# heyblackC/DFMIR

Measured on AMD Instinct MI355X. Metric: train-step image-pairs/sec (fwd+bwd): 2D 256x256 bs=16 and 3D 160^3 bs=1, higher is better.
Workload: dtype f32 (fp16x2-split MFMA, fp32 accumulate)

## Files before the change

dfmir_amd/csrc/common.h:

```cpp
#pragma once
#include <hip/hip_runtime.h>
#include <stdint.h>
#include <stdlib.h>
#include <atomic>
#include "../../include/dfmir_hip.h"

#define DF_LAUNCH_CHECK()                                  \
  do {                                                     \
    hipError_t e_ = hipGetLastError();                     \
    if (e_ != hipSuccess) return df_set_error((int)e_, __FILE__, __LINE__); \
  } while (0)
#define DF_ARG_CHECK(cond)                                 \
  do {                                                     \
    if (!(cond)) return df_set_error(-1, __FILE__, __LINE__); \
  } while (0)

int df_set_error(int code, const char* file, int line);

bool df_opt_get(const char* name, char* buf, int buf_len);
int df_opt_gen();
static inline bool df_opt_on(const char* name) {
  char b[8];
  return df_opt_get(name, b, sizeof(b)) && b[0] != 0 && !(b[0] == '0' && b[1] == 0);
}
struct DfOptFlag {
  const char* name;
  std::atomic<long long> st{-1};
  bool get() {
    const int g = df_opt_gen();
    const long long s = st.load(std::memory_order_relaxed);
    if (s >= 0 && (int)(s >> 1) == g) return (s & 1) != 0;
    const bool v = df_opt_on(name);
    st.store(((long long)g << 1) | (v ? 1 : 0), std::memory_order_relaxed);
    return v;
  }
};
struct DfOptInt {
  const char* name;
  int def;
  std::atomic<long long> st{-1};
  int get() {
    const int g = df_opt_gen();
    const long long s = st.load(std::memory_order_relaxed);
    if (s >= 0 && (int)(s >> 32) == g) return (int)(unsigned)(s & 0xffffffffLL);
    char b[32];
    const int v = df_opt_get(name, b, sizeof(b)) ? atoi(b) : def;
    st.store(((long long)g << 32) | (unsigned)v, std::memory_order_relaxed);
    return v;
  }
};

static inline unsigned df_grid(long long n, int bs, long long cap = 1LL << 20) {
  long long b = (n + bs - 1) / bs;
  if (b < 1) b = 1;
  if (b > cap) b = cap;
  return (unsigned)b;
}

static inline int df_cu_count() {
  static std::atomic<int> cache[64];
  int dev = 0;
  if (hipGetDevice(&dev) != hipSuccess || dev < 0 || dev >= 64) return 256;
  int v = cache[dev].load(std::memory_order_relaxed);
  if (v > 0) return v;
  if (hipDeviceGetAttribute(&v, hipDeviceAttributeMultiprocessorCount, dev) != hipSuccess || v <= 0) v = 256;
  cache[dev].store(v, std::memory_order_relaxed);
  return v;
}

const float* df_det_fx();
__device__ __forceinline__ void df_acc(float* base, long long idx, float v, const float* fx) {
  if (fx) atomicAdd(reinterpret_cast<unsigned long long*>(base) + idx, (unsigned long long)__float2ll_rn(v * fx[0]));
  else atomicAdd(base + idx, v);
}

static __global__ void df_zero_small_k(float* __restrict__ p, int n) {
  const int i = blockIdx.x * blockDim.x + threadIdx.x;
  if (i < n) p[i] = 0.f;
}
static inline hipError_t df_zero_async(float* p, int n, hipStream_t st) {
  df_zero_small_k<<<(unsigned)((n + 63) / 64), 64, 0, st>>>(p, n);
  return hipGetLastError();
}

__device__ __forceinline__ float wave_sum(float v) {
#pragma unroll
  for (int o = 32; o > 0; o >>= 1) v += __shfl_down(v, o, 64);
  return v;
}
__device__ __forceinline__ double wave_sum(double v) {
#pragma unroll
  for (int o = 32; o > 0; o >>= 1) v += __shfl_down(v, o, 64);
  return v;
}
__device__ __forceinline__ float wave_max(float v) {
#pragma unroll
  for (int o = 32; o > 0; o >>= 1) v = fmaxf(v, __shfl_down(v, o, 64));
  return v;
}

__device__ __forceinline__ float block_sum(float v, float* sm ) {
  const int lane = threadIdx.x & 63, wid = threadIdx.x >> 6;
  const int nw = (blockDim.x + 63) >> 6;
  v = wave_sum(v);
  __syncthreads();
  if (lane == 0) sm[wid] = v;
  __syncthreads();
  if (wid == 0) {
    float t = (lane < nw) ? sm[lane] : 0.f;
    t = wave_sum(t);
    if (lane == 0) sm[16] = t;
  }
  __syncthreads();
  return sm[16];
}
template <int T>
__device__ __forceinline__ double block_sum_ordered(double v, double* sm ) {
  v = wave_sum(v);
  __syncthreads();
  if ((threadIdx.x & 63) == 0) sm[threadIdx.x >> 6] = v;
  __syncthreads();
  double t = 0.0;
  if (threadIdx.x == 0)
    for (int w = 0; w < T / 64; ++w) t += sm[w];
  return t;
}
template <int T>
static __global__ __launch_bounds__(T) void df_slot_mean_k(const double* __restrict__ part, int nslots, double count,
                                                           float* __restrict__ out) {
  __shared__ double red[T / 64];
  double s = 0.0;
  for (int i = threadIdx.x; i < nslots; i += T) s += part[i];
  s = block_sum_ordered<T>(s, red);
  if (threadIdx.x == 0) out[0] = (float)(s / count);
}
__device__ __forceinline__ float block_max(float v, float* sm) {
  const int lane = threadIdx.x & 63, wid = threadIdx.x >> 6;
  const int nw = (blockDim.x + 63) >> 6;
  v = wave_max(v);
  __syncthreads();
  if (lane == 0) sm[wid] = v;
  __syncthreads();
  if (wid == 0) {
    float t = (lane < nw) ? sm[lane] : -3.0e38f;
    t = wave_max(t);
    if (lane == 0) sm[16] = t;
  }
  __syncthreads();
  return sm[16];
}
__device__ __forceinline__ void publish_block_absmax(float m, unsigned* smax, float* out_block) {
  const float t = wave_max(m);
  if ((threadIdx.x & 63) == 0) atomicMax(smax, __float_as_uint(t == t ? t : __uint_as_float(0x7f800000u)));
  __syncthreads();
  if (threadIdx.x == 0) *out_block = __uint_as_float(*smax);
}
#define DF_PROBE_SLOTS 64
__device__ __forceinline__ void publish_block_absmax_acc(float m, unsigned* smax, float* out) {
  const float t = wave_max(m);
  if ((threadIdx.x & 63) == 0) atomicMax(smax, __float_as_uint(t == t ? t : __uint_as_float(0x7f800000u)));
  __syncthreads();
  if (threadIdx.x == 0) atomicMax(reinterpret_cast<unsigned*>(out) + (blockIdx.x & (DF_PROBE_SLOTS - 1)), *smax);
}
__device__ __forceinline__ float reduce_absmax(const float* __restrict__ a, int n, float* sm) {
  if (n <= 1) return a[0];
  float m = 0.f;
  for (int i = threadIdx.x; i < n; i += blockDim.x) m = fmaxf(m, a[i]);
  return block_max(m, sm);
}

__device__ __forceinline__ bool df_in_coord(int o, int t, int stride, int pad, int dil, int size,
                                            int pad_mode, int& idx) {
  int c = o * stride - pad + t;
  if (dil == 1) {
    if (pad_mode == 1) {
      if (c < 0) c = -c;
      if (c >= size) c = 2 * (size - 1) - c;
      c = c < 0 ? 0 : (c >= size ? size - 1 : c);
      idx = c;
      return true;
    }
    idx = c;
    return (unsigned)c < (unsigned)size;
  }
  if (c < 0) { idx = 0; return false; }
  int q = c / dil;
  idx = q;
  return (q * dil == c) && (q < size);
}
```

dfmir_amd/csrc/conv3x3s.hip:

```cpp
#include "split_f16.h"

#ifndef PP_COMPUTE_PRIO
#define PP_COMPUTE_PRIO 1
#endif
#ifndef CS_COMPUTE_PRIO
#define CS_COMPUTE_PRIO 1
#endif
#ifndef CS_STORE_PRIO
#define CS_STORE_PRIO 0
#endif
typedef __bf16 bf16x8 __attribute__((ext_vector_type(8)));
typedef __bf16 bf16x2 __attribute__((ext_vector_type(2)));
typedef _Float16 f16x2 __attribute__((ext_vector_type(2)));
typedef float f32x2 __attribute__((ext_vector_type(2)));

__device__ __forceinline__ unsigned pk_bf16(float a, float b) {
  const f32x2 v = {a, b};
  return __builtin_bit_cast(unsigned, __builtin_convertvector(v, bf16x2));
}

template <int NSP>
__device__ __forceinline__ void split_pair(float x0, float x1, unsigned (&p)[NSP]) {
  if constexpr (NSP == 3) {
    p[0] = pk_bf16(x0, x1);
    const float r0 = x0 - __uint_as_float(p[0] << 16), r1 = x1 - __uint_as_float(p[0] & 0xffff0000u);
    p[1] = pk_bf16(r0, r1);
    p[2] = pk_bf16(r0 - __uint_as_float(p[1] << 16), r1 - __uint_as_float(p[1] & 0xffff0000u));
  } else {
    const f32x2 v = {x0, x1};
    const f16x2 h = __builtin_convertvector(v, f16x2);
    const f32x2 r = v - __builtin_convertvector(h, f32x2);
    p[0] = __builtin_bit_cast(unsigned, h);
    p[1] = __builtin_bit_cast(unsigned, __builtin_convertvector(r, f16x2));
  }
}
template <int NSP>
__device__ __forceinline__ void split_pair_s(float x0, float x1, float s, unsigned (&p)[NSP]) {
  if constexpr (NSP == 2) split_pair_scaled(x0, x1, s, p[0], p[1]);
  else split_pair<NSP>(x0, x1, p);
}
template <int NSP>
__device__ __forceinline__ void split8(const float v[8], u32x4 (&out)[NSP]) {
#pragma unroll
  for (int w = 0; w < 4; ++w) {
    unsigned p[NSP];
    split_pair<NSP>(v[2 * w], v[2 * w + 1], p);
#pragma unroll
    for (int s = 0; s < NSP; ++s) out[s][w] = p[s];
  }
}
template <int NSP>
__device__ __forceinline__ void split8_s(const float v[8], float s, u32x4 (&out)[NSP]) {
  if constexpr (NSP == 2) split8_scaled(v, s, out[0], out[1]);
  else split8<NSP>(v, out);
}
template <int NSP>
__device__ __forceinline__ f32x16 mma16(u32x4 a, u32x4 b, f32x16 c) {
  if constexpr (NSP == 3)
    return __builtin_amdgcn_mfma_f32_32x32x16_bf16(__builtin_bit_cast(bf16x8, a), __builtin_bit_cast(bf16x8, b), c, 0, 0, 0);
  else
    return mfma32_f16(a, b, c);
}
template <int NSP> struct Prod;
template <> struct Prod<3> { static constexpr int N = 6; static constexpr int A[6] = {2, 0, 1, 1, 0, 0}, B[6] = {0, 2, 1, 0, 1, 0}; };
template <> struct Prod<2> { static constexpr int N = 3; static constexpr int A[3] = {1, 0, 0}, B[3] = {0, 1, 0}; };

__global__ __launch_bounds__(256) void absmax_k(const float* __restrict__ x, long long n, unsigned* __restrict__ out) {
  __shared__ float red[8];
  float m = 0.f;
  const long long n4 = n >> 2;
  const float4* x4 = reinterpret_cast<const float4*>(x);
  const long long st = (long long)gridDim.x * 256;
  long long i = (long long)blockIdx.x * 256 + threadIdx.x;
  const float4 z4 = make_float4(0.f, 0.f, 0.f, 0.f);
  for (; i < n4; i += 4 * st) {
    const float4 a = x4[i];
    const float4 b = i + st < n4 ? x4[i + st] : z4;
    const float4 c = i + 2 * st < n4 ? x4[i + 2 * st] : z4;
    const float4 d = i + 3 * st < n4 ? x4[i + 3 * st] : z4;
    const float ma = fmaxf(fmaxf(fabsf(a.x), fabsf(a.y)), fmaxf(fabsf(a.z), fabsf(a.w)));
    const float mb = fmaxf(fmaxf(fabsf(b.x), fabsf(b.y)), fmaxf(fabsf(b.z), fabsf(b.w)));
    const float mc = fmaxf(fmaxf(fabsf(c.x), fabsf(c.y)), fmaxf(fabsf(c.z), fabsf(c.w)));
    const float md = fmaxf(fmaxf(fabsf(d.x), fabsf(d.y)), fmaxf(fabsf(d.z), fabsf(d.w)));
    m = fmaxf(m, fmaxf(fmaxf(ma, mb), fmaxf(mc, md)));
  }
  for (i = (n4 << 2) + (long long)blockIdx.x * 256 + threadIdx.x; i < n; i += (long long)gridDim.x * 256)
    m = fmaxf(m, fabsf(x[i]));
#pragma unroll
  for (int o = 32; o > 0; o >>= 1) m = fmaxf(m, __shfl_xor(m, o));
  if ((threadIdx.x & 63) == 0) red[threadIdx.x >> 6] = m;
  __syncthreads();
  if (threadIdx.x == 0) {
    m = fmaxf(fmaxf(red[0], red[1]), fmaxf(red[2], red[3]));
    if (!(m == m)) m = __uint_as_float(0x7f800000u);
    if (__float_as_uint(m) > *reinterpret_cast<volatile unsigned*>(out)) atomicMax(out, __float_as_uint(m));
  }
}
int df_absmax_launch(const float* x, long long n, float* out, hipStream_t st, bool zero_first) {
  if (zero_first) {
    hipError_t e = df_zero_async(out, 1, st);
    if (e != hipSuccess) return (int)e;
  }
  long long blocks = (n / 4 + 255) / 256;
  if (blocks < 1) blocks = 1;
  if (blocks > 2048) blocks = 2048;
  absmax_k<<<(unsigned)blocks, 256, 0, st>>>(x, n, reinterpret_cast<unsigned*>(out));
  return (int)hipGetLastError();
}

template <int NSP>
__global__ __launch_bounds__(256) void weight_split_k(const float* __restrict__ w_tcc, u32x4* __restrict__ out,
                                                      float* __restrict__ trailer, int npart, int K, int M) {
  __shared__ float red[17];
  const int chunks = (K + 7) >> 3;
  const long long total = (long long)chunks * 9 * M;
  int e = 0;
  if (NSP == 2) {
    e = scale_exp(reduce_absmax(trailer + 4, npart, red));
    if (blockIdx.x == 0 && threadIdx.x == 0) trailer[1] = (float)e;
  }
  const float sc = pow2f(e);
  for (long long i = (long long)blockIdx.x * 256 + threadIdx.x; i < total; i += (long long)gridDim.x * 256) {
    const int m = (int)(i % M);
    const int tap = (int)((i / M) % 9);
    const int ch = (int)(i / ((long long)9 * M));
    float v[8];
#pragma unroll
    for (int j = 0; j < 8; ++j) {
      const int kk = ch * 8 + j;
      v[j] = kk < K ? w_tcc[((long long)tap * K + kk) * M + m] * sc : 0.f;
    }
    u32x4 sp[NSP];
    split8<NSP>(v, sp);
    const long long base = (long long)ch * 9 * NSP * M + (long long)tap * M + m;
#pragma unroll
    for (int s = 0; s < NSP; ++s) out[base + (long long)s * 9 * M] = sp[s];
  }
}

int df_split_mode() {
  static std::atomic<long long> st{-1};
  const int g = df_opt_gen();
  const long long cur = st.load(std::memory_order_relaxed);
  if (cur >= 0 && (int)(cur >> 8) == g) return (int)(cur & 0xff);
  char s[16];
  const bool has = df_opt_get("DFMIR_CONV_SPLIT", s, sizeof(s));
  const int mode = df_opt_on("DFMIR_CONV_FP32") ? 0 : ((has && s[0] == 'b') ? 3 : 2);
  st.store(((long long)g << 8) | mode, std::memory_order_relaxed);
  return mode;
}

static inline float* split_section(const float* packed, int K, int M) {
  return const_cast<float*>(packed) + df_pack_tcc_floats(K, M, 9);
}
static inline float* split_trailer(const float* packed, int K, int M, int nsp) {
  return split_section(packed, K, M) + (long long)((K + 7) / 8) * 9 * nsp * M * 4;
}

float* df_weight_probe_slots(float* packed, int K, int M) {
  const int mode = df_split_mode();
  return mode == 2 ? split_trailer(packed, K, M, mode) + 4 : nullptr;
}
int df_weight_split_launch(const float* w_tcc, float* packed, int K, int M, int npart, hipStream_t st) {
  const int mode = df_split_mode();
  if (mode == 0) return 0;
  const long long total = (long long)((K + 7) / 8) * 9 * M;
  u32x4* sec = reinterpret_cast<u32x4*>(split_section(packed, K, M));
  float* tr = split_trailer(packed, K, M, mode);
  if (mode == 2) weight_split_k<2><<<df_grid(total, 256, 2048), 256, 0, st>>>(w_tcc, sec, tr, npart, K, M);
  else weight_split_k<3><<<df_grid(total, 256, 2048), 256, 0, st>>>(w_tcc, sec, tr, npart, K, M);
  return (int)hipGetLastError();
}

template <int NSP>
__global__ __launch_bounds__(256) void weight_split_batch_k(const DfPackJobDev* __restrict__ jobs) {
  const DfPackJobDev jb = jobs[blockIdx.y];
  if ((int)blockIdx.x >= jb.nsplit) return;
  __shared__ float red[17];
  const int K = jb.mode ? jb.Cout : jb.Cin, M = jb.mode ? jb.Cin : jb.Cout;
  const int chunks = (K + 7) >> 3;
  const long long total = (long long)chunks * 9 * M;
  int e = 0;
  if (NSP == 2) {
    e = scale_exp(reduce_absmax(jb.trailer + 4, jb.nblk, red));
    if (blockIdx.x == 0 && threadIdx.x == 0) jb.trailer[1] = (float)e;
  }
  const float sc = pow2f(e);
  u32x4* out = reinterpret_cast<u32x4*>(jb.sec);
  for (long long i = (long long)blockIdx.x * 256 + threadIdx.x; i < total; i += (long long)jb.nsplit * 256) {
    const int m = (int)(i % M);
    const int tap = (int)((i / M) % 9);
    const int ch = (int)(i / ((long long)9 * M));
    float v[8];
#pragma unroll
    for (int j = 0; j < 8; ++j) {
      const int kk = ch * 8 + j;
      v[j] = kk < K ? jb.o[((long long)tap * K + kk) * M + m] * sc : 0.f;
    }
    u32x4 sp[NSP];
    split8<NSP>(v, sp);
    const long long base = (long long)ch * 9 * NSP * M + (long long)tap * M + m;
#pragma unroll
    for (int s = 0; s < NSP; ++s) out[base + (long long)s * 9 * M] = sp[s];
  }
}
void df_weight_split_fill(DfPackJobDev* j) {
  const int mode = df_split_mode();
  j->part = nullptr; j->sec = nullptr; j->trailer = nullptr; j->nsplit = 0;
  if (j->T != 9 || mode == 0) return;
  const int K = j->mode ? j->Cout : j->Cin, M = j->mode ? j->Cin : j->Cout;
  j->sec = split_section(j->o, K, M);
  j->trailer = split_trailer(j->o, K, M, mode);
  j->part = mode == 2 ? j->trailer + 4 : nullptr;
  j->nsplit = (int)df_grid((long long)((K + 7) / 8) * 9 * M, 256, 2048);
}
int df_weight_split_batch_launch(const DfPackJobDev* jobs_dev, int njobs, int max_nsplit, hipStream_t st) {
  const int mode = df_split_mode();
  if (mode == 0 || max_nsplit <= 0) return 0;
  const dim3 grid((unsigned)max_nsplit, (unsigned)njobs);
  if (mode == 2) weight_split_batch_k<2><<<grid, 256, 0, st>>>(jobs_dev);
  else weight_split_batch_k<3><<<grid, 256, 0, st>>>(jobs_dev);
  return (int)hipGetLastError();
}

template <int NSP, int BM, int XP, int TM, int TN, int NV>
__device__ __forceinline__ void split_mma_chunk(const u32x4* __restrict__ Ab, const u32x4* __restrict__ Xb,
                                                const int (&aoff)[5], const int (&bidx)[5][TN],
                                                f32x16 (&acc)[TM][TN]) {
  using P = Prod<NSP>;
  u32x4 a[2][TM][NSP], b[2][TN][NSP];
#define SPLIT_LOAD(set_, pr_)                                                                    \
  {                                                                                              \
    _Pragma("unroll") for (int i = 0; i < TM; ++i)                                               \
      _Pragma("unroll") for (int s = 0; s < NSP; ++s) a[set_][i][s] = Ab[s * 9 * BM + aoff[pr_] + i * 32]; \
    _Pragma("unroll") for (int j = 0; j < TN; ++j)                                               \
      _Pragma("unroll") for (int s = 0; s < NSP; ++s) b[set_][j][s] = Xb[s * XP + bidx[pr_][j]]; \
  }
  SPLIT_LOAD(0, 0)
#pragma unroll
  for (int pr = 0; pr < 5; ++pr) {
    if (pr < 4) SPLIT_LOAD((pr + 1) & 1, pr + 1)
#pragma unroll
    for (int q = 0; q < P::N; ++q)
#pragma unroll
      for (int i = 0; i < TM; ++i)
#pragma unroll
        for (int j = 0; j < TN; ++j)
          acc[i][j] = mma16<NSP>(a[pr & 1][i][P::A[q]], b[pr & 1][j][P::B[q]], acc[i][j]);
  }
#undef SPLIT_LOAD
  constexpr int NL = NSP * (TM + TN), NM = P::N * TM * TN;
  constexpr int LP = NL < NM ? NL : NM;
  constexpr int VP = ((NV + 3) / 4 < NM - LP) ? (NV + 3) / 4 : NM - LP;
#pragma unroll
  for (int i = 0; i < NL; ++i) __builtin_amdgcn_sched_group_barrier(0x100, 1, 0);
#pragma unroll
  for (int pr = 0; pr < 4; ++pr) {
#pragma unroll
    for (int i = 0; i < LP; ++i) {
      __builtin_amdgcn_sched_group_barrier(0x008, 1, 0);
      __builtin_amdgcn_sched_group_barrier(0x100, 1, 0);
      if (i == LP - 1) {
#pragma unroll
        for (int e = 0; e < NL - LP; ++e) __builtin_amdgcn_sched_group_barrier(0x100, 1, 0);
      }
    }
#pragma unroll
    for (int i = 0; i < VP; ++i) {
      __builtin_amdgcn_sched_group_barrier(0x008, 1, 0);
      __builtin_amdgcn_sched_group_barrier(0x020, 1, 0);
    }
#pragma unroll
    for (int i = 0; i < NM - LP - VP; ++i) __builtin_amdgcn_sched_group_barrier(0x008, 1, 0);
  }
#pragma unroll
  for (int i = 0; i < NM; ++i) __builtin_amdgcn_sched_group_barrier(0x008, 1, 0);
}

struct SplitScale {
  const float* x_amax;
  int x_n;
  const float* w_trailer;
};

template <int NSP, int XP, int BM>
__global__ __launch_bounds__(512, 1) void conv3x3_split_pp_k(const float* __restrict__ x,
                                                             const u32x4* __restrict__ ws,
                                                             const float* __restrict__ bias,
                                                             float* __restrict__ y, Conv3P k, SplitScale sc) {
  constexpr int BNG = 128, CK = 8, TM = 2, TN = (BM == 128) ? 2 : 1, WN = (BM == 128) ? 2 : 4;
  constexpr int NS = (XP + 255) / 256;
  constexpr int WU = 9 * NSP * BM, WH = WU / 2;
  constexpr int NW = (WH + 255) / 256;
  constexpr int ZPOS = XP - 1;
  __shared__ __attribute__((aligned(16))) u32x4 As[2][WU];
  __shared__ __attribute__((aligned(16))) u32x4 Xs[2][NSP * XP];
  __shared__ float bs[BM];

  const int grp = threadIdx.x >> 8, tid = threadIdx.x & 255, lane = tid & 63, wid = tid >> 6;
  const int wm = wid / WN, wn = wid % WN;
  const int l31 = lane & 31, lhi = lane >> 5;
  const int HWo = k.Ho * k.Wo, HWi = k.Hi * k.Wi;
  const int n = blockIdx.x / k.tiles_per_img;
  const int t = blockIdx.x - n * k.tiles_per_img;
  const int p0 = t * (2 * BNG) + grp * BNG;
  const bool gvalid = p0 < HWo;
  const int pend = (p0 + BNG < HWo) ? p0 + BNG : HWo;
  const int m0 = blockIdx.y * BM;
  const int y0 = p0 / k.Wo, y1 = (pend - 1) / k.Wo;
  const bool single = (y0 == y1);
  const int x0 = p0 - y0 * k.Wo, x1 = (pend - 1) - y1 * k.Wo;
  const int xoff = single ? x0 : 0;
  const int ncols = single ? (x1 - x0 + 3) : (k.Wo + 2);
  const int nrows = y1 - y0 + 3;
  const int npos = gvalid ? nrows * ncols : 0;
  u32x4* __restrict__ Xg = Xs[grp];

  float xscale = 1.f, oscale = 1.f, oscale2 = 1.f;
  if (NSP == 2) {
    const int ex = scale_exp(reduce_absmax(sc.x_amax, sc.x_n, bs));
    __syncthreads();
    const int ew = (int)sc.w_trailer[1];
    xscale = pow2f(ex);
    oscale = pow2f(-ex);
    oscale2 = pow2f(-ew);
  }

  constexpr unsigned OOB = 0x80000000u;
  unsigned gvo[NS][CK];
#pragma unroll
  for (int s = 0; s < NS; ++s) {
    const int pos = tid + 256 * s;
    int off = -1;
    if (pos < npos) {
      const int r = pos / ncols, c = pos - r * ncols;
      off = halo_offset(y0 - k.pad + r, xoff - k.pad + c, k.Hi, k.Wi, k.pad_mode);
    }
#pragma unroll
    for (int c = 0; c < CK; ++c) gvo[s][c] = off < 0 ? OOB : (unsigned)(off + c * HWi) * 4u;
  }
  if ((int)threadIdx.x < BM) bs[threadIdx.x] = (bias && (m0 + (int)threadIdx.x) < k.Cout) ? bias[m0 + threadIdx.x] : 0.f;
  if (tid < NSP) Xg[tid * XP + ZPOS] = u32x4{0u, 0u, 0u, 0u};

  int pbase[TN];
#pragma unroll
  for (int j = 0; j < TN; ++j) {
    int q = p0 + (wn * TN + j) * 32 + l31;
    q = q < pend ? q : pend - 1;
    const int yy = q / k.Wo, xx = q - yy * k.Wo;
    pbase[j] = (yy - y0) * ncols + (xx - xoff);
  }
  int aoff[5], bidx[5][TN];
#pragma unroll
  for (int pr = 0; pr < 5; ++pr) {
    const int tp = (pr == 4) ? 8 : 2 * pr + lhi;
    aoff[pr] = tp * BM + wm * TM * 32 + l31;
#pragma unroll
    for (int j = 0; j < TN; ++j)
      bidx[pr][j] = ((pr == 4) && lhi) ? ZPOS : pbase[j] + (tp / 3) * ncols + (tp % 3);
  }

  f32x16 acc[TM][TN];
#pragma unroll
  for (int i = 0; i < TM; ++i)
#pragma unroll
    for (int j = 0; j < TN; ++j)
#pragma unroll
      for (int r = 0; r < 16; ++r) acc[i][j][r] = 0.f;

  const float* xn = x + (long long)n * k.Cin * HWi;
  const int chunks = (k.Cin + CK - 1) / CK;
  unsigned wbyte[NW];
#pragma unroll
  for (int j = 0; j < NW; ++j) {
    const int loc = tid + 256 * j;
    const int idx = grp * WH + loc;
    const int seg = idx / BM, co = m0 + (idx % BM);
    wbyte[j] = (loc < WH && co < k.Cout) ? (unsigned)(seg * k.Cout + co) * 16u : OOB;
  }
  const int wunits = 9 * NSP * k.Cout;

  u32x4 rw[NW];
  unsigned rx[NS][CK];

#define P3_GLOADW(ch_)                                                                           \
  {                                                                                              \
    const int c_ = (ch_);                                                                        \
    const __amdgpu_buffer_rsrc_t rw_ = __builtin_amdgcn_make_buffer_rsrc(                        \
        const_cast<u32x4*>(ws + (long long)c_ * wunits), 0, c_ < chunks ? (unsigned)wunits * 16u : 0u, 0x00020000); \
    _Pragma("unroll") for (int j = 0; j < NW; ++j)                                               \
      rw[j] = __builtin_amdgcn_raw_buffer_load_b128(rw_, wbyte[j], 0, 0);                        \
  }
#define P3_GLOADX(ch_)                                                                           \
  {                                                                                              \
    const int c0_ = (ch_) * CK;                                                                  \
    const int left_ = k.Cin - c0_;                                                               \
    const __amdgpu_buffer_rsrc_t rx_ = __builtin_amdgcn_make_buffer_rsrc(                        \
        const_cast<float*>(xn + (long long)c0_ * HWi), 0,                                        \
        left_ > 0 ? (unsigned)((left_ < CK ? left_ : CK) * HWi) * 4u : 0u, 0x00020000);          \
    _Pragma("unroll") for (int s = 0; s < NS; ++s) {                                             \
      _Pragma("unroll") for (int c = 0; c < CK; ++c)                                             \
        rx[s][c] = __builtin_amdgcn_raw_buffer_load_b32(rx_, gvo[s][c], 0, 0);                   \
    }                                                                                            \
  }
#define P3_LSTOREW(buf_)                                                                         \
  {                                                                                              \
    _Pragma("unroll") for (int j = 0; j < NW; ++j) {                                             \
      const int loc = tid + 256 * j;                                                             \
      if (loc < WH) As[buf_][grp * WH + loc] = rw[j];                                            \
    }                                                                                            \
  }
#define P3_LSTOREX()                                                                             \
  {                                                                                              \
    _Pragma("unroll") for (int s = 0; s < NS; ++s) {                                             \
      const int pos = tid + 256 * s;                                                             \
      if (pos < npos) {                                                                          \
        float v[8];                                                                              \
        _Pragma("unroll") for (int c = 0; c < CK; ++c)                                           \
          v[c] = __uint_as_float(rx[s][c]);                                                      \
        u32x4 sp[NSP];                                                                           \
        split8_s<NSP>(v, xscale, sp);                                                                      \
        _Pragma("unroll") for (int q = 0; q < NSP; ++q) Xg[q * XP + pos] = sp[q];                \
      }                                                                                          \
    }                                                                                            \
  }

  P3_GLOADW(0);
  P3_GLOADX(0);
  P3_LSTOREW(0);
  P3_LSTOREX();
  if (grp == 1 && chunks > 1) P3_GLOADW(1);
  __syncthreads();

  for (int h = 0; h < 2 * chunks; ++h) {
    const int c = h >> 1;
    if ((h & 1) == grp) {
      __builtin_amdgcn_s_setprio(PP_COMPUTE_PRIO);
      if (gvalid) {
        P3_GLOADX(c + 1);
        P3_GLOADW(c + 1 + grp);
        split_mma_chunk<NSP, BM, XP, TM, TN, NW + NS * CK>(As[c & 1], Xg, aoff, bidx, acc);
      } else {
        P3_GLOADW(c + 1 + grp);
      }
    } else {
      __builtin_amdgcn_s_setprio(0);
      const int cx = c + 1 - grp;
      if (cx < chunks && h > 0) P3_LSTOREX();
      if (c + 1 < chunks) P3_LSTOREW((c + 1) & 1);
    }
    __syncthreads();
  }
#undef P3_GLOADW
#undef P3_GLOADX
#undef P3_LSTOREW
#undef P3_LSTOREX

  if (!gvalid) return;
  float* yb = y + (long long)n * k.Cout * HWo;
#pragma unroll
  for (int j = 0; j < TN; ++j) {
    const int q = p0 + (wn * TN + j) * 32 + l31;
    if (q >= pend) continue;
#pragma unroll
    for (int i = 0; i < TM; ++i) {
      const int cl = (wm * TM + i) * 32 + 4 * lhi;
#pragma unroll
      for (int r = 0; r < 16; ++r) {
        const int cc = cl + (r & 3) + 8 * (r >> 2);
        const int co = m0 + cc;
        if (co < k.Cout) {
          float v = (NSP == 2 ? acc[i][j][r] * oscale * oscale2 : acc[i][j][r]) + bs[cc];
          if (k.act == 1) v = v > 0.f ? v : v * k.slope;
          else if (k.act == 2) v = tanhf(v);
          yb[(long long)co * HWo + q] = v;
        }
      }
    }
  }
}

constexpr int CS_TH = 8, CS_TW = 32, CS_PW = CS_TW + 2, CS_XP = 352;

template <int CPG, int XP, int NW, int NS>
__device__ __forceinline__ void cs_mma_chunk_rr(const u32x4* __restrict__ Ab, const u32x4* __restrict__ Xb, int abase,
                                                int xb, f32x16 (&acc)[4],
                                                const __amdgpu_buffer_rsrc_t rw_, const unsigned (&wb)[NW], u32x4 (&rw)[NW],
                                                const __amdgpu_buffer_rsrc_t rx_, const unsigned (&gvo)[NS][8],
                                                unsigned (&rx)[NS][8]) {
  constexpr int SA = 9 * 2 * CPG, SX = 2 * XP;
  constexpr int NL = NW + 8 * NS;
  using P = Prod<2>;
  u32x4 a[9][2], xr[3][6][2];
#define CS_LDA(st_, s_) a[st_][s_] = Ab[(s_) * SA + (((st_) % 3) * 3 + (st_) / 3) * (2 * CPG) + abase];
#define CS_LDX(kx_, r_, s_) xr[kx_][r_][s_] = Xb[(s_) * SX + xb + (r_) * CS_PW + (kx_)];
#define CS_NEED(n_)                                                                              \
  {                                                                                              \
    constexpr int kx_ = (n_) / 3, ky_ = (n_) % 3;                                                \
    CS_LDA(n_, 1)                                                                                \
    if (ky_ == 0) { _Pragma("unroll") for (int r = 0; r < 4; ++r) CS_LDX(kx_, r, 0) }            \
    else CS_LDX(kx_, ky_ + 3, 0)                                                                 \
    CS_LDA(n_, 0)                                                                                \
    if (ky_ == 0) { _Pragma("unroll") for (int r = 0; r < 4; ++r) CS_LDX(kx_, r, 1) }            \
    else CS_LDX(kx_, ky_ + 3, 1)                                                                 \
  }
  CS_NEED(0)
  __builtin_amdgcn_sched_barrier(0);
#pragma unroll
  for (int st = 0; st < 9; ++st) {
    const int kx = st / 3, ky = st % 3;
    int nds = 0;
    if (st == 0) { CS_NEED(1) CS_NEED(2) nds = 8; }
    else if (st == 1) { CS_NEED(3) nds = 10; }
    else if (st == 2) { CS_NEED(4) nds = 4; }
    else if (st == 3) { CS_NEED(5) nds = 4; }
    else if (st == 4) { CS_NEED(6) nds = 10; }
    else if (st == 5) { CS_NEED(7) nds = 4; }
    else if (st == 6) { CS_NEED(8) nds = 4; }
    int L0, nvm;
    if (NL == 25) {
      L0 = st == 0 ? 0 : st == 1 ? 4 : st == 2 ? 6 : st == 3 ? 10 : st == 4 ? 14 : st == 5 ? 16 : st == 6 ? 20 : 24;
      nvm = (st == 1 || st == 4) ? 2 : (st == 7 ? 1 : (st == 8 ? 0 : 4));
    } else {
      const int lo = NL / 8, ex = NL % 8;
      L0 = st * lo + (st < ex ? st : ex);
      nvm = st < 8 ? lo + (st < ex ? 1 : 0) : 0;
    }
#pragma unroll
    for (int q = 0; q < (NL + 7) / 8; ++q) {
      const int L = L0 + q;
      if (q < nvm) {
        if (L < NW) rw[L] = __builtin_amdgcn_raw_buffer_load_b128(rw_, wb[L], 0, 0);
        else if (L < NL) rx[(L - NW) >> 3][(L - NW) & 7] = __builtin_amdgcn_raw_buffer_load_b32(rx_, gvo[(L - NW) >> 3][(L - NW) & 7], 0, 0);
      }
    }
#pragma unroll
    for (int q = 0; q < P::N; ++q)
#pragma unroll
      for (int j = 0; j < 4; ++j)
        acc[j] = mma16<2>(xr[kx][ky + j][P::B[q]], a[st][P::A[q]], acc[j]);
#pragma unroll
    for (int i = 0; i < 12; ++i) {
      __builtin_amdgcn_sched_group_barrier(0x008, 1, 0);
      if (i < nds) __builtin_amdgcn_sched_group_barrier(0x100, 1, 0);
      if (i >= 12 - nvm) __builtin_amdgcn_sched_group_barrier(0x020, 1, 0);
    }
    __builtin_amdgcn_sched_barrier(0);
  }
#undef CS_NEED
#undef CS_LDA
#undef CS_LDX
}

struct ConvCsP {
  int N, Cin, Cout, Hi, Wi, Ho, Wo, pad, pad_mode, act;
  float slope;
  int tiles_x, tiles_y;
  const float* res;
  const float* ring;
  int ring_rl;
  int xcd_pair;
  int dephase;
  int vec4;
};

#ifdef CS_TRACE
__device__ unsigned g_cs_trace[8 * 32 * 8 + 8];
extern "C" int dfmir_cs_trace_dump(unsigned* out) {
  return (int)hipMemcpyFromSymbol(out, HIP_SYMBOL(g_cs_trace), sizeof(unsigned) * (8 * 32 * 8 + 8));
}
#define TRC(slot_) { if (trace_blk && lane == 0) trc[((grp * 4 + wid) * 32 + (h & 31)) * 8 + (slot_)] = (unsigned)__builtin_readcyclecounter(); }
__device__ unsigned g_cs_wg[2048 * 6];
extern "C" int dfmir_cs_wg_dump(unsigned* out) {
  return (int)hipMemcpyFromSymbol(out, HIP_SYMBOL(g_cs_wg), sizeof(unsigned) * 2048 * 6);
}
#define WGT(slot_) { if (threadIdx.x == 0 && bix < 2048 && biy == 0) g_cs_wg[bix * 6 + (slot_)] = (unsigned)wall_clock64(); }
#else
#define WGT(slot_)
#define TRC(slot_)
#endif
template <int CPG, int TH>
struct CsLds {
  static constexpr int XP = (TH == 8 ? CS_XP : 640);
  static constexpr int WUG = 2 * 9 * 2 * CPG;
  static constexpr int XSU = 2 * 2 * XP;
  static constexpr int XS_OFF = 2 * WUG * 16, BS_OFF = XS_OFF + 2 * XSU * 16, BYTES = BS_OFF + 2 * CPG * 4;
};
template <int CPG, int TH>
__global__ __launch_bounds__(512, 1) void conv3x3_split_cs_k(const float* __restrict__ x, const u32x4* __restrict__ ws,
                                                             const float* __restrict__ bias, float* __restrict__ y,
                                                             ConvCsP k, SplitScale sc) {
  using L = CsLds<CPG, TH>;
  __shared__ __attribute__((aligned(16))) u32x4 Wg[2][L::WUG];
  __shared__ __attribute__((aligned(16))) u32x4 Xs[2][L::XSU];
  __shared__ float bs[2 * CPG];
  const int bix = (int)blockIdx.x, biy = (int)blockIdx.y, gdx = (int)gridDim.x;
#include "conv3x3s_cs_body.inc"
}

#ifdef DFMIR_BUILD_W1
#include "../../scripts/ubench/conv3x3_split_w1.inc"
#endif

static bool cs_plan(const DfConvGeom* g, int* th_out, int* tx_out, int* ty_out) {
  if (df_split_mode() != 2) return false;
  const int th = g->Cout > 64 ? 8 : 16;
  const int tx = (g->Wo + CS_TW - 1) / CS_TW, ty = (g->Ho + th - 1) / th;
  const double fill = (double)g->Ho * g->Wo / ((double)tx * CS_TW * ty * th);
  if (!((long long)g->N * tx * ty < (1LL << 31) && fill >= 0.85)) return false;
  *th_out = th; *tx_out = tx; *ty_out = ty;
  return true;
}
static bool split_fwd_geom_ok(const DfConvGeom* g) {
  if (!(g->KD == 1 && g->KH == 3 && g->KW == 3 && g->Di == 1 && g->Do == 1 && g->stride == 1 && g->dil == 1))
    return false;
  if (g->Cout <= 32 || g->Cin < 16 || g->ph != g->pw || g->pd != 0) return false;
  const int p = g->ph;
  if (!(p == 1 || (p == 2 && g->pad_mode == 0))) return false;
  if (g->Ho != g->Hi + 2 * p - 2 || g->Wo != g->Wi + 2 * p - 2) return false;
  const long long HWo = (long long)g->Ho * g->Wo;
  if (HWo >= (1LL << 30) || (long long)g->Hi * g->Wi >= (1LL << 30)) return false;
  if ((long long)((g->Cin + 7) / 8) * 27 * g->Cout * 16 >= (1LL << 31)) return false;
  if (worst_npos(g->Wo, (int)HWo, 128) > 399) return false;
  return true;
}
int df_conv3x3_split_res_ok(const DfConvGeom* g) {
  int th, tx, ty;
  return (df_split_mode() == 2 && split_fwd_geom_ok(g) && cs_plan(g, &th, &tx, &ty)) ? 1 : 0;
}
struct CsLaunch {
  ConvCsP kc;
  dim3 grid;
  int form;
};
static bool cs_setup(const DfConvGeom* g, const float* res, const float* ring, int ring_rl, const float* y, CsLaunch* L) {
  int th = 0, tlx = 0, tly = 0;
  if (!cs_plan(g, &th, &tlx, &tly)) return false;
  ConvCsP kc{g->N, g->Cin, g->Cout, g->Hi, g->Wi, g->Ho, g->Wo, g->ph, g->pad_mode, g->act, g->slope, tlx, tly, res,
             ring, ring_rl, 0, 0, 0};
  kc.vec4 = (g->Wo % 4 == 0 && ((uintptr_t)y & 15) == 0 && ((uintptr_t)res & 15) == 0) ? 1 : 0;
  static DfOptInt dephase_o{"DFMIR_CS_DEPHASE", 0};
  const long long nb = (long long)g->N * tlx * tly;
  if (nb * ((g->Cout + 127) / 128) >= 512) kc.dephase = dephase_o.get();
  static DfOptInt xcd_o{"DFMIR_CS_XCD_PAIR", 2};
  const int xcd_pair = xcd_o.get();
  if (g->Cout > 64) {
    dim3 grid((unsigned)nb, (unsigned)((g->Cout + 127) / 128));
    if (xcd_pair && grid.y <= 2 && (nb & 7) == 0) {
      kc.xcd_pair = xcd_pair == 1 ? (grid.y == 2 ? 1 : 0) : (int)grid.y + 1;
      if (kc.xcd_pair) grid = dim3((unsigned)(grid.y * nb), 1u);
    }
    L->grid = grid;
    L->form = 1;
  } else {
    if (xcd_pair >= 2 && (nb & 7) == 0) kc.xcd_pair = 2;
    L->grid = dim3((unsigned)nb, 1u);
    L->form = 2;
  }
  L->kc = kc;
  return true;
}
bool df_conv3x3_split_fwd_try(const DfConvGeom* g, const float* x, const float* x_amax, int x_n, const float* w_packed,
                              const float* bias, const float* res, const float* ring, int ring_rl, float* y,
                              hipStream_t st, int* rc) {
  const int mode = df_split_mode();
  if (mode == 0 || (mode == 2 && !(x_amax && x_n > 0))) return false;
  if (!split_fwd_geom_ok(g)) return false;
  const int p = g->ph;
  const long long HWo = (long long)g->Ho * g->Wo;
  Conv3P k{g->N, g->Cin, g->Cout, g->Hi, g->Wi, g->Ho, g->Wo, p, g->pad_mode, g->act, g->slope, 0};
  const u32x4* ws = reinterpret_cast<const u32x4*>(split_section(w_packed, g->Cin, g->Cout));
  const SplitScale sc{x_amax, x_n, split_trailer(w_packed, g->Cin, g->Cout, mode)};
  CsLaunch cl;
  if (mode == 2 && cs_setup(g, res, ring, ring_rl, y, &cl)) {
    const ConvCsP& kc = cl.kc;
    if (cl.form == 1) {
#ifdef DFMIR_BUILD_W1
      static DfOptFlag w1_o{"DFMIR_CONV_W1"};
      if (w1_o.get() && kc.vec4 && g->act != 2 && (g->Cin % 16) == 0 && (g->Ho % 16) == 0 && (g->Wo % 32) == 0) {
        ConvCsP kw = kc;
        kw.tiles_y = g->Ho / 16;
        const long long nbw = (long long)g->N * kw.tiles_x * kw.tiles_y;
        const unsigned gyw = (unsigned)((g->Cout + 127) / 128);
        kw.xcd_pair = 0;
        dim3 gw((unsigned)nbw, gyw);
        if ((nbw & 7) == 0 && gyw <= 2) { kw.xcd_pair = (int)gyw + 1; gw = dim3((unsigned)(gyw * nbw), 1u); }
        conv3x3_split_w1_k<0><<<gw, 256, 0, st>>>(x, ws, bias, y, kw, sc);
      } else
#endif
      conv3x3_split_cs_k<64, 8><<<cl.grid, 512, 0, st>>>(x, ws, bias, y, kc, sc);
    } else {
      conv3x3_split_cs_k<32, 16><<<cl.grid, 512, 0, st>>>(x, ws, bias, y, kc, sc);
    }
    hipError_t e = hipGetLastError();
    *rc = (e == hipSuccess) ? 0 : df_set_error((int)e, __FILE__, __LINE__);
    return true;
  }
  if (res || ring) { *rc = df_set_error((int)hipErrorInvalidValue, __FILE__, __LINE__); return true; }
  k.tiles_per_img = (int)((HWo + 255) / 256);
  const bool big = g->Cout > 64;
  dim3 grid((unsigned)(g->N * k.tiles_per_img), big ? (unsigned)((g->Cout + 127) / 128) : 1u);
  if (mode == 2) {
    if (big) conv3x3_split_pp_k<2, 400, 128><<<grid, 512, 0, st>>>(x, ws, bias, y, k, sc);
    else conv3x3_split_pp_k<2, 400, 64><<<grid, 512, 0, st>>>(x, ws, bias, y, k, sc);
  } else {
    if (big) conv3x3_split_pp_k<3, 400, 128><<<grid, 512, 0, st>>>(x, ws, bias, y, k, sc);
    else conv3x3_split_pp_k<3, 400, 64><<<grid, 512, 0, st>>>(x, ws, bias, y, k, sc);
  }
  hipError_t e = hipGetLastError();
  *rc = (e == hipSuccess) ? 0 : df_set_error((int)e, __FILE__, __LINE__);
  return true;
}

struct WS3P {
  int N, Cin, Cout, H, W, pad_mode;
  int runs_per_row, runs_per_img, runs_total, runs_per_block;
  const float* x_amax;
  const float* dy_amax;
  int x_n, dy_n;
  float* db;
  const float* dy_pmax;
  int swap;
  float* dbx;
  const float* fx;
};

template <int NSP, int BC>
__global__ __launch_bounds__(512, 1) void conv3x3_wgrad_split_k(const float* __restrict__ x,
                                                                const float* __restrict__ dy,
                                                                float* __restrict__ dwt, WS3P k) {
  using P = Prod<NSP>;
  constexpr int CT = 64, NWC = BC / 32, KS = 4 / NWC, NSTEP = 18 / KS;
  constexpr int XSLAB = 2 * CT;
  __shared__ __attribute__((aligned(16))) u32x4 Xc[NSP * 3 * 4 * XSLAB];
  __shared__ __attribute__((aligned(16))) u32x4 Dy[NSP * 2 * 2 * BC];
  __shared__ float bsum[BC];

  const int tid = threadIdx.x, lane = tid & 63, wid = tid >> 6;
  const bool want_db = k.db != nullptr && blockIdx.y == 0;
  if (tid < BC) bsum[tid] = 0.f;
  float bacc = 0.f;
  const int wc = wid % NWC, wi = (wid / NWC) & 1, kh = wid / (2 * NWC);
  const int l31 = lane & 31, lhi = lane >> 5;
  const int HW = k.H * k.W;
  const int ci0 = blockIdx.y * CT, co0 = blockIdx.z * BC;
  const int run_beg = blockIdx.x * k.runs_per_block;
  int run_end = run_beg + k.runs_per_block;
  if (run_end > k.runs_total) run_end = k.runs_total;

  float xscale = 1.f, dscale = 1.f, oscale = 1.f, oscale2 = 1.f;
  if (NSP == 2) {
    __shared__ float red[17];
    const int ex = scale_exp(reduce_absmax(k.x_amax, k.x_n, red));
    __syncthreads();
    const int ed = scale_exp(reduce_absmax(k.dy_amax, k.dy_n, red));
    xscale = pow2f(ex); dscale = pow2f(ed); oscale = pow2f(-ex); oscale2 = pow2f(-ed);
  }

  const int xc = tid & 63, xu = (tid >> 6) & 1, xr = tid >> 7;
  const int dc = tid % BC, du = (tid / BC) & 1, dk = (tid / (2 * BC)) & 1;
  const bool dload = tid < 4 * BC;
  const unsigned hw4 = (unsigned)HW * 4u;
  constexpr unsigned OOB = 0x80000000u;

  f32x16 acc[9];
#pragma unroll
  for (int t = 0; t < 9; ++t)
#pragma unroll
    for (int r = 0; r < 16; ++r) acc[t][r] = 0.f;

  u32x4 rxa, rxb, rda, rdb;
  unsigned rxl, rxr;

#define WS_GLOAD(run_)                                                                           \
  {                                                                                              \
    const int n_ = (run_) / k.runs_per_img;                                                      \
    const int q_ = (run_) - n_ * k.runs_per_img;                                                 \
    const int yp_ = q_ / k.runs_per_row, xs_ = q_ - yp_ * k.runs_per_row;                        \
    const int y0_ = 2 * yp_, x0_ = 16 * xs_ + 8 * xu;                                            \
    const __amdgpu_buffer_rsrc_t bx_ = __builtin_amdgcn_make_buffer_rsrc(                        \
        const_cast<float*>(x + (long long)n_ * k.Cin * HW), 0, (unsigned)(k.Cin * HW) * 4u, 0x00020000); \
    const __amdgpu_buffer_rsrc_t bd_ = __builtin_amdgcn_make_buffer_rsrc(                        \
        const_cast<float*>(dy + (long long)n_ * k.Cout * HW), 0, (unsigned)(k.Cout * HW) * 4u, 0x00020000); \
    const bool cok_ = ci0 + xc < k.Cin;                                                          \
    const unsigned cb_ = (unsigned)(ci0 + xc) * hw4;                                             \
     \
                                             \
    int ry_ = y0_ - 1 + xr;                                                                      \
    bool rok_ = (unsigned)ry_ < (unsigned)k.H;                                                   \
    if (k.pad_mode == 1) { ry_ = ry_ < 0 ? -ry_ : (ry_ >= k.H ? 2 * (k.H - 1) - ry_ : ry_); rok_ = true; } \
    const int rb_ = ry_ * k.W;                                                                   \
    const bool lin_ = x0_ > 0, rin_ = x0_ + 8 < k.W;                                             \
    const int ol_ = rb_ + (lin_ ? x0_ - 1 : 1), or_ = rb_ + (rin_ ? x0_ + 8 : k.W - 2);          \
    const bool lok_ = rok_ && cok_ && (lin_ || k.pad_mode == 1), rrok_ = rok_ && cok_ && (rin_ || k.pad_mode == 1); \
    const unsigned xb_ = (rok_ && cok_) ? cb_ + (unsigned)(rb_ + x0_) * 4u : OOB;                \
    rxa = __builtin_amdgcn_raw_buffer_load_b128(bx_, xb_, 0, 0);                                 \
    rxb = __builtin_amdgcn_raw_buffer_load_b128(bx_, xb_ == OOB ? OOB : xb_ + 16u, 0, 0);        \
    rxl = __builtin_amdgcn_raw_buffer_load_b32(bx_, lok_ ? cb_ + (unsigned)ol_ * 4u : OOB, 0, 0); \
    rxr = __builtin_amdgcn_raw_buffer_load_b32(bx_, rrok_ ? cb_ + (unsigned)or_ * 4u : OOB, 0, 0); \
    const unsigned db_ = (co0 + dc >= k.Cout || !dload) ? OOB                                    \
        : (unsigned)(co0 + dc) * hw4 + (unsigned)((y0_ + dk) * k.W + 16 * xs_ + 8 * du) * 4u;    \
    rda = __builtin_amdgcn_raw_buffer_load_b128(bd_, db_, 0, 0);                                 \
    rdb = __builtin_amdgcn_raw_buffer_load_b128(bd_, db_ == OOB ? OOB : db_ + 16u, 0, 0);        \
  }
#define WS_LSTORE()                                                                              \
  {                                                                                              \
    float r[10];                                                                                 \
    r[0] = __uint_as_float(rxl); r[9] = __uint_as_float(rxr);                                    \
    _Pragma("unroll") for (int e = 0; e < 4; ++e) { r[1 + e] = __uint_as_float(rxa[e]); r[5 + e] = __uint_as_float(rxb[e]); } \
    unsigned pa[5][NSP], pb[4][NSP];                                                             \
    _Pragma("unroll") for (int i = 0; i < 5; ++i) split_pair_s<NSP>(r[2 * i], r[2 * i + 1], xscale, pa[i]); \
    if (NSP == 2) {             \
      _Pragma("unroll") for (int i = 0; i < 4; ++i)                                              \
        _Pragma("unroll") for (int s = 0; s < NSP; ++s) pb[i][s] = __builtin_amdgcn_alignbit(pa[i + 1][s], pa[i][s], 16); \
    } else {                                                                                     \
      _Pragma("unroll") for (int i = 0; i < 4; ++i) split_pair<NSP>(r[2 * i + 1], r[2 * i + 2], pb[i]); \
    }                                                                                            \
    _Pragma("unroll") for (int s = 0; s < NSP; ++s) {                                            \
      u32x4* dst = Xc + ((s * 3 * 4 + xr) * 2 + xu) * CT + xc;                                   \
      dst[0] = u32x4{pa[0][s], pa[1][s], pa[2][s], pa[3][s]};                                    \
      dst[4 * XSLAB] = u32x4{pb[0][s], pb[1][s], pb[2][s], pb[3][s]};                            \
      dst[8 * XSLAB] = u32x4{pa[1][s], pa[2][s], pa[3][s], pa[4][s]};                            \
    }                                                                                            \
    float v[8];                                                                                  \
    _Pragma("unroll") for (int e = 0; e < 4; ++e) { v[e] = __uint_as_float(rda[e]); v[4 + e] = __uint_as_float(rdb[e]); } \
    bacc += ((v[0] + v[1]) + (v[2] + v[3])) + ((v[4] + v[5]) + (v[6] + v[7]));    \
    u32x4 sp[NSP];                                                                               \
    split8_s<NSP>(v, dscale, sp);                                                                \
    if (dload) { _Pragma("unroll") for (int s = 0; s < NSP; ++s) Dy[((s * 2 + dk) * 2 + du) * BC + dc] = sp[s]; } \
  }

  if (run_beg < run_end) {
    WS_GLOAD(run_beg);
    WS_LSTORE();
  }
  __syncthreads();

  const int abase = lhi * CT + wi * 32 + l31 + (KS == 2 ? kh * XSLAB : 0);
  const int bbase = lhi * BC + wc * 32 + l31 + (KS == 2 ? kh * 2 * BC : 0);
  for (int run = run_beg; run < run_end; ++run) {
    const bool more = (run + 1) < run_end;
    if (more) WS_GLOAD(run + 1);
    u32x4 b[NSP], a[2][NSP];
#define WS_LOADA(set_, step_)                                                                    \
  _Pragma("unroll") for (int s = 0; s < NSP; ++s)                                                \
    a[set_][s] = Xc[((s * 3 + ((step_) % 3)) * 4 + (step_) / 9 + ((step_) % 9) / 3) * XSLAB + abase];
    WS_LOADA(0, 0)
#pragma unroll
    for (int step = 0; step < NSTEP; ++step) {
      if (step % 9 == 0) {
#pragma unroll
        for (int s = 0; s < NSP; ++s) b[s] = Dy[(s * 2 + step / 9) * 2 * BC + bbase];
      }
      if (step + 1 < NSTEP) WS_LOADA((step + 1) & 1, step + 1)
#pragma unroll
      for (int q = 0; q < P::N; ++q)
        acc[step % 9] = mma16<NSP>(a[step & 1][P::A[q]], b[P::B[q]], acc[step % 9]);
    }
#undef WS_LOADA
#pragma unroll
    for (int i = 0; i < 2 * NSP; ++i) __builtin_amdgcn_sched_group_barrier(0x100, 1, 0);
#pragma unroll
    for (int step = 0; step < NSTEP; ++step) {
      const int nr = (step + 1 < NSTEP ? NSP : 0) + ((step + 1) % 9 == 0 && step + 1 < NSTEP ? NSP : 0);
#pragma unroll
      for (int i = 0; i < P::N; ++i) {
        __builtin_amdgcn_sched_group_barrier(0x008, 1, 0);
        if (i < nr) __builtin_amdgcn_sched_group_barrier(0x100, 1, 0);
        if (i == P::N - 1) {
#pragma unroll
          for (int e = P::N; e < nr; ++e) __builtin_amdgcn_sched_group_barrier(0x100, 1, 0);
        }
      }
    }
    if (more) {
      __syncthreads();
      WS_LSTORE();
      __syncthreads();
    }
  }
#undef WS_GLOAD
#undef WS_LSTORE

  if (want_db) {
    if (dload) atomicAdd(&bsum[dc], bacc);
    __syncthreads();
    if (tid < BC && co0 + tid < k.Cout) atomicAdd(&k.db[co0 + tid], bsum[tid]);
  }
  const int co = co0 + wc * 32 + l31;
  if (co < k.Cout) {
#pragma unroll
    for (int t = 0; t < 9; ++t) {
#pragma unroll
      for (int r = 0; r < 16; ++r) {
        const int ci = ci0 + wi * 32 + 4 * lhi + (r & 3) + 8 * (r >> 2);
        if (ci < k.Cin)
          df_acc(dwt, ((long long)t * k.Cin + ci) * k.Cout + co, NSP == 2 ? acc[t][r] * oscale * oscale2 : acc[t][r], k.fx);
      }
    }
  }
}

struct RingP {
  int N, K, M, H, W;
  int RL;
  const float* cols;
};
constexpr int RING_KG = 32;

template <int RP>
__global__ __launch_bounds__(512) void conv3x3_reflect_ring_k(const float* __restrict__ dy, const u32x4* __restrict__ ws,
                                                              float* __restrict__ ring, RingP k, SplitScale sc) {
  constexpr int NSP = 2;
  using P = Prod<2>;
  __shared__ __attribute__((aligned(16))) u32x4 Ls[NSP * RING_KG * RP];
  __shared__ float red[17];
  const int tid = threadIdx.x, lane = tid & 63;
  const int wid = __builtin_amdgcn_readfirstlane((int)(threadIdx.x >> 6));
  const int l31 = lane & 31, lhi = lane >> 5;
  const int strip = blockIdx.x & 3, n = blockIdx.x >> 2;
  const int m0 = blockIdx.y * 128;
  const bool rowstrip = strip < 2;
  const int L = rowstrip ? k.W : k.H;
  const int HW = k.H * k.W;
  const float* dyl = dy + (long long)n * k.K * HW +
                     (strip == 0 ? 0 : strip == 1 ? (k.H - 1) * k.W : strip == 2 ? 0 : k.W - 1);
  const int istr = rowstrip ? 1 : k.W;

  const int ex = scale_exp(reduce_absmax(sc.x_amax, sc.x_n, red));
  const int ew = (int)sc.w_trailer[1];
  const float xscale = pow2f(ex), oscale = pow2f(-ex), oscale2 = pow2f(-ew);

  const int kg_n = (k.K + 7) >> 3;
  {
    const int npad = RP - L;
    for (int it = tid; it < NSP * RING_KG * npad; it += 512) {
      const int q = it % npad, g = it / npad;
      Ls[g * RP + (q < 2 ? q : L + q)] = u32x4{0u, 0u, 0u, 0u};
    }
    const int kz = RING_KG - kg_n;
    for (int it = tid; it < NSP * kz * L; it += 512) {
      const int i = it % L, g = it / L, s2 = g / kz, kg = kg_n + g % kz;
      Ls[(s2 * RING_KG + kg) * RP + i + 2] = u32x4{0u, 0u, 0u, 0u};
    }
  }
  for (int it = tid; it < kg_n * L; it += 512) {
    const int i = it % L, kg = it / L;
    float v[8];
#pragma unroll
    for (int e = 0; e < 8; ++e) {
      const int kk = kg * 8 + e;
      if (!rowstrip && k.cols) v[e] = kk < k.K ? k.cols[(((long long)n * k.K + kk) * 2 + (strip - 2)) * k.H + i] : 0.f;
      else v[e] = kk < k.K ? dyl[(long long)kk * HW + (long long)i * istr] : 0.f;
    }
    u32x4 sp[NSP];
    split8_s<NSP>(v, xscale, sp);
#pragma unroll
    for (int s = 0; s < NSP; ++s) Ls[(s * RING_KG + kg) * RP + i + 2] = sp[s];
  }
  __syncthreads();

  const int mb = wid & 3, kh = wid >> 2;
  const int m = m0 + mb * 32 + l31;
  const int nb_n = (L + 2 + 31) >> 5;
  f32x16 acc[3];
#pragma unroll
  for (int b = 0; b < 3; ++b)
#pragma unroll
    for (int r = 0; r < 16; ++r) acc[b][r] = 0.f;
  const int chunks = (k.K + 15) >> 4;
  const int tap0 = strip == 0 ? 6 : strip == 1 ? 0 : strip == 2 ? 2 : 0, tapd = rowstrip ? 1 : 3;
  u32x4 a[3][NSP], an[3][NSP], an2[3][NSP];
#define RING_LOADA(dst_, c_)                                                                     \
  {                                                                                              \
    const int kg_ = 2 * (c_) + lhi;                                                              \
    const bool ok_ = (c_) < chunks && kg_ < kg_n && m < k.M;                                     \
    _Pragma("unroll") for (int j = 0; j < 3; ++j)                                                \
      _Pragma("unroll") for (int s = 0; s < NSP; ++s)                                            \
        dst_[j][s] = ok_ ? ws[((long long)kg_ * NSP * 9 + s * 9 + tap0 + j * tapd) * k.M + m] : u32x4{0u, 0u, 0u, 0u}; \
  }
  RING_LOADA(a, kh)
  RING_LOADA(an, kh + 2)
  for (int c = kh; c < chunks; c += 2) {
    RING_LOADA(an2, c + 4)
    const int kg = 2 * c + lhi;
#pragma unroll
    for (int j = 0; j < 3; ++j) {
#pragma unroll
      for (int b = 0; b < 3; ++b) {
        if (b < nb_n) {
          int pos = b * 32 + l31 + j;
          pos = pos < RP ? pos : RP - 1;
          u32x4 x2[NSP];
#pragma unroll
          for (int s = 0; s < NSP; ++s) x2[s] = Ls[(s * RING_KG + kg) * RP + pos];
#pragma unroll
          for (int q = 0; q < P::N; ++q) acc[b] = mma16<NSP>(a[j][P::A[q]], x2[P::B[q]], acc[b]);
        }
      }
    }
#pragma unroll
    for (int j = 0; j < 3; ++j)
#pragma unroll
      for (int s = 0; s < NSP; ++s) { a[j][s] = an[j][s]; an[j][s] = an2[j][s]; }
  }
#undef RING_LOADA

  __syncthreads();
  float* xch = reinterpret_cast<float*>(Ls);
  if (kh == 1) {
#pragma unroll
    for (int b = 0; b < 3; ++b)
#pragma unroll
      for (int r = 0; r < 16; ++r) xch[((mb * 3 + b) * 16 + r) * 64 + lane] = acc[b][r];
  }
  __syncthreads();
  if (kh == 1) return;
  float* rg = ring + ((long long)(n * 4 + strip) * k.M) * k.RL;
#pragma unroll
  for (int b = 0; b < 3; ++b) {
    if (b >= nb_n) continue;
    const int c = b * 32 + l31;
    if (c > L + 1) continue;
#pragma unroll
    for (int r = 0; r < 16; ++r) {
      const int mm = m0 + mb * 32 + 4 * lhi + (r & 3) + 8 * (r >> 2);
      if (mm < k.M)
        rg[(long long)mm * k.RL + c] = (acc[b][r] + xch[((mb * 3 + b) * 16 + r) * 64 + lane]) * oscale * oscale2;
    }
  }
}

int df_conv3x3_reflect_ring_ok(const DfConvGeom* g) {
  if (df_split_mode() != 2) return 0;
  if (!(g->KD == 1 && g->KH == 3 && g->KW == 3 && g->Di == 1 && g->Do == 1 && g->stride == 1 && g->dil == 1)) return 0;
  if (g->pad_mode != 1 || g->ph != 1 || g->pw != 1 || g->pd != 0) return 0;
  if (g->Ho != g->Hi || g->Wo != g->Wi || g->Hi < 4 || g->Wi < 4 || g->Hi > 94 || g->Wi > 94) return 0;
  if (g->Cout > 8 * RING_KG || g->Cout < 16 || g->Cin <= 32) return 0;
  return 1;
}
int df_conv3x3_reflect_ring_len(const DfConvGeom* g) { return ((g->Hi > g->Wi ? g->Hi : g->Wi) + 2 + 3) & ~3; }
int df_conv3x3_reflect_ring_launch(const DfConvGeom* g, const float* dy, const float* dy_cols, const float* dy_amax,
                                   int dy_n, const float* wd_packed, float* ring, hipStream_t st) {
  const RingP k{g->N, g->Cout, g->Cin, g->Hi, g->Wi, df_conv3x3_reflect_ring_len(g), dy_cols};
  const u32x4* ws = reinterpret_cast<const u32x4*>(split_section(wd_packed, g->Cout, g->Cin));
  const SplitScale sc{dy_amax, dy_n, split_trailer(wd_packed, g->Cout, g->Cin, 2)};
  const dim3 grid((unsigned)(4 * g->N), (unsigned)((g->Cin + 127) / 128));
  if (g->Hi <= 64 && g->Wi <= 64) conv3x3_reflect_ring_k<72><<<grid, 512, 0, st>>>(dy, ws, ring, k, sc);
  else conv3x3_reflect_ring_k<100><<<grid, 512, 0, st>>>(dy, ws, ring, k, sc);
  return (int)hipGetLastError();
}

#ifdef W2_TRACE
__device__ unsigned g_w2_trace[8 * 64 * 8];
extern "C" int dfmir_w2_trace_dump(unsigned* out) {
  return (int)hipMemcpyFromSymbol(out, HIP_SYMBOL(g_w2_trace), sizeof(g_w2_trace));
}
#define W2T(slot_) { if (trace_blk && lane == 0 && run - run_beg < 64) g_w2_trace[(wid * 64 + (run - run_beg)) * 8 + (slot_)] = (unsigned)__builtin_readcyclecounter(); }
#define W2T_VM() { __builtin_amdgcn_s_waitcnt(0x0f70); W2T(4) }
#else
#define W2T(slot_)
#define W2T_VM()
#endif
#ifndef W2_ALT
#define W2_ALT 0
#endif
#ifndef W2_PRIO_C
#define W2_PRIO_C 0
#endif
#ifndef W2_PRIO_G0
#define W2_PRIO_G0 1
#endif
#ifndef W2_PRIO_G1
#define W2_PRIO_G1 2
#endif
#ifndef W2_CTPAD
#define W2_CTPAD 0
#endif
struct W2Lds {
  static constexpr int XCU = 2 * 3 * 4 * 2 * (64 + W2_CTPAD), DYU = 2 * 2 * 2 * 128;
  static constexpr int DY_OFF = 2 * XCU * 16, EDC_OFF = DY_OFF + 2 * DYU * 16, RED_OFF = EDC_OFF + 128 * 4, BYTES = RED_OFF + 80;
};
__global__ __launch_bounds__(512, 1) void conv3x3_wgrad_split2_k(const float* __restrict__ x,
                                                                 const float* __restrict__ dy,
                                                                 float* __restrict__ dwt, WS3P k) {
  __shared__ __attribute__((aligned(16))) u32x4 Xc[2 * W2Lds::XCU];
  __shared__ __attribute__((aligned(16))) u32x4 Dy[2 * W2Lds::DYU];
  __shared__ float red[17];
  __shared__ int edc[128];
  const unsigned bix = blockIdx.x, biy = blockIdx.y, biz = blockIdx.z;
#include "conv3x3s_w2_body.inc"
}

bool df_conv3x3_split_wgrad_swaps(const DfConvGeom* g) {
  return df_split_mode() == 2 && g->KD == 1 && g->KH == 3 && g->KW == 3 && g->Di == 1 && g->Do == 1 && g->stride == 1 &&
         g->dil == 1 && g->ph == 1 && g->pw == 1 && g->pd == 0 && g->Ho == g->Hi && g->Wo == g->Wi && g->pad_mode == 0 &&
         g->Cout == 64 && g->Cin > 64;
}
static bool ws_setup(const DfConvGeom* g, const float* x_amax, int x_n, const float* dy_amax, int dy_n, float* db,
                     const float* dy_pmax, WS3P* kp, dim3* grid, int* which) {
  const int mode = df_split_mode();
  if (mode == 0 || (mode == 2 && !(x_amax && dy_amax && x_n > 0 && dy_n > 0))) return false;
  if (!(g->KD == 1 && g->KH == 3 && g->KW == 3 && g->Di == 1 && g->Do == 1 && g->stride == 1 && g->dil == 1))
    return false;
  if (g->ph != 1 || g->pw != 1 || g->pd != 0 || g->Ho != g->Hi || g->Wo != g->Wi) return false;
  if (g->Cout < 64 || g->Cin < 64) return false;
  const bool wide = g->Cout > 64;
  if ((g->Hi & 1) || (g->Wi & 15) || g->Hi < 2) return false;
  const long long HW = (long long)g->Hi * g->Wi;
  if (HW * g->Cin * 4 >= (1LL << 31) || HW * g->Cout * 4 >= (1LL << 31)) return false;
  const bool swap = mode == 2 && x_amax && dy_amax && df_conv3x3_split_wgrad_swaps(g);
  WS3P k{g->N, g->Cin, g->Cout, g->Hi, g->Wi, g->pad_mode, g->Wi / 16, 0, 0, 0, x_amax, dy_amax, x_n, dy_n, db, dy_pmax, 0, nullptr, df_det_fx()};
  if (swap) {
    k.Cin = g->Cout; k.Cout = g->Cin;
    k.x_amax = dy_amax; k.dy_amax = x_amax; k.x_n = dy_n; k.dy_n = x_n;
    k.db = nullptr; k.dbx = db; k.dy_pmax = nullptr; k.swap = 1;
  }
  k.runs_per_img = (g->Hi / 2) * k.runs_per_row;
  const long long total = (long long)g->N * k.runs_per_img;
  if (total >= (1LL << 30)) return false;
  k.runs_total = (int)total;
  const unsigned ny = (k.Cin + 63) / 64, nz = (wide || swap) ? (k.Cout + 127) / 128 : 1;
  long long want = 256 / ((long long)ny * nz);
  if (want < 1) want = 1;
  long long maxs = (k.runs_total + 7) / 8;
  if (maxs < 1) maxs = 1;
  if (want > maxs) want = maxs;
  k.runs_per_block = (int)((k.runs_total + want - 1) / want);
  const unsigned nx = (k.runs_total + k.runs_per_block - 1) / k.runs_per_block;
  *grid = dim3(nx, ny, nz);
  *kp = k;
  if (mode == 2) *which = swap ? 1 : wide ? 2 : 3;
  else *which = wide ? 4 : 5;
  return true;
}
bool df_conv3x3_split_wgrad_try(const DfConvGeom* g, const float* x, const float* x_amax, int x_n, const float* dy,
                                const float* dy_amax, int dy_n, float* dw_tcc, float* db, hipStream_t st, int* rc,
                                const float* dy_pmax) {
  WS3P k;
  dim3 grid;
  int which = 0;
  if (!ws_setup(g, x_amax, x_n, dy_amax, dy_n, db, dy_pmax, &k, &grid, &which)) return false;
  if (which == 1) conv3x3_wgrad_split2_k<<<grid, 512, 0, st>>>(dy, x, dw_tcc, k);
  else if (which == 2) conv3x3_wgrad_split2_k<<<grid, 512, 0, st>>>(x, dy, dw_tcc, k);
  else if (which == 3) conv3x3_wgrad_split_k<2, 64><<<grid, 512, 0, st>>>(x, dy, dw_tcc, k);
  else if (which == 4) conv3x3_wgrad_split_k<3, 128><<<grid, 512, 0, st>>>(x, dy, dw_tcc, k);
  else conv3x3_wgrad_split_k<3, 64><<<grid, 512, 0, st>>>(x, dy, dw_tcc, k);
  hipError_t e = hipGetLastError();
  *rc = (e == hipSuccess) ? 0 : df_set_error((int)e, __FILE__, __LINE__);
  return true;
}

struct PairP {
  int order;
  int nd, ndx;
  int nw, nwx, nwy;
  int gd, gw;
};
template <int CPG, int TH>
__global__ __launch_bounds__(512, 1) void conv3x3_bwd_pair_k(const float* __restrict__ dyd, const u32x4* __restrict__ ws,
                                                             float* __restrict__ dx, ConvCsP kc, SplitScale sc,
                                                             const float* __restrict__ xw, const float* __restrict__ dyw,
                                                             float* __restrict__ dwt, WS3P kw, PairP pp) {
  constexpr int LDS_B = CsLds<CPG, TH>::BYTES > W2Lds::BYTES ? CsLds<CPG, TH>::BYTES : W2Lds::BYTES;
  __shared__ __attribute__((aligned(16))) unsigned char lds[LDS_B];
  const int id = (int)blockIdx.x;
  bool wg;
  int l;
  if (pp.order == 0) {
    wg = id < 8 * pp.gw;
    l = wg ? id : id - 8 * pp.gw;
  } else if (pp.order == 1) {
    wg = id >= 8 * pp.gd;
    l = wg ? id - 8 * pp.gd : id;
  } else {
    const unsigned long long g = (unsigned)id >> 3, tot = (unsigned)(pp.gd + pp.gw);
    const int wb = (int)(g * (unsigned)pp.gw / tot);
    wg = (int)((g + 1) * (unsigned)pp.gw / tot) > wb;
    l = ((wg ? wb : (int)g - wb) << 3) | (id & 7);
  }
  if (!wg) {
    if (l >= pp.nd) return;
    using L = CsLds<CPG, TH>;
    const float* __restrict__ x = dyd;
    const float* __restrict__ bias = nullptr;
    float* __restrict__ y = dx;
    const ConvCsP& k = kc;
    const int bix = l % pp.ndx, biy = l / pp.ndx, gdx = pp.ndx;
    u32x4 (*Wg)[L::WUG] = reinterpret_cast<u32x4 (*)[L::WUG]>(lds);
    u32x4 (*Xs)[L::XSU] = reinterpret_cast<u32x4 (*)[L::XSU]>(lds + L::XS_OFF);
    float* bs = reinterpret_cast<float*>(lds + L::BS_OFF);
#include "conv3x3s_cs_body.inc"
  } else {
    if (l >= pp.nw) return;
    const float* __restrict__ x = xw;
    const float* __restrict__ dy = dyw;
    const WS3P& k = kw;
    const int t = l / pp.nwx;
    const unsigned bix = (unsigned)(l - t * pp.nwx), biy = (unsigned)(t % pp.nwy), biz = (unsigned)(t / pp.nwy);
    u32x4* Xc = reinterpret_cast<u32x4*>(lds);
    u32x4* Dy = reinterpret_cast<u32x4*>(lds + W2Lds::DY_OFF);
    int* edc = reinterpret_cast<int*>(lds + W2Lds::EDC_OFF);
    float* red = reinterpret_cast<float*>(lds + W2Lds::RED_OFF);
#include "conv3x3s_w2_body.inc"
  }
}

#ifndef DF_BWD_PAIR_DEFAULT
#define DF_BWD_PAIR_DEFAULT 1
#endif
#ifndef DF_BWD_PAIR_ORDER_DEFAULT
#define DF_BWD_PAIR_ORDER_DEFAULT 1
#endif
static bool bwd_pair_enabled() {
  static DfOptFlag no_o{"DFMIR_NO_BWD_PAIR"};
  static DfOptInt on_o{"DFMIR_BWD_PAIR", DF_BWD_PAIR_DEFAULT};
  return !no_o.get() && on_o.get() != 0;
}
static bool bwd_pair_setup(const DfConvGeom* gd, const DfConvGeom* gw, const float* dy_amax, int dy_n, const float* x_amax,
                           int x_n, const float* res, const float* ring, int ring_rl, const float* dx, float* db,
                           const float* dy_pmax, CsLaunch* cl, WS3P* kw, dim3* wgrid, int* which) {
  if (!bwd_pair_enabled() || df_split_mode() != 2) return false;
  if (!(gd->N == gw->N && gd->Cin == gw->Cout && gd->Cout == gw->Cin && gd->Hi == gw->Ho && gd->Wi == gw->Wo &&
        gd->Ho == gw->Hi && gd->Wo == gw->Wi && gd->act == 0))
    return false;
  if (!(dy_amax && dy_n > 0 && x_amax && x_n > 0)) return false;
#ifdef DFMIR_BUILD_W1
  static DfOptFlag w1_o{"DFMIR_CONV_W1"};
  if (w1_o.get()) return false;
#endif
  if (!split_fwd_geom_ok(gd) || !cs_setup(gd, res, ring, ring_rl, dx, cl)) return false;
  if (!ws_setup(gw, x_amax, x_n, dy_amax, dy_n, db, dy_pmax, kw, wgrid, which) || *which > 2 || kw->fx != nullptr) return false;
  const long long nd = (long long)cl->grid.x * cl->grid.y, nw = (long long)wgrid->x * wgrid->y * wgrid->z;
  return nd + nw + 16 < (1LL << 31);
}
int df_conv3x3_bwd_pair_ok(const DfConvGeom* gd, const DfConvGeom* gw) {
  static const float one = 1.f;
  CsLaunch cl;
  WS3P kw;
  dim3 wgrid;
  int which = 0;
  return bwd_pair_setup(gd, gw, &one, 1, &one, 1, nullptr, nullptr, 0, nullptr, nullptr, nullptr, &cl, &kw, &wgrid, &which) ? 1 : 0;
}
bool df_conv3x3_bwd_pair_try(const DfConvGeom* gd, const DfConvGeom* gw, const float* dy, const float* dy_amax, int dy_n,
                             const float* dy_pmax, const float* wd_packed, const float* res, const float* ring, int ring_rl,
                             float* dx, const float* x, const float* x_amax, int x_n, float* dw_tcc, float* db,
                             hipStream_t st, int* rc) {
  CsLaunch cl;
  WS3P kw;
  dim3 wgrid;
  int which = 0;
  if (!bwd_pair_setup(gd, gw, dy_amax, dy_n, x_amax, x_n, res, ring, ring_rl, dx, db, dy_pmax, &cl, &kw, &wgrid, &which))
    return false;
  static DfOptInt order_o{"DFMIR_BWD_PAIR_ORDER", DF_BWD_PAIR_ORDER_DEFAULT};
  int order = order_o.get();
  if (order < 0 || order > 2) order = DF_BWD_PAIR_ORDER_DEFAULT;
  const u32x4* ws = reinterpret_cast<const u32x4*>(split_section(wd_packed, gd->Cin, gd->Cout));
  const SplitScale sc{dy_amax, dy_n, split_trailer(wd_packed, gd->Cin, gd->Cout, 2)};
  PairP pp;
  pp.order = order;
  pp.nd = (int)(cl.grid.x * cl.grid.y); pp.ndx = (int)cl.grid.x;
  pp.nw = (int)(wgrid.x * wgrid.y * wgrid.z); pp.nwx = (int)wgrid.x; pp.nwy = (int)wgrid.y;
  pp.gd = (pp.nd + 7) >> 3; pp.gw = (pp.nw + 7) >> 3;
  const dim3 grid((unsigned)(8 * (pp.gd + pp.gw)));
  const float* xw = which == 1 ? dy : x;
  const float* dyw = which == 1 ? x : dy;
  if (cl.form == 1) conv3x3_bwd_pair_k<64, 8><<<grid, 512, 0, st>>>(dy, ws, dx, cl.kc, sc, xw, dyw, dw_tcc, kw, pp);
  else conv3x3_bwd_pair_k<32, 16><<<grid, 512, 0, st>>>(dy, ws, dx, cl.kc, sc, xw, dyw, dw_tcc, kw, pp);
  hipError_t e = hipGetLastError();
  *rc = (e == hipSuccess) ? 0 : df_set_error((int)e, __FILE__, __LINE__);
  return true;
}
```

dfmir_amd/csrc/conv3x3s_cs_body.inc:

```
  static_assert((CPG == 64 && TH == 8) || (CPG == 32 && TH == 16), "tile forms");
  constexpr int CS_TH = TH;
  constexpr int NSP = 2, XP = CsLds<CPG, TH>::XP, NPOS = (CS_TH + 2) * CS_PW;
  constexpr int WUG = NSP * 9 * 2 * CPG;
  constexpr int NW = (WUG + 255) / 256;
  constexpr int NS = (NPOS + 255) / 256;
  static_assert(WUG == CsLds<CPG, TH>::WUG && NSP * 2 * XP == CsLds<CPG, TH>::XSU, "arena layout");
#ifdef CS_TRACE
  __shared__ unsigned trc[8 * 32 * 8];
  const bool trace_blk = bix == 300 && biy == 0;
  const unsigned long long trc_t0 = __builtin_readcyclecounter(), trc_r0 = wall_clock64();
#endif

  const int grp = __builtin_amdgcn_readfirstlane((int)(threadIdx.x >> 8));
  const int tid = threadIdx.x & 255, lane = tid & 63, wid = tid >> 6;
  const int l31 = lane & 31, lhi = lane >> 5;
  const int HWo = k.Ho * k.Wo, HWi = k.Hi * k.Wi;
  if (k.dephase > 0 && biy == 0 && bix < 256) {
    const unsigned long long t0 = wall_clock64();
    const unsigned wait = (unsigned)bix * (unsigned)k.dephase >> 8;
    while ((unsigned)(wall_clock64() - t0) < wait) __builtin_amdgcn_s_sleep(4);
  }
  WGT(0)
#ifdef CS_TRACE
  if (threadIdx.x == 0 && bix < 2048 && biy == 0) {
    g_cs_wg[bix * 6 + 4] = __builtin_amdgcn_s_getreg(63492);
    g_cs_wg[bix * 6 + 5] = __builtin_amdgcn_s_getreg(63508);
  }
#endif
  int bt = bix, bm = biy;
  if (k.xcd_pair == 1) { bm = (bt >> 3) & 1; bt = ((bt >> 4) << 3) + (bt & 7); }
  else if (k.xcd_pair >= 2) {
    const int ny = k.xcd_pair - 1, per = (gdx >> 3) / ny, j = bt >> 3;
    bm = j % ny;
    bt = (bt & 7) * per + j / ny;
  }
  const int tx = bt % k.tiles_x; bt /= k.tiles_x;
  const int ty = bt % k.tiles_y;
  const int n = bt / k.tiles_y;
  const int oy0 = ty * CS_TH, ox0 = tx * CS_TW;
  const int m0 = bm * (2 * CPG), m0g = m0 + CPG * grp;

  const int ex = scale_exp(reduce_absmax(sc.x_amax, sc.x_n, bs));
  __syncthreads();
  const int ew = (int)sc.w_trailer[1];
  const float xscale = pow2f(ex), oscale = pow2f(-ex), oscale2 = pow2f(-ew);

  constexpr unsigned OOB = 0x80000000u;
  unsigned gvo[NS][8];
#pragma unroll
  for (int s = 0; s < NS; ++s) {
    const int pos = tid + 256 * s;
    int off = -1;
    if (pos < NPOS) {
      const int r = pos / CS_PW, c = pos - r * CS_PW;
      off = halo_offset(oy0 - k.pad + r, ox0 - k.pad + c, k.Hi, k.Wi, k.pad_mode);
    }
#pragma unroll
    for (int c = 0; c < 8; ++c) gvo[s][c] = off < 0 ? OOB : (unsigned)(off + (8 * grp + c) * HWi) * 4u;
  }
  if (threadIdx.x < 2 * CPG) bs[threadIdx.x] = (bias && (m0 + (int)threadIdx.x) < k.Cout) ? bias[m0 + threadIdx.x] : 0.f;

  const int rowgrp = CPG == 64 ? (wid >> 1) : wid;
  const int xb = lhi * XP + 4 * rowgrp * CS_PW + l31;
  const int abase = lhi * CPG + l31 + (CPG == 64 ? 32 * (wid & 1) : 0);

  f32x16 acc[4];
#pragma unroll
  for (int i = 0; i < 4; ++i)
#pragma unroll
    for (int r = 0; r < 16; ++r) acc[i][r] = 0.f;

  const float* xn = x + (long long)n * k.Cin * HWi;
  const int chunks8 = (k.Cin + 7) / 8, chunks = (k.Cin + 15) / 16;
  unsigned wb[NW];
#pragma unroll
  for (int j = 0; j < NW; ++j) {
    const int idx = tid + 256 * j;
    const int co = m0g + (idx % CPG), r = idx / CPG;
    const int half = r & 1, st = r >> 1;
    wb[j] = (idx < WUG && co < k.Cout) ? (unsigned)((half * NSP * 9 + st) * k.Cout + co) * 16u : OOB;
  }
  const int wunits8 = NSP * 9 * k.Cout;

  u32x4 rw[NW];
  unsigned rx[NS][8];
#define CS_GLOADW(c_)                                                                            \
  {                                                                                              \
    const int q_ = 2 * (c_);                                                                     \
    const int left_ = chunks8 - q_;                                                              \
    const __amdgpu_buffer_rsrc_t rw_ = __builtin_amdgcn_make_buffer_rsrc(                        \
        const_cast<u32x4*>(ws + (long long)q_ * wunits8), 0,                                     \
        left_ > 0 ? (unsigned)((left_ < 2 ? left_ : 2) * wunits8) * 16u : 0u, 0x00020000);       \
    _Pragma("unroll") for (int j = 0; j < NW; ++j) rw[j] = __builtin_amdgcn_raw_buffer_load_b128(rw_, wb[j], 0, 0); \
  }
#define CS_GLOADX(c_)                                                                            \
  {                                                                                              \
    const int c0_ = 16 * (c_);                                                                   \
    const int left_ = k.Cin - c0_;                                                               \
    const __amdgpu_buffer_rsrc_t rx_ = __builtin_amdgcn_make_buffer_rsrc(                        \
        const_cast<float*>(xn + (long long)c0_ * HWi), 0,                                        \
        left_ > 0 ? (unsigned)((left_ < 16 ? left_ : 16) * HWi) * 4u : 0u, 0x00020000);          \
    _Pragma("unroll") for (int s = 0; s < NS; ++s)                                               \
      _Pragma("unroll") for (int c = 0; c < 8; ++c)                                              \
        rx[s][c] = __builtin_amdgcn_raw_buffer_load_b32(rx_, gvo[s][c], 0, 0);                   \
  }
#define CS_LSTOREW()                                                                             \
  { _Pragma("unroll") for (int j = 0; j < NW; ++j) if (WUG % 256 == 0 || tid + 256 * j < WUG) Wg[grp][tid + 256 * j] = rw[j]; }
#define CS_LSTOREX(buf_)                                                                         \
  {                                                                                              \
    _Pragma("unroll") for (int s = 0; s < NS; ++s) {                                             \
      const int pos = tid + 256 * s;                                                             \
      if (pos < NPOS) {                                                                          \
        float v[8];                                                                              \
        _Pragma("unroll") for (int c = 0; c < 8; ++c) v[c] = __uint_as_float(rx[s][c]);          \
        CS_NORM_PROBE_OPS()                                                                      \
        u32x4 sp[NSP];                                                                           \
        split8_s<NSP>(v, xscale, sp);                                                                      \
        _Pragma("unroll") for (int q = 0; q < NSP; ++q) Xs[buf_][(q * 2 + grp) * XP + pos] = sp[q]; \
      }                                                                                          \
    }                                                                                            \
  }

#ifdef CS_NORM_PROBE
  const float np_r = fmaf(oscale2, 0.f, 1.f), np_m = oscale2 * 0.f, np_lo = fmaf(oscale2, 0.f, -3.0e38f);
#define CS_NORM_PROBE_OPS() _Pragma("unroll") for (int c = 0; c < 8; ++c) v[c] = fmaxf(fmaf(v[c], np_r, np_m), np_lo);
#else
#define CS_NORM_PROBE_OPS()
#endif
  CS_GLOADX(0);
  if (grp == 0) CS_GLOADW(0);
  CS_LSTOREX(0);
  if (grp == 0) CS_LSTOREW();
  if (grp == 1) { CS_GLOADW(0); CS_GLOADX(1); }
  __syncthreads();
  WGT(1)

  for (int h = 0; h < 2 * chunks; ++h) {
    const int c = h >> 1;
    TRC(0)
    if ((h & 1) == grp) {
      __builtin_amdgcn_s_setprio(CS_COMPUTE_PRIO);
      const int qw_ = 2 * (c + 1), lw_ = chunks8 - qw_;
      const __amdgpu_buffer_rsrc_t rwd = __builtin_amdgcn_make_buffer_rsrc(
          const_cast<u32x4*>(ws + (long long)qw_ * wunits8), 0,
          lw_ > 0 ? (unsigned)((lw_ < 2 ? lw_ : 2) * wunits8) * 16u : 0u, 0x00020000);
      const int cx_ = 16 * (c + 1 + grp), lx_ = k.Cin - cx_;
      const __amdgpu_buffer_rsrc_t rxd = __builtin_amdgcn_make_buffer_rsrc(
          const_cast<float*>(xn + (long long)cx_ * HWi), 0,
          lx_ > 0 ? (unsigned)((lx_ < 16 ? lx_ : 16) * HWi) * 4u : 0u, 0x00020000);
      cs_mma_chunk_rr<CPG, XP, NW, NS>(Wg[grp], Xs[c & 1], abase, xb, acc, rwd, wb, rw, rxd, gvo, rx);
    } else {
      __builtin_amdgcn_s_setprio(CS_STORE_PRIO);
      {
#ifdef CS_TRACE
      __builtin_amdgcn_s_waitcnt(0x0f70);
      TRC(3)
#endif
#ifdef CS_TRACE
      CS_LSTOREW();
      TRC(4)
      if (c + 1 < chunks) CS_LSTOREX((c + 1) & 1);
#else
      if (grp == 0) {
        if (c + 1 < chunks) { CS_LSTOREW(); CS_LSTOREX((c + 1) & 1); }
      } else {
        CS_LSTOREW();
        if (c + 1 < chunks) CS_LSTOREX((c + 1) & 1);
      }
#endif
      }
    }
    TRC(1)
#ifndef CS_NO_EARLY_EPI
    if (h + 1 < 2 * chunks)
#endif
    __syncthreads();
    TRC(2)
  }
  WGT(2)
#ifdef CS_TRACE
  if (trace_blk) {
    __syncthreads();
    for (int i = threadIdx.x; i < 8 * 32 * 8; i += 512) g_cs_trace[i] = trc[i];
    if (threadIdx.x == 0) {
      const unsigned long long t1 = __builtin_readcyclecounter(), r1 = wall_clock64();
      g_cs_trace[2048] = (unsigned)trc_t0; g_cs_trace[2049] = (unsigned)t1;
      g_cs_trace[2050] = (unsigned)trc_r0; g_cs_trace[2051] = (unsigned)r1;
    }
  }
#endif
#undef CS_GLOADW
#undef CS_GLOADX
#undef CS_LSTOREW
#undef CS_LSTOREX
#undef CS_NORM_PROBE_OPS

  float* yb = y + (long long)n * k.Cout * HWo;
#pragma unroll
  for (int b = 0; b < 4; ++b) {
    const int i = CPG == 32 ? 0 : (wid & 1);
    const int row = 4 * rowgrp + b;
    const int oy = oy0 + row;
    const int cc = CPG * grp + i * 32 + l31, co = m0 + cc;
#ifdef CS_KO_EPI
    if (oy >= k.Ho || co >= k.Cout || acc[b][0] != 12345.678f) continue;
#else
    if (oy >= k.Ho || co >= k.Cout) continue;
#endif
    const float bv = bs[cc], osc = oscale * oscale2;
    const long long rowoff = (long long)co * HWo + (long long)oy * k.Wo;
    const float* rb = k.res ? k.res + (long long)n * k.Cout * HWo + rowoff : nullptr;
    const float* rg = k.ring ? k.ring + ((long long)n * 4 * k.Cout + co) * k.ring_rl : nullptr;
    const long long ss = (long long)k.Cout * k.ring_rl;
    const bool row_ring = rg != nullptr && (oy == 1 || oy == k.Ho - 2);
    float4 rv[4];
#pragma unroll
    for (int q = 0; q < 4; ++q) {
      rv[q] = make_float4(0.f, 0.f, 0.f, 0.f);
      const int ox = ox0 + 8 * q + 4 * lhi;
      if (rb && ox < k.Wo) {
        if (k.vec4) rv[q] = *reinterpret_cast<const float4*>(rb + ox);
        else {
          rv[q].x = rb[ox];
          if (ox + 1 < k.Wo) rv[q].y = rb[ox + 1];
          if (ox + 2 < k.Wo) rv[q].z = rb[ox + 2];
          if (ox + 3 < k.Wo) rv[q].w = rb[ox + 3];
        }
      }
    }
#pragma unroll
    for (int q = 0; q < 4; ++q) {
      const int ox = ox0 + 8 * q + 4 * lhi;
      if (ox >= k.Wo) continue;
      float v[4];
      const float r4[4] = {rv[q].x, rv[q].y, rv[q].z, rv[q].w};
#pragma unroll
      for (int e = 0; e < 4; ++e) {
        float t = acc[b][4 * q + e] * osc + bv;
        if (k.act == 1) t = t > 0.f ? t : t * k.slope;
        else if (k.act == 2) t = tanhf(t);
        v[e] = t + r4[e];
      }
      if (rg) {
#pragma unroll
        for (int e = 0; e < 4; ++e) {
          const int xx = ox + e;
          if (xx < k.Wo) {
            if (row_ring) {
              if (oy == 1) v[e] += rg[xx + 1] + (xx == 1 ? rg[0] : 0.f) + (xx == k.Wo - 2 ? rg[k.Wo + 1] : 0.f);
              if (oy == k.Ho - 2) v[e] += rg[ss + xx + 1] + (xx == 1 ? rg[ss] : 0.f) + (xx == k.Wo - 2 ? rg[ss + k.Wo + 1] : 0.f);
            }
            if (xx == 1) v[e] += rg[2 * ss + oy + 1];
            if (xx == k.Wo - 2) v[e] += rg[3 * ss + oy + 1];
          }
        }
      }
      float* yp = yb + rowoff + ox;
#ifdef CS_NT_STORE
      if (k.vec4) __builtin_nontemporal_store(f32x4{v[0], v[1], v[2], v[3]}, reinterpret_cast<f32x4*>(yp));
#else
      if (k.vec4) *reinterpret_cast<f32x4*>(yp) = f32x4{v[0], v[1], v[2], v[3]};
#endif
      else {
        yp[0] = v[0];
        if (ox + 1 < k.Wo) yp[1] = v[1];
        if (ox + 2 < k.Wo) yp[2] = v[2];
        if (ox + 3 < k.Wo) yp[3] = v[3];
      }
    }
  }
#ifdef CS_TRACE
  __builtin_amdgcn_s_waitcnt(0x0f70);
#endif
  WGT(3)
```

dfmir_amd/csrc/conv3x3s_w2_body.inc:

```
  constexpr int NSP = 2, BC = 128, CT = 64;
  using P = Prod<2>;
  constexpr int CTP = CT + W2_CTPAD;
  constexpr int XSLAB = 2 * CTP;
  constexpr int XCU = NSP * 3 * 4 * XSLAB, DYU = NSP * 2 * 2 * BC;
  static_assert(XCU == W2Lds::XCU && DYU == W2Lds::DYU, "arena layout");

  const int tid = threadIdx.x, lane = tid & 63;
  const int wid = __builtin_amdgcn_readfirstlane((int)(threadIdx.x >> 6));
  const bool want_db = k.db != nullptr && biy == 0;
  float bacc = 0.f, baccx = 0.f;
  const int wc = wid & 3, wi = wid >> 2;
  const int l31 = lane & 31, lhi = lane >> 5;
  const int HW = k.H * k.W;
  const int ci0 = biy * CT, co0 = biz * BC;
  const int run_beg = bix * k.runs_per_block;
  int run_end = run_beg + k.runs_per_block;
  if (run_end > k.runs_total) run_end = k.runs_total;

  const int ex = scale_exp(reduce_absmax(k.x_amax, k.x_n, red));
  __syncthreads();
  const int ed = scale_exp(reduce_absmax(k.dy_amax, k.dy_n, red));
  if (tid < BC) {
    int e = ed;
    if (k.dy_pmax) {
      float m = 0.f;
      if (co0 + tid < k.Cout)
        for (int n = 0; n < k.N; ++n) m = fmaxf(m, k.dy_pmax[(long long)n * k.Cout + co0 + tid]);
      e = scale_exp(m);
    }
    edc[tid] = e;
  }
  __syncthreads();

  const int xc = tid & 63, xu = (tid >> 6) & 1, xr = tid >> 7;
  const int dc = tid & (BC - 1), du = (tid >> 7) & 1, dk = tid >> 8;
  const bool xin = k.dbx != nullptr && biz == 0 && (xr == 1 || xr == 2);
  const float xscale = pow2f(ex), dscale = pow2f(edc[dc]), oscale = pow2f(-ex), oscale2 = pow2f(-edc[wc * 32 + l31]);
  const unsigned hw4 = (unsigned)HW * 4u;
  constexpr unsigned OOB = 0x80000000u;

  f32x16 acc[9];
#pragma unroll
  for (int t = 0; t < 9; ++t)
#pragma unroll
    for (int r = 0; r < 16; ++r) acc[t][r] = 0.f;

  u32x4 rxa, rxb, rda, rdb;
  unsigned rxl, rxr;

#ifndef W2_KO
#define W2_KO 0
#endif
#define W2_GLOAD(run_)                                                                           \
  if (!(W2_KO & 1) || k.N < 0) {                                                                 \
    const bool live_ = (run_) < run_end;                                                         \
    const int n_ = live_ ? (run_) / k.runs_per_img : 0;                                          \
    const int q_ = live_ ? (run_) - n_ * k.runs_per_img : 0;                                     \
    const int yp_ = q_ / k.runs_per_row, xs_ = q_ - yp_ * k.runs_per_row;                        \
    const int y0_ = 2 * yp_, x0_ = 16 * xs_ + 8 * xu;                                            \
    const __amdgpu_buffer_rsrc_t bx_ = __builtin_amdgcn_make_buffer_rsrc(                        \
        const_cast<float*>(x + (long long)n_ * k.Cin * HW), 0, live_ ? (unsigned)(k.Cin * HW) * 4u : 0u, 0x00020000); \
    const __amdgpu_buffer_rsrc_t bd_ = __builtin_amdgcn_make_buffer_rsrc(                        \
        const_cast<float*>(dy + (long long)n_ * k.Cout * HW), 0, live_ ? (unsigned)(k.Cout * HW) * 4u : 0u, 0x00020000); \
    const bool cok_ = ci0 + xc < k.Cin;                                                          \
    const unsigned cb_ = (unsigned)(ci0 + xc) * hw4;                                             \
    int ry_ = y0_ - 1 + xr;                                                                      \
    bool rok_ = (unsigned)ry_ < (unsigned)k.H;                                                   \
    if (k.pad_mode == 1) { ry_ = ry_ < 0 ? -ry_ : (ry_ >= k.H ? 2 * (k.H - 1) - ry_ : ry_); rok_ = true; } \
    const int rb_ = ry_ * k.W;                                                                   \
    const bool lin_ = x0_ > 0, rin_ = x0_ + 8 < k.W;                                             \
    const int ol_ = rb_ + (lin_ ? x0_ - 1 : 1), or_ = rb_ + (rin_ ? x0_ + 8 : k.W - 2);          \
    const bool lok_ = rok_ && cok_ && (lin_ || k.pad_mode == 1), rrok_ = rok_ && cok_ && (rin_ || k.pad_mode == 1); \
    const unsigned xb_ = (rok_ && cok_) ? cb_ + (unsigned)(rb_ + x0_) * 4u : OOB;                \
    rxa = __builtin_amdgcn_raw_buffer_load_b128(bx_, xb_, 0, 0);                                 \
    rxb = __builtin_amdgcn_raw_buffer_load_b128(bx_, xb_ == OOB ? OOB : xb_ + 16u, 0, 0);        \
    rxl = __builtin_amdgcn_raw_buffer_load_b32(bx_, lok_ ? cb_ + (unsigned)ol_ * 4u : OOB, 0, 0); \
    rxr = __builtin_amdgcn_raw_buffer_load_b32(bx_, rrok_ ? cb_ + (unsigned)or_ * 4u : OOB, 0, 0); \
    const unsigned db_ = (co0 + dc >= k.Cout) ? OOB                                              \
        : (unsigned)(co0 + dc) * hw4 + (unsigned)((y0_ + dk) * k.W + 16 * xs_ + 8 * du) * 4u;    \
    rda = __builtin_amdgcn_raw_buffer_load_b128(bd_, db_, 0, 0);                                 \
    rdb = __builtin_amdgcn_raw_buffer_load_b128(bd_, db_ == OOB ? OOB : db_ + 16u, 0, 0);        \
  }
#ifdef W2_NORM_PROBE
  const float np_r = fmaf(oscale, 0.f, 1.f), np_m = oscale * 0.f, np_lo = fmaf(oscale, 0.f, -3.0e38f);
#define W2_NORM_PROBE_OPS() _Pragma("unroll") for (int i = 0; i < 10; ++i) r[i] = fmaxf((r[i] - np_m) * np_r, np_lo);
#else
#define W2_NORM_PROBE_OPS()
#endif
#define W2_LSTORE(buf_)                                                                          \
  {                                                                                              \
    float r[10];                                                                                 \
    r[0] = __uint_as_float(rxl); r[9] = __uint_as_float(rxr);                                    \
    _Pragma("unroll") for (int e = 0; e < 4; ++e) { r[1 + e] = __uint_as_float(rxa[e]); r[5 + e] = __uint_as_float(rxb[e]); } \
    W2_NORM_PROBE_OPS()                                                                          \
    baccx += xin ? ((r[1] + r[2]) + (r[3] + r[4])) + ((r[5] + r[6]) + (r[7] + r[8])) : 0.f;      \
    unsigned pa[5][NSP], pb[4][NSP];                                                             \
    if (W2_KO & 4) { _Pragma("unroll") for (int i = 0; i < 5; ++i) { pa[i][0] = __float_as_uint(r[2 * i]); pa[i][1] = __float_as_uint(r[2 * i + 1]); } } \
    else _Pragma("unroll") for (int i = 0; i < 5; ++i) split_pair_scaled(r[2 * i], r[2 * i + 1], xscale, pa[i][0], pa[i][1]); \
    _Pragma("unroll") for (int i = 0; i < 4; ++i)                                                \
      _Pragma("unroll") for (int s = 0; s < NSP; ++s) pb[i][s] = __builtin_amdgcn_alignbit(pa[i + 1][s], pa[i][s], 16); \
    if (!(W2_KO & 2) || k.N < 0) _Pragma("unroll") for (int s = 0; s < NSP; ++s) {                 \
      u32x4* dst = Xc + (buf_) * XCU + (s * 3 * 4 + xr) * XSLAB + xu * CTP + xc;                    \
      dst[0] = u32x4{pa[0][s], pa[1][s], pa[2][s], pa[3][s]};                                    \
      dst[4 * XSLAB] = u32x4{pb[0][s], pb[1][s], pb[2][s], pb[3][s]};                            \
      dst[8 * XSLAB] = u32x4{pa[1][s], pa[2][s], pa[3][s], pa[4][s]};                            \
    }                                                                                            \
    float v[8];                                                                                  \
    _Pragma("unroll") for (int e = 0; e < 4; ++e) { v[e] = __uint_as_float(rda[e]); v[4 + e] = __uint_as_float(rdb[e]); } \
    bacc += ((v[0] + v[1]) + (v[2] + v[3])) + ((v[4] + v[5]) + (v[6] + v[7]));                   \
    u32x4 sp[NSP];                                                                               \
    if (W2_KO & 4) { sp[0] = rda; sp[1] = rdb; } else                                            \
    split8_s<NSP>(v, dscale, sp);                                                                \
    if (!(W2_KO & 2) || k.N < 0) _Pragma("unroll") for (int s = 0; s < NSP; ++s) Dy[(buf_) * DYU + ((s * 2 + dk) * 2 + du) * BC + dc] = sp[s]; \
  }

  const int abase = lhi * CTP + wi * 32 + l31;
  const int bbase = lhi * BC + wc * 32 + l31;
#ifndef W2_LEAD
#define W2_LEAD 1
#endif
#ifdef W2_NOPRIO
#define W2_PRIO(p_)
#else
#define W2_PRIO(p_) __builtin_amdgcn_s_setprio(p_)
#endif
#define W2_UDX(u_) ((u_) / 4)
#define W2_UROW(u_) ((u_) < 4 ? (u_) : ((u_) % 4 == 0 ? 1 : ((u_) % 4 == 1 ? 0 : (u_) % 4)))
#define W2_LOADA(set_, u_)                                                                       \
  _Pragma("unroll") for (int s = 0; s < NSP; ++s)                                                \
    a[set_][s] = Xb[((s * 3 + W2_UDX(u_)) * 4 + W2_UROW(u_)) * XSLAB + abase];
#define W2_MMA_PHASE(buf_)                                                                       \
  {                                                                                              \
    const u32x4* Xb = Xc + (buf_) * XCU;                                                         \
    const u32x4* Db = Dy + (buf_) * DYU;                                                         \
    u32x4 b[2][NSP], a[W2_LEAD + 1][NSP];                                                        \
    _Pragma("unroll") for (int s = 0; s < NSP; ++s) b[0][s] = Db[(s * 2 + 0) * 2 * BC + bbase];  \
    W2_LOADA(0, 0)                                                                               \
    _Pragma("unroll") for (int s = 0; s < NSP; ++s) b[1][s] = Db[(s * 2 + 1) * 2 * BC + bbase];  \
    if (W2_LEAD > 1) W2_LOADA(1, 1)                                                              \
    __builtin_amdgcn_sched_barrier(0);                                                           \
    _Pragma("unroll") for (int u = 0; u < 12; ++u) {                                             \
      if (u + W2_LEAD < 12) W2_LOADA((u + W2_LEAD) % (W2_LEAD + 1), u + W2_LEAD)                 \
      const int dx_ = W2_UDX(u), row_ = W2_UROW(u);                                              \
       \
      _Pragma("unroll") for (int qo = 0; qo < (W2_ALT ? P::N : 1); ++qo)                         \
      _Pragma("unroll") for (int ks = 0; ks < 2; ++ks) {                                         \
        const int ty_ = row_ - ks;                                                               \
        if (ty_ >= 0 && ty_ <= 2) {                                                              \
          _Pragma("unroll") for (int q = (W2_ALT ? qo : 0); q < (W2_ALT ? qo + 1 : P::N); ++q)   \
            acc[ty_ * 3 + dx_] = mma16<NSP>(a[u % (W2_LEAD + 1)][P::A[q]], b[ks][P::B[q]], acc[ty_ * 3 + dx_]); \
        }                                                                                        \
      }                                                                                          \
      const int nm_ = (row_ == 0 || row_ == 3) ? 3 : 6;                                          \
      _Pragma("unroll") for (int i = 0; i < 6; ++i) {                                            \
        if (i < nm_) __builtin_amdgcn_sched_group_barrier(0x008, 1, 0);                          \
        if (i < NSP && u + W2_LEAD < 12) __builtin_amdgcn_sched_group_barrier(0x100, 1, 0);      \
      }                                                                                          \
      __builtin_amdgcn_sched_barrier(0);                                                         \
    }                                                                                            \
  }

  if (run_beg < run_end) {
    W2_GLOAD(run_beg);
    W2_LSTORE(0);
    W2_GLOAD(run_beg + 1);
  }
  __syncthreads();

#ifdef W2_TRACE
  const bool trace_blk = bix == 5 && biy == 1 && biz == 0;
#endif
  if (wi == 0) {
    for (int run = run_beg; run < run_end; ++run) {
      const int buf = (run - run_beg) & 1;
      W2T(0)
      W2_PRIO(W2_PRIO_C);
      W2T_VM()
      W2_LSTORE(buf ^ 1);
      W2_GLOAD(run + 2);
      __builtin_amdgcn_sched_barrier(0);
      W2T(1)
      W2_PRIO(W2_PRIO_G0);
      if (!(W2_KO & 8) || k.N < 0) W2_MMA_PHASE(buf);
      W2T(2)
      __syncthreads();
      W2T(3)
    }
  } else {
    for (int run = run_beg; run < run_end; ++run) {
      const int buf = (run - run_beg) & 1;
      W2T(0)
      W2_PRIO(W2_PRIO_G1);
      if (!(W2_KO & 8) || k.N < 0) W2_MMA_PHASE(buf);
      __builtin_amdgcn_sched_barrier(0);
      W2T(1)
      W2_PRIO(W2_PRIO_C);
      W2T_VM()
      W2_LSTORE(buf ^ 1);
      W2_GLOAD(run + 2);
      W2T(2)
      __syncthreads();
      W2T(3)
    }
  }
#undef W2_GLOAD
#undef W2_LSTORE
#undef W2_LOADA
#undef W2_MMA_PHASE
#undef W2_UDX
#undef W2_UROW

  float* part = reinterpret_cast<float*>(Xc);
  if (want_db) {
    part[(tid >> 7) * BC + dc] = bacc;
    __syncthreads();
    if (tid < BC && co0 + tid < k.Cout)
      atomicAdd(&k.db[co0 + tid], (part[tid] + part[BC + tid]) + (part[2 * BC + tid] + part[3 * BC + tid]));
    __syncthreads();
  }
  if (k.dbx != nullptr && biz == 0) {
    part[(tid >> 6) * CT + xc] = baccx;
    __syncthreads();
    if (tid < CT && ci0 + tid < k.Cin) {
      float t = 0.f;
#pragma unroll
      for (int i = 0; i < 8; i += 2) t += part[i * CT + tid] + part[(i + 1) * CT + tid];
      atomicAdd(&k.dbx[ci0 + tid], t);
    }
  }
  if (k.swap) {
    __syncthreads();
    float* T = reinterpret_cast<float*>(Xc) + wid * (32 * 33);
#pragma unroll
    for (int t = 0; t < 9; ++t) {
#pragma unroll
      for (int r = 0; r < 16; ++r) T[(4 * lhi + (r & 3) + 8 * (r >> 2)) * 33 + l31] = acc[t][r] * oscale * oscale2;
      __syncthreads();
      const int ci = ci0 + wi * 32 + l31;
#pragma unroll
      for (int r = 0; r < 16; ++r) {
        const int col = 4 * lhi + (r & 3) + 8 * (r >> 2);
        const int co = co0 + wc * 32 + col;
        const float v = T[l31 * 33 + col];
        if (ci < k.Cin && co < k.Cout) df_acc(dwt, ((long long)(8 - t) * k.Cout + co) * k.Cin + ci, v, k.fx);
      }
      __syncthreads();
    }
    return;
  }
  const int co = co0 + wc * 32 + l31;
  if (co < k.Cout) {
#pragma unroll
    for (int t = 0; t < 9; ++t) {
#pragma unroll
      for (int r = 0; r < 16; ++r) {
        const int ci = ci0 + wi * 32 + 4 * lhi + (r & 3) + 8 * (r >> 2);
        if (ci < k.Cin) df_acc(dwt, ((long long)t * k.Cin + ci) * k.Cout + co, acc[t][r] * oscale * oscale2, k.fx);
      }
    }
  }
```

dfmir_amd/csrc/in_blurdown.hip:

```cpp
#include "common.h"

typedef unsigned irb_u32x4 __attribute__((ext_vector_type(4)));
typedef unsigned irb_u32x2 __attribute__((ext_vector_type(2)));
__device__ __forceinline__ float4 irb_ld4(__amdgpu_buffer_rsrc_t r, unsigned voff, unsigned soff) {
  const irb_u32x4 t = __builtin_amdgcn_raw_buffer_load_b128(r, voff, soff, 0);
  return make_float4(__uint_as_float(t.x), __uint_as_float(t.y), __uint_as_float(t.z), __uint_as_float(t.w));
}
__device__ __forceinline__ float2 irb_ld2(__amdgpu_buffer_rsrc_t r, unsigned voff, unsigned soff) {
  const irb_u32x2 t = __builtin_amdgcn_raw_buffer_load_b64(r, voff, soff, 0);
  return make_float2(__uint_as_float(t.x), __uint_as_float(t.y));
}
__device__ __forceinline__ void irb_st4(float4 v, __amdgpu_buffer_rsrc_t r, unsigned voff, unsigned soff) {
  irb_u32x4 t;
  t.x = __float_as_uint(v.x); t.y = __float_as_uint(v.y); t.z = __float_as_uint(v.z); t.w = __float_as_uint(v.w);
  __builtin_amdgcn_raw_buffer_store_b128(t, r, voff + soff, 0, 0);
}
__device__ __forceinline__ void irb_st2(float2 v, __amdgpu_buffer_rsrc_t r, unsigned voff, unsigned soff) {
  irb_u32x2 t;
  t.x = __float_as_uint(v.x); t.y = __float_as_uint(v.y);
  __builtin_amdgcn_raw_buffer_store_b64(t, r, voff, soff, 0);
}
__global__ __launch_bounds__(1024) void in_relu_blurdown_fwd256_k(const float* __restrict__ x, float* __restrict__ z,
                                                                  float* __restrict__ mean_o, float* __restrict__ rstd_o,
                                                                  float eps, float* __restrict__ amax) {
  constexpr int S = 65536;
  __shared__ float sm[17];
  __shared__ unsigned smax;
  __shared__ float edge[16][128];
  if (threadIdx.x == 0) smax = 0u;
  const int w = __builtin_amdgcn_readfirstlane((int)(threadIdx.x >> 6)), l = threadIdx.x & 63;
  const __amdgpu_buffer_rsrc_t xr = __builtin_amdgcn_make_buffer_rsrc(const_cast<float*>(x + (long long)blockIdx.x * S), 0,
                                                                       S * 4u, 0x00020000);
  const __amdgpu_buffer_rsrc_t zr = __builtin_amdgcn_make_buffer_rsrc(z + (long long)blockIdx.x * (S / 4), 0, S, 0x00020000);
  float4 v[16];
  float s = 0.f;
#pragma unroll
  for (int i = 0; i < 16; ++i) {
    v[i] = irb_ld4(xr, 16u * l, (unsigned)(16 * w + i) * 1024u);
    s += (v[i].x + v[i].y) + (v[i].z + v[i].w);
  }
  const float mean = block_sum(s, sm) / (float)S;
  float q = 0.f;
#pragma unroll
  for (int i = 0; i < 16; ++i) {
    const float a = v[i].x - mean, b = v[i].y - mean, c = v[i].z - mean, d = v[i].w - mean;
    q += (a * a + b * b) + (c * c + d * d);
  }
  const float var = block_sum(q, sm) / (float)S;
  const float rstd = 1.0f / sqrtf(var + eps);
  if (threadIdx.x == 0) {
    mean_o[blockIdx.x] = mean;
    rstd_o[blockIdx.x] = rstd;
  }
  float am = 0.f;
#pragma unroll
  for (int i = 0; i < 16; ++i) {
    const float ox = fmaxf((v[i].x - mean) * rstd, 0.f), oy = fmaxf((v[i].y - mean) * rstd, 0.f);
    const float oz = fmaxf((v[i].z - mean) * rstd, 0.f), ow = fmaxf((v[i].w - mean) * rstd, 0.f);
    am = fmaxf(fmaxf(am, fmaxf(ox, oy)), fmaxf(oz, ow));
    float left = __shfl_up(ow, 1, 64);
    if (l == 0) left = oy;
    v[i].x = 0.25f * left + 0.5f * ox + 0.25f * oy;
    v[i].y = 0.25f * oy + 0.5f * oz + 0.25f * ow;
  }
  *reinterpret_cast<float2*>(&edge[w][2 * l]) = make_float2(v[15].x, v[15].y);
  __syncthreads();
  const float2 up = w > 0 ? *reinterpret_cast<const float2*>(&edge[w - 1][2 * l]) : make_float2(v[1].x, v[1].y);
#pragma unroll
  for (int j = 0; j < 8; ++j) {
    const float a0 = j == 0 ? up.x : v[2 * j - 1].x, a1 = j == 0 ? up.y : v[2 * j - 1].y;
    float2 o;
    o.x = 0.25f * a0 + 0.5f * v[2 * j].x + 0.25f * v[2 * j + 1].x;
    o.y = 0.25f * a1 + 0.5f * v[2 * j].y + 0.25f * v[2 * j + 1].y;
    irb_st2(o, zr, 8u * l, (unsigned)(8 * w + j) * 512u);
  }
  if (amax) publish_block_absmax_acc(am, &smax, amax);
}

__global__ __launch_bounds__(1024) void in_relu_blurdown_bwd256_k(const float* __restrict__ dz, const float* __restrict__ x,
                                                                  const float* __restrict__ mean_i,
                                                                  const float* __restrict__ rstd_i, float* __restrict__ dx,
                                                                  float* __restrict__ amax, float* __restrict__ pmax) {
  constexpr int S = 65536;
  __shared__ float sm[17];
  __shared__ unsigned smax;
  __shared__ __attribute__((aligned(16))) float dzs[129 * 128];
  if (threadIdx.x == 0) smax = 0u;
  const int w = __builtin_amdgcn_readfirstlane((int)(threadIdx.x >> 6)), l = threadIdx.x & 63;
  const float mean = mean_i[blockIdx.x], rstd = rstd_i[blockIdx.x];
  const __amdgpu_buffer_rsrc_t xr = __builtin_amdgcn_make_buffer_rsrc(const_cast<float*>(x + (long long)blockIdx.x * S), 0,
                                                                       S * 4u, 0x00020000);
  const __amdgpu_buffer_rsrc_t zr = __builtin_amdgcn_make_buffer_rsrc(const_cast<float*>(dz + (long long)blockIdx.x * (S / 4)), 0,
                                                                       S, 0x00020000);
  const __amdgpu_buffer_rsrc_t dr = __builtin_amdgcn_make_buffer_rsrc(dx + (long long)blockIdx.x * S, 0, S * 4u, 0x00020000);
  float4 v[16];
#pragma unroll
  for (int i = 0; i < 16; ++i) v[i] = irb_ld4(xr, 16u * l, (unsigned)(16 * w + i) * 1024u);
#pragma unroll
  for (int q = 0; q < 4; ++q)
    *reinterpret_cast<float4*>(&dzs[4 * (threadIdx.x + 1024 * q)]) = irb_ld4(zr, 16u * (threadIdx.x + 1024 * q), 0u);
  if (threadIdx.x < 32) *reinterpret_cast<float4*>(&dzs[128 * 128 + 4 * threadIdx.x]) = make_float4(0.f, 0.f, 0.f, 0.f);
  __syncthreads();
  const float* dzw = dzs + (8 * w) * 128 + 2 * l;
#define IRB2_CA(k_, c_)                                                                           \
  {                                                                                               \
    const float2 d_ = *reinterpret_cast<const float2*>(dzw + (k_) * 128);                         \
    const float nx_ = l == 63 ? 0.f : dzw[(k_) * 128 + 2];                                        \
    c_.x = 0.5f * d_.x;                                                                           \
    c_.y = 0.25f * d_.x + 0.25f * d_.y + (l == 0 ? 0.25f * d_.x : 0.f);                           \
    c_.z = 0.5f * d_.y;                                                                           \
    c_.w = 0.25f * d_.y + 0.25f * nx_;                                                            \
  }
#define IRB2_ROW(i_, g_, BODY_)                                                                   \
  {                                                                                               \
    const float hx = (v[i_].x - MEAN_) * RSTD_, hy = (v[i_].y - MEAN_) * RSTD_, hz = (v[i_].z - MEAN_) * RSTD_, \
                hw = (v[i_].w - MEAN_) * RSTD_;                                                   \
    if (!(hx > 0.f)) g_.x = 0.f;                                                                  \
    if (!(hy > 0.f)) g_.y = 0.f;                                                                  \
    if (!(hz > 0.f)) g_.z = 0.f;                                                                  \
    if (!(hw > 0.f)) g_.w = 0.f;                                                                  \
    BODY_                                                                                         \
  }
#define IRB2_PASS(BODY_)                                                                          \
  {                                                                                               \
    float4 cur, nxt;                                                                              \
    IRB2_CA(0, cur)                                                                               \
    _Pragma("unroll") for (int j = 0; j < 8; ++j) {                                               \
      IRB2_CA(j + 1, nxt)                                                                         \
      const float e_ = (j == 0 && w == 0) ? 0.25f : 0.f;                                          \
      float4 g0, g1;                                                                              \
      g0.x = 0.5f * cur.x; g0.y = 0.5f * cur.y; g0.z = 0.5f * cur.z; g0.w = 0.5f * cur.w;          \
      g1.x = 0.25f * cur.x + 0.25f * nxt.x + e_ * cur.x;                                          \
      g1.y = 0.25f * cur.y + 0.25f * nxt.y + e_ * cur.y;                                          \
      g1.z = 0.25f * cur.z + 0.25f * nxt.z + e_ * cur.z;                                          \
      g1.w = 0.25f * cur.w + 0.25f * nxt.w + e_ * cur.w;                                          \
      { const int i = 2 * j; IRB2_ROW(i, g0, BODY_(g0)) }                                         \
      { const int i = 2 * j + 1; IRB2_ROW(i, g1, BODY_(g1)) }                                     \
      cur = nxt;                                                                                  \
    }                                                                                             \
  }
  float s1 = 0.f, s2 = 0.f;
#define MEAN_ mean
#define RSTD_ rstd
#define IRB2_SUMS(g_) s1 += (g_.x + g_.y) + (g_.z + g_.w); s2 += (g_.x * hx + g_.y * hy) + (g_.z * hz + g_.w * hw);
  IRB2_PASS(IRB2_SUMS)
  const float m1 = block_sum(s1, sm) / (float)S;
  const float m2 = block_sum(s2, sm) / (float)S;
  const float mean_b = mean, rstd_b = rstd;
  float am = 0.f;
#define IRB2_OUT(g_)                                                                              \
  {                                                                                               \
    float4 o;                                                                                     \
    o.x = rstd_b * (g_.x - m1 - hx * m2); o.y = rstd_b * (g_.y - m1 - hy * m2);                   \
    o.z = rstd_b * (g_.z - m1 - hz * m2); o.w = rstd_b * (g_.w - m1 - hw * m2);                   \
    irb_st4(o, dr, 16u * l, (unsigned)(16 * w + i) * 1024u);                                      \
    am = fmaxf(fmaxf(am, fmaxf(fabsf(o.x), fabsf(o.y))), fmaxf(fabsf(o.z), fabsf(o.w)));         \
  }
#undef MEAN_
#undef RSTD_
#define MEAN_ mean_b
#define RSTD_ rstd_b
  IRB2_PASS(IRB2_OUT)
#undef MEAN_
#undef RSTD_
#undef IRB2_OUT
#undef IRB2_SUMS
#undef IRB2_PASS
#undef IRB2_ROW
#undef IRB2_CA
  if (amax) publish_block_absmax_acc(am, &smax, amax);
  if (amax && pmax && threadIdx.x == 0) pmax[blockIdx.x] = __uint_as_float(smax);
}


__global__ __launch_bounds__(512) void in_relu_blurdown_fwd128_k(const float* __restrict__ x, float* __restrict__ z,
                                                                 float* __restrict__ mean_o, float* __restrict__ rstd_o,
                                                                 float eps, float* __restrict__ amax) {
  constexpr int S = 16384;
  __shared__ float sm[17];
  __shared__ unsigned smax;
  __shared__ float edge[8][64];
  if (threadIdx.x == 0) smax = 0u;
  const int w = __builtin_amdgcn_readfirstlane((int)(threadIdx.x >> 6)), l = threadIdx.x & 63;
  const __amdgpu_buffer_rsrc_t xr = __builtin_amdgcn_make_buffer_rsrc(const_cast<float*>(x + (long long)blockIdx.x * S), 0,
                                                                       S * 4u, 0x00020000);
  float2 v[16];
  float s = 0.f;
#pragma unroll
  for (int i = 0; i < 16; ++i) {
    v[i] = irb_ld2(xr, 8u * l, (unsigned)(16 * w + i) * 512u);
    s += v[i].x + v[i].y;
  }
  const float mean = block_sum(s, sm) / (float)S;
  float q = 0.f;
#pragma unroll
  for (int i = 0; i < 16; ++i) {
    const float a = v[i].x - mean, b = v[i].y - mean;
    q += a * a + b * b;
  }
  const float var = block_sum(q, sm) / (float)S;
  const float rstd = 1.0f / sqrtf(var + eps);
  if (threadIdx.x == 0) {
    mean_o[blockIdx.x] = mean;
    rstd_o[blockIdx.x] = rstd;
  }
  float h[16], am = 0.f;
#pragma unroll
  for (int i = 0; i < 16; ++i) {
    const float ox = fmaxf((v[i].x - mean) * rstd, 0.f), oy = fmaxf((v[i].y - mean) * rstd, 0.f);
    am = fmaxf(am, fmaxf(ox, oy));
    float left = __shfl_up(oy, 1, 64);
    if (l == 0) left = oy;
    h[i] = 0.25f * left + 0.5f * ox + 0.25f * oy;
  }
  edge[w][l] = h[15];
  __syncthreads();
  const float up = w > 0 ? edge[w - 1][l] : h[1];
  float* zp = z + (long long)blockIdx.x * (S / 4) + (8 * w) * 64 + l;
#pragma unroll
  for (int j = 0; j < 8; ++j) {
    const float a0 = j == 0 ? up : h[2 * j - 1];
    zp[j * 64] = 0.25f * a0 + 0.5f * h[2 * j] + 0.25f * h[2 * j + 1];
  }
  if (amax) publish_block_absmax_acc(am, &smax, amax);
}

__global__ __launch_bounds__(512) void in_relu_blurdown_bwd128_k(const float* __restrict__ dz, const float* __restrict__ x,
                                                                 const float* __restrict__ mean_i,
                                                                 const float* __restrict__ rstd_i, float* __restrict__ dx,
                                                                 float* __restrict__ amax, float* __restrict__ pmax) {
  constexpr int S = 16384;
  __shared__ float sm[17];
  __shared__ unsigned smax;
  __shared__ __attribute__((aligned(16))) float dzs[65 * 64 + 4];
  if (threadIdx.x == 0) smax = 0u;
  const int w = __builtin_amdgcn_readfirstlane((int)(threadIdx.x >> 6)), l = threadIdx.x & 63;
  const float mean = mean_i[blockIdx.x], rstd = rstd_i[blockIdx.x];
  const __amdgpu_buffer_rsrc_t xr = __builtin_amdgcn_make_buffer_rsrc(const_cast<float*>(x + (long long)blockIdx.x * S), 0,
                                                                       S * 4u, 0x00020000);
  const __amdgpu_buffer_rsrc_t zr = __builtin_amdgcn_make_buffer_rsrc(const_cast<float*>(dz + (long long)blockIdx.x * (S / 4)), 0,
                                                                       S, 0x00020000);
  const __amdgpu_buffer_rsrc_t dr = __builtin_amdgcn_make_buffer_rsrc(dx + (long long)blockIdx.x * S, 0, S * 4u, 0x00020000);
  float2 v[16];
#pragma unroll
  for (int i = 0; i < 16; ++i) v[i] = irb_ld2(xr, 8u * l, (unsigned)(16 * w + i) * 512u);
#pragma unroll
  for (int q = 0; q < 2; ++q)
    *reinterpret_cast<float4*>(&dzs[4 * (threadIdx.x + 512 * q)]) = irb_ld4(zr, 16u * (threadIdx.x + 512 * q), 0u);
  if (threadIdx.x < 17) *reinterpret_cast<float4*>(&dzs[64 * 64 + 4 * threadIdx.x]) = make_float4(0.f, 0.f, 0.f, 0.f);
  __syncthreads();
  const float* dzw = dzs + (8 * w) * 64 + l;
#define IRB1_CA(k_, c_)                                                                           \
  {                                                                                               \
    const float d_ = dzw[(k_) * 64];                                                              \
    const float nx_ = l == 63 ? 0.f : dzw[(k_) * 64 + 1];                                         \
    c_.x = 0.5f * d_;                                                                             \
    c_.y = 0.25f * d_ + 0.25f * nx_ + (l == 0 ? 0.25f * d_ : 0.f);                                \
  }
#define IRB1_ROW(i_, g_, BODY_)                                                                   \
  {                                                                                               \
    const float hx = (v[i_].x - mean) * rstd, hy = (v[i_].y - mean) * rstd;                       \
    if (!(hx > 0.f)) g_.x = 0.f;                                                                  \
    if (!(hy > 0.f)) g_.y = 0.f;                                                                  \
    BODY_                                                                                         \
  }
#define IRB1_PASS(BODY_)                                                                          \
  {                                                                                               \
    float2 cur, nxt;                                                                              \
    IRB1_CA(0, cur)                                                                               \
    _Pragma("unroll") for (int j = 0; j < 8; ++j) {                                               \
      IRB1_CA(j + 1, nxt)                                                                         \
      const float e_ = (j == 0 && w == 0) ? 0.25f : 0.f;                                          \
      float2 g0, g1;                                                                              \
      g0.x = 0.5f * cur.x; g0.y = 0.5f * cur.y;                                                   \
      g1.x = 0.25f * cur.x + 0.25f * nxt.x + e_ * cur.x;                                          \
      g1.y = 0.25f * cur.y + 0.25f * nxt.y + e_ * cur.y;                                          \
      { const int i = 2 * j; IRB1_ROW(i, g0, BODY_(g0)) }                                         \
      { const int i = 2 * j + 1; IRB1_ROW(i, g1, BODY_(g1)) }                                     \
      cur = nxt;                                                                                  \
    }                                                                                             \
  }
  float s1 = 0.f, s2 = 0.f;
#define IRB1_SUMS(g_) s1 += g_.x + g_.y; s2 += g_.x * hx + g_.y * hy;
  IRB1_PASS(IRB1_SUMS)
  const float m1 = block_sum(s1, sm) / (float)S;
  const float m2 = block_sum(s2, sm) / (float)S;
  float am = 0.f;
#define IRB1_OUT(g_)                                                                              \
  {                                                                                               \
    float2 o;                                                                                     \
    o.x = rstd * (g_.x - m1 - hx * m2); o.y = rstd * (g_.y - m1 - hy * m2);                       \
    irb_st2(o, dr, 8u * l, (unsigned)(16 * w + i) * 512u);                                        \
    am = fmaxf(am, fmaxf(fabsf(o.x), fabsf(o.y)));                                                \
  }
  IRB1_PASS(IRB1_OUT)
#undef IRB1_OUT
#undef IRB1_SUMS
#undef IRB1_PASS
#undef IRB1_ROW
#undef IRB1_CA
  if (amax) publish_block_absmax_acc(am, &smax, amax);
  if (amax && pmax && threadIdx.x == 0) pmax[blockIdx.x] = __uint_as_float(smax);
}

int df_in_relu_blurdown_fwd256_launch(const float* x, float* z, float* mean, float* rstd, int planes, float eps, float* z_amax,
                                      hipStream_t st, int W) {
  if (W == 128) in_relu_blurdown_fwd128_k<<<planes, 512, 0, st>>>(x, z, mean, rstd, eps, z_amax);
  else in_relu_blurdown_fwd256_k<<<planes, 1024, 0, st>>>(x, z, mean, rstd, eps, z_amax);
  DF_LAUNCH_CHECK();
  return 0;
}
int df_in_relu_blurdown_bwd256_launch(const float* dz, const float* x, const float* mean, const float* rstd, float* dx,
                                      int planes, float* dx_amax, float* dx_pmax, hipStream_t st, int W) {
  if (W == 128) in_relu_blurdown_bwd128_k<<<planes, 512, 0, st>>>(dz, x, mean, rstd, dx, dx_amax, dx_pmax);
  else in_relu_blurdown_bwd256_k<<<planes, 1024, 0, st>>>(dz, x, mean, rstd, dx, dx_amax, dx_pmax);
  DF_LAUNCH_CHECK();
  return 0;
}
```

dfmir_amd/csrc/norm_resample.hip:

```cpp
#include "common.h"

__global__ __launch_bounds__(256) void instnorm_fwd_k(const float* __restrict__ x,
                                                      const float* __restrict__ res,
                                                      float* __restrict__ y, float* __restrict__ mean_o,
                                                      float* __restrict__ rstd_o, long long S,
                                                      float eps, int relu) {
  __shared__ float sm[17];
  const long long base = (long long)blockIdx.x * S;
  const float* xp = x + base;
  const bool vec = (S & 3) == 0;
  float s = 0.f;
  if (vec) {
    const float4* x4 = reinterpret_cast<const float4*>(xp);
    for (long long i = threadIdx.x; i < (S >> 2); i += 256) {
      const float4 v = x4[i];
      s += (v.x + v.y) + (v.z + v.w);
    }
  } else {
    for (long long i = threadIdx.x; i < S; i += 256) s += xp[i];
  }
  const float mean = block_sum(s, sm) / (float)S;
  float q = 0.f;
  if (vec) {
    const float4* x4 = reinterpret_cast<const float4*>(xp);
    for (long long i = threadIdx.x; i < (S >> 2); i += 256) {
      const float4 v = x4[i];
      const float a = v.x - mean, b = v.y - mean, c = v.z - mean, d = v.w - mean;
      q += (a * a + b * b) + (c * c + d * d);
    }
  } else {
    for (long long i = threadIdx.x; i < S; i += 256) {
      const float a = xp[i] - mean;
      q += a * a;
    }
  }
  const float var = block_sum(q, sm) / (float)S;
  const float rstd = 1.0f / sqrtf(var + eps);
  if (threadIdx.x == 0) {
    mean_o[blockIdx.x] = mean;
    rstd_o[blockIdx.x] = rstd;
  }
  float* yp = y + base;
  const float* rp = res ? res + base : nullptr;
  if (vec) {
    const float4* x4 = reinterpret_cast<const float4*>(xp);
    const float4* r4 = reinterpret_cast<const float4*>(rp);
    float4* y4 = reinterpret_cast<float4*>(yp);
    for (long long i = threadIdx.x; i < (S >> 2); i += 256) {
      float4 v = x4[i];
      v.x = (v.x - mean) * rstd; v.y = (v.y - mean) * rstd;
      v.z = (v.z - mean) * rstd; v.w = (v.w - mean) * rstd;
      if (relu) {
        v.x = fmaxf(v.x, 0.f); v.y = fmaxf(v.y, 0.f); v.z = fmaxf(v.z, 0.f); v.w = fmaxf(v.w, 0.f);
      }
      if (rp) {
        const float4 r = r4[i];
        v.x += r.x; v.y += r.y; v.z += r.z; v.w += r.w;
      }
      y4[i] = v;
    }
  } else {
    for (long long i = threadIdx.x; i < S; i += 256) {
      float v = (xp[i] - mean) * rstd;
      if (relu) v = fmaxf(v, 0.f);
      if (rp) v += rp[i];
      yp[i] = v;
    }
  }
}

template <int NT, int E>
__global__ __launch_bounds__(NT) void instnorm_fwd_reg_k(const float* __restrict__ x,
                                                         const float* __restrict__ res,
                                                         float* __restrict__ y, float* __restrict__ mean_o,
                                                         float* __restrict__ rstd_o, float eps, int relu,
                                                         float* __restrict__ amax) {
  __shared__ float sm[17];
  __shared__ unsigned smax;
  if (threadIdx.x == 0) smax = 0u;
  constexpr long long S = (long long)NT * 4 * E;
  const long long base = (long long)blockIdx.x * S;
  const float4* x4 = reinterpret_cast<const float4*>(x + base);
  float4 v[E];
  float s = 0.f;
#pragma unroll
  for (int i = 0; i < E; ++i) {
    v[i] = x4[threadIdx.x + NT * i];
    s += (v[i].x + v[i].y) + (v[i].z + v[i].w);
  }
  const float mean = block_sum(s, sm) / (float)S;
  float q = 0.f;
#pragma unroll
  for (int i = 0; i < E; ++i) {
    const float a = v[i].x - mean, b = v[i].y - mean, c = v[i].z - mean, d = v[i].w - mean;
    q += (a * a + b * b) + (c * c + d * d);
  }
  const float var = block_sum(q, sm) / (float)S;
  const float rstd = 1.0f / sqrtf(var + eps);
  if (threadIdx.x == 0) {
    mean_o[blockIdx.x] = mean;
    rstd_o[blockIdx.x] = rstd;
  }
  const float4* r4 = res ? reinterpret_cast<const float4*>(res + base) : nullptr;
  float4* y4 = reinterpret_cast<float4*>(y + base);
  float am = 0.f;
#pragma unroll
  for (int i = 0; i < E; ++i) {
    float4 o;
    o.x = (v[i].x - mean) * rstd; o.y = (v[i].y - mean) * rstd;
    o.z = (v[i].z - mean) * rstd; o.w = (v[i].w - mean) * rstd;
    if (relu) {
      o.x = fmaxf(o.x, 0.f); o.y = fmaxf(o.y, 0.f); o.z = fmaxf(o.z, 0.f); o.w = fmaxf(o.w, 0.f);
    }
    if (r4) {
      const float4 r = r4[threadIdx.x + NT * i];
      o.x += r.x; o.y += r.y; o.z += r.z; o.w += r.w;
    }
    if (y) y4[threadIdx.x + NT * i] = o;
    am = fmaxf(fmaxf(am, fmaxf(fabsf(o.x), fabsf(o.y))), fmaxf(fabsf(o.z), fabsf(o.w)));
  }
  if (amax) publish_block_absmax_acc(am, &smax, amax);
}
template <int NT, int E, bool COLS>
__global__ __launch_bounds__(NT) void instnorm_bwd_reg_k(const float* __restrict__ dy,
                                                         const float* __restrict__ x,
                                                         const float* __restrict__ mean_i,
                                                         const float* __restrict__ rstd_i,
                                                         float* __restrict__ dx, int relu,
                                                         float* __restrict__ amax, float* __restrict__ cols, int W,
                                                         float* __restrict__ pmax) {
  __shared__ float sm[17];
  __shared__ unsigned smax;
  if (threadIdx.x == 0) smax = 0u;
  constexpr long long S = (long long)NT * 4 * E;
  const long long base = (long long)blockIdx.x * S;
  const float mean = mean_i[blockIdx.x], rstd = rstd_i[blockIdx.x];
  const float4* x4 = reinterpret_cast<const float4*>(x + base);
  const float4* g4 = reinterpret_cast<const float4*>(dy + base);
  float4 xh[E], g[E];
  float s1 = 0.f, s2 = 0.f;
#pragma unroll
  for (int i = 0; i < E; ++i) {
    const float4 xv = x4[threadIdx.x + NT * i];
    float4 gi = g4[threadIdx.x + NT * i];
    xh[i].x = (xv.x - mean) * rstd; xh[i].y = (xv.y - mean) * rstd;
    xh[i].z = (xv.z - mean) * rstd; xh[i].w = (xv.w - mean) * rstd;
    if (relu) {
      if (!(xh[i].x > 0.f)) gi.x = 0.f;
      if (!(xh[i].y > 0.f)) gi.y = 0.f;
      if (!(xh[i].z > 0.f)) gi.z = 0.f;
      if (!(xh[i].w > 0.f)) gi.w = 0.f;
    }
    s1 += (gi.x + gi.y) + (gi.z + gi.w);
    s2 += (gi.x * xh[i].x + gi.y * xh[i].y) + (gi.z * xh[i].z + gi.w * xh[i].w);
    g[i] = gi;
  }
  const float m1 = block_sum(s1, sm) / (float)S;
  const float m2 = block_sum(s2, sm) / (float)S;
  float4* d4 = reinterpret_cast<float4*>(dx + base);
  float am = 0.f;
#pragma unroll
  for (int i = 0; i < E; ++i) {
    const float4 gi = g[i];
    float4 o;
    o.x = rstd * (gi.x - m1 - xh[i].x * m2); o.y = rstd * (gi.y - m1 - xh[i].y * m2);
    o.z = rstd * (gi.z - m1 - xh[i].z * m2); o.w = rstd * (gi.w - m1 - xh[i].w * m2);
    d4[threadIdx.x + NT * i] = o;
    am = fmaxf(fmaxf(am, fmaxf(fabsf(o.x), fabsf(o.y))), fmaxf(fabsf(o.z), fabsf(o.w)));
    if (COLS && cols) {
      const int e0 = 4 * (threadIdx.x + NT * i), H = (int)(S / W);
      float* cp = cols + (long long)blockIdx.x * 2 * H;
      if (e0 % W == 0) cp[e0 / W] = o.x;
      if ((e0 + 3) % W == W - 1) cp[H + (e0 + 3) / W] = o.w;
    }
  }
  if (amax) publish_block_absmax_acc(am, &smax, amax);
  if (amax && pmax && threadIdx.x == 0) pmax[blockIdx.x] = __uint_as_float(smax);
}

__global__ __launch_bounds__(256) void instnorm_bwd_k(const float* __restrict__ dy,
                                                      const float* __restrict__ x,
                                                      const float* __restrict__ mean_i,
                                                      const float* __restrict__ rstd_i,
                                                      float* __restrict__ dx, long long S, int relu) {
  __shared__ float sm[17];
  const long long base = (long long)blockIdx.x * S;
  const float mean = mean_i[blockIdx.x], rstd = rstd_i[blockIdx.x];
  const float* xp = x + base;
  const float* gp = dy + base;
  float* dp = dx + base;
  float s1 = 0.f, s2 = 0.f;
  if ((S & 3) == 0) {
    const float4* x4 = reinterpret_cast<const float4*>(xp);
    const float4* g4 = reinterpret_cast<const float4*>(gp);
    float4* d4 = reinterpret_cast<float4*>(dp);
    const long long S4 = S >> 2;
    for (long long i = threadIdx.x; i < S4; i += 256) {
      const float4 xv = x4[i];
      float4 g = g4[i];
      const float a = (xv.x - mean) * rstd, b = (xv.y - mean) * rstd, c = (xv.z - mean) * rstd, d = (xv.w - mean) * rstd;
      if (relu) {
        if (!(a > 0.f)) g.x = 0.f;
        if (!(b > 0.f)) g.y = 0.f;
        if (!(c > 0.f)) g.z = 0.f;
        if (!(d > 0.f)) g.w = 0.f;
      }
      s1 += (g.x + g.y) + (g.z + g.w);
      s2 += (g.x * a + g.y * b) + (g.z * c + g.w * d);
    }
    const float m1 = block_sum(s1, sm) / (float)S;
    const float m2 = block_sum(s2, sm) / (float)S;
    for (long long i = threadIdx.x; i < S4; i += 256) {
      const float4 xv = x4[i];
      float4 g = g4[i];
      const float a = (xv.x - mean) * rstd, b = (xv.y - mean) * rstd, c = (xv.z - mean) * rstd, d = (xv.w - mean) * rstd;
      if (relu) {
        if (!(a > 0.f)) g.x = 0.f;
        if (!(b > 0.f)) g.y = 0.f;
        if (!(c > 0.f)) g.z = 0.f;
        if (!(d > 0.f)) g.w = 0.f;
      }
      float4 o;
      o.x = rstd * (g.x - m1 - a * m2); o.y = rstd * (g.y - m1 - b * m2);
      o.z = rstd * (g.z - m1 - c * m2); o.w = rstd * (g.w - m1 - d * m2);
      d4[i] = o;
    }
    return;
  }
  for (long long i = threadIdx.x; i < S; i += 256) {
    const float xh = (xp[i] - mean) * rstd;
    float g = gp[i];
    if (relu && !(xh > 0.f)) g = 0.f;
    s1 += g;
    s2 += g * xh;
  }
  const float m1 = block_sum(s1, sm) / (float)S;
  const float m2 = block_sum(s2, sm) / (float)S;
  for (long long i = threadIdx.x; i < S; i += 256) {
    const float xh = (xp[i] - mean) * rstd;
    float g = gp[i];
    if (relu && !(xh > 0.f)) g = 0.f;
    dp[i] = rstd * (g - m1 - xh * m2);
  }
}

__global__ void act_bwd_k(const float* __restrict__ dy, const float* __restrict__ y,
                          float* __restrict__ dx, long long n, int act, float slope) {
  for (long long i = (long long)blockIdx.x * blockDim.x + threadIdx.x; i < n;
       i += (long long)gridDim.x * blockDim.x) {
    const float yv = y[i], g = dy[i];
    dx[i] = (act == 2) ? g * (1.f - yv * yv) : (yv > 0.f ? g : g * slope);
  }
}
__global__ __launch_bounds__(256) void act_bwd_v4_k(const float4* __restrict__ dy, const float4* __restrict__ y,
                                                    float4* __restrict__ dx, long long n4, int act, float slope) {
  for (long long i = (long long)blockIdx.x * 256 + threadIdx.x; i < n4; i += (long long)gridDim.x * 256) {
    const float4 yv = y[i], g = dy[i];
    float4 o;
    o.x = (act == 2) ? g.x * (1.f - yv.x * yv.x) : (yv.x > 0.f ? g.x : g.x * slope);
    o.y = (act == 2) ? g.y * (1.f - yv.y * yv.y) : (yv.y > 0.f ? g.y : g.y * slope);
    o.z = (act == 2) ? g.z * (1.f - yv.z * yv.z) : (yv.z > 0.f ? g.z : g.z * slope);
    o.w = (act == 2) ? g.w * (1.f - yv.w * yv.w) : (yv.w > 0.f ? g.w : g.w * slope);
    dx[i] = o;
  }
}

__global__ __launch_bounds__(256) void act_bwd_amax_k(const float* __restrict__ dy, const float* __restrict__ y,
                                                      float* __restrict__ dx, long long n, int act, float slope,
                                                      float* __restrict__ amax) {
  __shared__ unsigned smax;
  if (threadIdx.x == 0) smax = 0u;
  __syncthreads();
  const long long n4 = n >> 2;
  float m = 0.f;
  for (long long i = (long long)blockIdx.x * 256 + threadIdx.x; i < n4; i += (long long)gridDim.x * 256) {
    const float4 yv = reinterpret_cast<const float4*>(y)[i], g = reinterpret_cast<const float4*>(dy)[i];
    float4 o;
    o.x = (act == 2) ? g.x * (1.f - yv.x * yv.x) : (yv.x > 0.f ? g.x : g.x * slope);
    o.y = (act == 2) ? g.y * (1.f - yv.y * yv.y) : (yv.y > 0.f ? g.y : g.y * slope);
    o.z = (act == 2) ? g.z * (1.f - yv.z * yv.z) : (yv.z > 0.f ? g.z : g.z * slope);
    o.w = (act == 2) ? g.w * (1.f - yv.w * yv.w) : (yv.w > 0.f ? g.w : g.w * slope);
    reinterpret_cast<float4*>(dx)[i] = o;
    m = fmaxf(fmaxf(m, fmaxf(fabsf(o.x), fabsf(o.y))), fmaxf(fabsf(o.z), fabsf(o.w)));
  }
  if (blockIdx.x == 0 && threadIdx.x < (n & 3)) {
    const long long i = (n4 << 2) + threadIdx.x;
    const float yv = y[i], g = dy[i];
    const float o = (act == 2) ? g * (1.f - yv * yv) : (yv > 0.f ? g : g * slope);
    dx[i] = o;
    m = fmaxf(m, fabsf(o));
  }
  publish_block_absmax_acc(m, &smax, amax);
}

__device__ __forceinline__ int refl1(int c, int n) {
  if (c < 0) c = -c;
  if (c >= n) c = 2 * (n - 1) - c;
  return c < 0 ? 0 : c;
}
__global__ void blur_down_fwd_k(const float* __restrict__ x, float* __restrict__ y, int planes, int H,
                                int W, int Ho, int Wo) {
  const long long total = (long long)planes * Ho * Wo;
  const float f[3] = {0.25f, 0.5f, 0.25f};
  for (long long i = (long long)blockIdx.x * blockDim.x + threadIdx.x; i < total;
       i += (long long)gridDim.x * blockDim.x) {
    const int ox = (int)(i % Wo);
    long long r = i / Wo;
    const int oy = (int)(r % Ho);
    const long long pl = r / Ho;
    const float* xp = x + pl * H * W;
    float s = 0.f;
#pragma unroll
    for (int a = 0; a < 3; ++a) {
      const int iy = refl1(2 * oy + a - 1, H);
      float rs = 0.f;
#pragma unroll
      for (int b = 0; b < 3; ++b) rs += f[b] * xp[(long long)iy * W + refl1(2 * ox + b - 1, W)];
      s += f[a] * rs;
    }
    y[i] = s;
  }
}
__device__ __forceinline__ void blur_down_adj(int i, int n, int no, int (&o)[3], float (&w)[3]) {
  if ((i & 1) == 0) {
    o[0] = i >> 1; w[0] = 0.5f;
    o[1] = 0; w[1] = 0.f;
  } else {
    o[0] = (i - 1) >> 1; w[0] = 0.25f;
    const int o1 = (i + 1) >> 1;
    o[1] = o1 < no ? o1 : 0; w[1] = o1 < no ? 0.25f : 0.f;
  }
  o[2] = 0; w[2] = 0.f;
  if (i == 1) { o[2] = 0; w[2] = 0.25f; }
  if (i == n - 2 && (n & 1)) {
    if (i == 1) {
      o[0] = 0; w[0] = 0.5f; o[1] = 1; w[1] = 0.5f; o[2] = 0; w[2] = 0.f;
    } else {
      o[2] = (n - 1) >> 1; w[2] = 0.25f;
    }
  }
}
__global__ void blur_down_bwd_k(const float* __restrict__ dy, float* __restrict__ dx, int planes, int H,
                                int W, int Ho, int Wo) {
  const long long total = (long long)planes * H * W;
  for (long long i = (long long)blockIdx.x * blockDim.x + threadIdx.x; i < total;
       i += (long long)gridDim.x * blockDim.x) {
    const int ix = (int)(i % W);
    long long r = i / W;
    const int iy = (int)(r % H);
    const long long pl = r / H;
    const float* gp = dy + pl * Ho * Wo;
    int oy[3], oxx[3];
    float wy[3], wx[3];
    blur_down_adj(iy, H, Ho, oy, wy);
    blur_down_adj(ix, W, Wo, oxx, wx);
    float s = 0.f;
#pragma unroll
    for (int a = 0; a < 3; ++a) {
      const float* row = gp + (long long)oy[a] * Wo;
      s += wy[a] * (wx[0] * row[oxx[0]] + wx[1] * row[oxx[1]] + wx[2] * row[oxx[2]]);
    }
    dx[i] = s;
  }
}

int df_in_relu_blurdown_fwd256_launch(const float* x, float* z, float* mean, float* rstd, int planes, float eps, float* z_amax,
                                      hipStream_t st, int W);
int df_in_relu_blurdown_bwd256_launch(const float* dz, const float* x, const float* mean, const float* rstd, float* dx,
                                      int planes, float* dx_amax, float* dx_pmax, hipStream_t st, int W);

__device__ __forceinline__ void blur_up_src(int o, int L, int& i0, int& i1) {
  const int m = o >> 1;
  i0 = m;
  i1 = (o & 1) ? (m + 1 < L ? m + 1 : L - 1) : (m > 0 ? m - 1 : 0);
}
__global__ void blur_up_fwd_k(const float* __restrict__ x, float* __restrict__ y, int planes, int H,
                              int W) {
  const int Ho = 2 * H, Wo = 2 * W;
  const long long total = (long long)planes * Ho * Wo;
  for (long long i = (long long)blockIdx.x * blockDim.x + threadIdx.x; i < total;
       i += (long long)gridDim.x * blockDim.x) {
    const int ox = (int)(i % Wo);
    long long r = i / Wo;
    const int oy = (int)(r % Ho);
    const long long pl = r / Ho;
    const float* xp = x + pl * H * W;
    int y0, y1, x0, x1;
    blur_up_src(oy, H, y0, y1);
    blur_up_src(ox, W, x0, x1);
    const float r0 = 0.75f * xp[(long long)y0 * W + x0] + 0.25f * xp[(long long)y0 * W + x1];
    const float r1 = 0.75f * xp[(long long)y1 * W + x0] + 0.25f * xp[(long long)y1 * W + x1];
    y[i] = 0.75f * r0 + 0.25f * r1;
  }
}
__device__ __forceinline__ int blur_up_adj(int m, int L, int* oo, float* ww) {
  int cnt = 0;
  oo[cnt] = 2 * m; ww[cnt++] = 0.75f;
  oo[cnt] = 2 * m + 1; ww[cnt++] = 0.75f;
  if (m + 1 <= L - 1) { oo[cnt] = 2 * m + 2; ww[cnt++] = 0.25f; }
  if (m == 0) { oo[cnt] = 0; ww[cnt++] = 0.25f; }
  if (m >= 1) { oo[cnt] = 2 * m - 1; ww[cnt++] = 0.25f; }
  if (m == L - 1) { oo[cnt] = 2 * L - 1; ww[cnt++] = 0.25f; }
  return cnt;
}
__global__ void blur_up_bwd_k(const float* __restrict__ dy, float* __restrict__ dx, int planes, int H,
                              int W) {
  const int Ho = 2 * H, Wo = 2 * W;
  const long long total = (long long)planes * H * W;
  for (long long i = (long long)blockIdx.x * blockDim.x + threadIdx.x; i < total;
       i += (long long)gridDim.x * blockDim.x) {
    const int ix = (int)(i % W);
    long long r = i / W;
    const int iy = (int)(r % H);
    const long long pl = r / H;
    const float* gp = dy + pl * Ho * Wo;
    int oy[6], oxx[6];
    float wy[6], wx[6];
    const int ny = blur_up_adj(iy, H, oy, wy);
    const int nx = blur_up_adj(ix, W, oxx, wx);
    float s = 0.f;
    for (int a = 0; a < ny; ++a) {
      float rs = 0.f;
      for (int b = 0; b < nx; ++b) rs += wx[b] * gp[(long long)oy[a] * Wo + oxx[b]];
      s += wy[a] * rs;
    }
    dx[i] = s;
  }
}

__global__ __launch_bounds__(256) void blur_down_fwd_v4_k(const float* __restrict__ x, float* __restrict__ y,
                                                          int H, int W) {
  const int Ho = H >> 1, Wo = W >> 1, G = Wo >> 2;
  const int i = blockIdx.x * 256 + threadIdx.x;
  if (i >= Ho * G) return;
  const int oy = i / G, ox = (i - oy * G) << 2;
  const float* xp = x + (long long)blockIdx.y * H * W;
  float h[3][4];
#pragma unroll
  for (int a = 0; a < 3; ++a) {
    const int iy = refl1(2 * oy + a - 1, H);
    const float* row = xp + iy * W + 2 * ox;
    const float4 v0 = *reinterpret_cast<const float4*>(row), v1 = *reinterpret_cast<const float4*>(row + 4);
    const float l = ox ? row[-1] : row[1];
    const float v[9] = {l, v0.x, v0.y, v0.z, v0.w, v1.x, v1.y, v1.z, v1.w};
#pragma unroll
    for (int j = 0; j < 4; ++j) {
      float rs = 0.f;
      rs += 0.25f * v[2 * j]; rs += 0.5f * v[2 * j + 1]; rs += 0.25f * v[2 * j + 2];
      h[a][j] = rs;
    }
  }
  float o[4];
#pragma unroll
  for (int j = 0; j < 4; ++j) {
    float t = 0.f;
    t += 0.25f * h[0][j]; t += 0.5f * h[1][j]; t += 0.25f * h[2][j];
    o[j] = t;
  }
  *reinterpret_cast<float4*>(y + ((long long)blockIdx.y * Ho + oy) * Wo + ox) = make_float4(o[0], o[1], o[2], o[3]);
}
__global__ __launch_bounds__(256) void blur_down_bwd_v4_k(const float* __restrict__ dy, float* __restrict__ dx,
                                                          int H, int W) {
  const int Ho = H >> 1, Wo = W >> 1, G = W >> 2;
  const int i = blockIdx.x * 256 + threadIdx.x;
  if (i >= H * G) return;
  const int iy = i / G, ix = (i - iy * G) << 2;
  const float* gp = dy + (long long)blockIdx.y * Ho * Wo;
  int oy[3]; float wy[3];
  blur_down_adj(iy, H, Ho, oy, wy);
  const int c = ix >> 1;
  const bool c2 = c + 2 < Wo;
  float s[4] = {0.f, 0.f, 0.f, 0.f};
#pragma unroll
  for (int a = 0; a < 3; ++a) {
    if (wy[a] == 0.f) continue;
    const float* row = gp + oy[a] * Wo + c;
    const float g0 = row[0], g1 = row[1], g2 = c2 ? row[2] : 0.f;
    const float r0 = 0.5f * g0;
    const float r1 = 0.25f * g0 + 0.25f * g1 + (ix == 0 ? 0.25f * g0 : 0.f);
    const float r2 = 0.5f * g1;
    const float r3 = 0.25f * g1 + 0.25f * g2;
    s[0] += wy[a] * r0; s[1] += wy[a] * r1; s[2] += wy[a] * r2; s[3] += wy[a] * r3;
  }
  *reinterpret_cast<float4*>(dx + ((long long)blockIdx.y * H + iy) * W + ix) = make_float4(s[0], s[1], s[2], s[3]);
}
__global__ __launch_bounds__(256) void blur_up_fwd_v4_k(const float* __restrict__ x, float* __restrict__ y,
                                                        int H, int W) {
  const int G = W >> 1, Wo = 2 * W, lane = threadIdx.x & 63;
  const int i = blockIdx.x * 256 + threadIdx.x;
  if (i >= H * G) return;
  const int iy = i / G, ix = (i - iy * G) << 1;
  const float* xp = x + (long long)blockIdx.y * H * W;
  float v[3][4];
#pragma unroll
  for (int a = 0; a < 3; ++a) {
    int r = iy + a - 1;
    r = r < 0 ? 0 : (r > H - 1 ? H - 1 : r);
    const float* row = xp + r * W + ix;
    const float2 q = *reinterpret_cast<const float2*>(row);
    const float lft = __shfl_up(q.y, 1, 64), rgt = __shfl_down(q.x, 1, 64);
    v[a][0] = ix ? (lane ? lft : row[-1]) : q.x;
    v[a][1] = q.x; v[a][2] = q.y;
    v[a][3] = (ix + 2 < W) ? (lane < 63 ? rgt : row[2]) : q.y;
  }
  float* yp = y + ((long long)blockIdx.y * 2 * H + 2 * iy) * Wo + 2 * ix;
#pragma unroll
  for (int p = 0; p < 2; ++p) {
    const int nb = p ? 2 : 0;
    float o[4];
#pragma unroll
    for (int j = 0; j < 2; ++j) {
#pragma unroll
      for (int q = 0; q < 2; ++q) {
        const int xn = q ? j + 2 : j;
        const float r0 = 0.75f * v[1][j + 1] + 0.25f * v[1][xn];
        const float r1 = 0.75f * v[nb][j + 1] + 0.25f * v[nb][xn];
        o[2 * j + q] = 0.75f * r0 + 0.25f * r1;
      }
    }
    *reinterpret_cast<float4*>(yp + p * Wo) = make_float4(o[0], o[1], o[2], o[3]);
  }
}
__global__ __launch_bounds__(256) void blur_up_bwd_v4_k(const float* __restrict__ dy, float* __restrict__ dx,
                                                        int H, int W) {
  const int G = W >> 2, Wo = 2 * W, Ho = 2 * H, lane = threadIdx.x & 63;
  const int i = blockIdx.x * 256 + threadIdx.x;
  if (i >= H * G) return;
  const int iy = i / G, ix = (i - iy * G) << 2;
  const float* gp = dy + (long long)blockIdx.y * Ho * Wo;
  const float w4[4] = {0.25f, 0.75f, 0.75f, 0.25f};
  float s[4] = {0.f, 0.f, 0.f, 0.f};
#pragma unroll
  for (int a = 0; a < 4; ++a) {
    int r = 2 * iy - 1 + a;
    r = r < 0 ? 0 : (r > Ho - 1 ? Ho - 1 : r);
    const float* row = gp + r * Wo + 2 * ix;
    const float4 q0 = *reinterpret_cast<const float4*>(row), q1 = *reinterpret_cast<const float4*>(row + 4);
    const float lft = __shfl_up(q1.w, 1, 64), rgt = __shfl_down(q0.x, 1, 64);
    const float l = ix ? (lane ? lft : row[-1]) : q0.x, rr = (2 * ix + 8 < Wo) ? (lane < 63 ? rgt : row[8]) : q1.w;
    const float v[10] = {l, q0.x, q0.y, q0.z, q0.w, q1.x, q1.y, q1.z, q1.w, rr};
#pragma unroll
    for (int j = 0; j < 4; ++j) {
      const float hs = 0.25f * v[2 * j] + 0.75f * v[2 * j + 1] + 0.75f * v[2 * j + 2] + 0.25f * v[2 * j + 3];
      s[j] += w4[a] * hs;
    }
  }
  *reinterpret_cast<float4*>(dx + ((long long)blockIdx.y * H + iy) * W + ix) = make_float4(s[0], s[1], s[2], s[3]);
}

__global__ void reflect_pad2d_fwd_k(const float* __restrict__ x, float* __restrict__ y, int planes,
                                    int H, int W, int p) {
  const int Ho = H + 2 * p, Wo = W + 2 * p;
  const long long total = (long long)planes * Ho * Wo;
  for (long long i = (long long)blockIdx.x * blockDim.x + threadIdx.x; i < total;
       i += (long long)gridDim.x * blockDim.x) {
    const int ox = (int)(i % Wo);
    long long r = i / Wo;
    const int oy = (int)(r % Ho);
    const long long pl = r / Ho;
    y[i] = x[pl * H * W + (long long)refl1(oy - p, H) * W + refl1(ox - p, W)];
  }
}
__device__ __forceinline__ int reflect_adj(int i, int n, int p, int* qq) {
  int cnt = 0;
  qq[cnt++] = i + p;
  if (i >= 1 && i <= p) qq[cnt++] = p - i;
  if (i <= n - 2 && i >= n - 1 - p) qq[cnt++] = p + 2 * (n - 1) - i;
  return cnt;
}
__global__ void reflect_pad2d_bwd_k(const float* __restrict__ dy, const float* __restrict__ add,
                                    float* __restrict__ dx, int planes, int H, int W, int p) {
  const int Ho = H + 2 * p, Wo = W + 2 * p;
  const long long total = (long long)planes * H * W;
  for (long long i = (long long)blockIdx.x * blockDim.x + threadIdx.x; i < total;
       i += (long long)gridDim.x * blockDim.x) {
    const int ix = (int)(i % W);
    long long r = i / W;
    const int iy = (int)(r % H);
    const long long pl = r / H;
    const float* gp = dy + pl * Ho * Wo;
    int qy[3], qx[3];
    const int ny = reflect_adj(iy, H, p, qy);
    const int nx = reflect_adj(ix, W, p, qx);
    float s = 0.f;
    for (int a = 0; a < ny; ++a)
      for (int b = 0; b < nx; ++b) s += gp[(long long)qy[a] * Wo + qx[b]];
    dx[i] = add ? s + add[i] : s;
  }
}

__global__ __launch_bounds__(256) void reflect_pad1_bwd_v4_k(const float* __restrict__ dy, const float* __restrict__ add,
                                                             float* __restrict__ dx, int H, int W) {
  typedef unsigned rp_u32x4 __attribute__((ext_vector_type(4)));
  const int G = W >> 2, Wo = W + 2;
  const int i = blockIdx.x * 256 + threadIdx.x;
  if (i >= H * G) return;
  const int y = i / G, x0 = (i - y * G) << 2;
  const float* gp = dy + (long long)blockIdx.y * (H + 2) * Wo;
  const __amdgpu_buffer_rsrc_t rs = __builtin_amdgcn_make_buffer_rsrc(const_cast<float*>(gp), 0,
                                                                      (unsigned)((H + 2) * Wo) * 4u, 0x00020000);
  int rows[2] = {y + 1, y + 1};
  int nr = 1;
  if (y == 1) { rows[1] = 0; nr = 2; }
  else if (y == H - 2) { rows[1] = H + 1; nr = 2; }
  float s[4] = {0.f, 0.f, 0.f, 0.f};
  for (int a = 0; a < nr; ++a) {
    const int rb = rows[a] * Wo;
    const rp_u32x4 v = __builtin_amdgcn_raw_buffer_load_b128(rs, (unsigned)(rb + x0 + 1) * 4u, 0, 0);
    s[0] += __uint_as_float(v[0]); s[1] += __uint_as_float(v[1]);
    s[2] += __uint_as_float(v[2]); s[3] += __uint_as_float(v[3]);
    if (x0 == 0) s[1] += gp[rb];
    if (x0 == W - 4) s[2] += gp[rb + W + 1];
  }
  const long long o = ((long long)blockIdx.y * H + y) * W + x0;
  if (add) {
    const float4 r = *reinterpret_cast<const float4*>(add + o);
    s[0] += r.x; s[1] += r.y; s[2] += r.z; s[3] += r.w;
  }
  *reinterpret_cast<float4*>(dx + o) = make_float4(s[0], s[1], s[2], s[3]);
}

__global__ void upcat_fwd_k(const float* __restrict__ a, const float* __restrict__ b,
                            float* __restrict__ y, int N, int Ca, int Cb, int Da, int Ha, int Wa, int sd) {
  const int Do = Da * sd, Ho = Ha * 2, Wo = Wa * 2, C = Ca + Cb;
  const long long So = (long long)Do * Ho * Wo, Sa = (long long)Da * Ha * Wa;
  const long long total = (long long)N * C * So;
  for (long long i = (long long)blockIdx.x * blockDim.x + threadIdx.x; i < total;
       i += (long long)gridDim.x * blockDim.x) {
    const int x = (int)(i % Wo);
    long long r = i / Wo;
    const int yy = (int)(r % Ho); r /= Ho;
    const int z = (int)(r % Do); r /= Do;
    const int c = (int)(r % C);
    const long long n = r / C;
    float v;
    if (c < Ca) v = a[(n * Ca + c) * Sa + ((long long)(z / sd) * Ha + (yy >> 1)) * Wa + (x >> 1)];
    else v = b[(n * Cb + (c - Ca)) * So + ((long long)z * Ho + yy) * Wo + x];
    y[i] = v;
  }
}
template <typename IDX>
__global__ __launch_bounds__(256) void upcat_fwd_v4_k(const float* __restrict__ a, const float* __restrict__ b,
                                                      float* __restrict__ y, int N, int Ca, int Cb, int Da, int Ha,
                                                      int Wa, int sd) {
  const int Do = Da * sd, Ho = Ha * 2, Wo = Wa * 2, C = Ca + Cb, Wq = Wo >> 2;
  const long long So = (long long)Do * Ho * Wo, Sa = (long long)Da * Ha * Wa;
  const IDX total = (IDX)((long long)N * C * Do * Ho * Wq);
  for (IDX i = (IDX)blockIdx.x * 256 + threadIdx.x; i < total; i += (IDX)gridDim.x * 256) {
    const int xq = (int)(i % (IDX)Wq);
    IDX r = i / (IDX)Wq;
    const int yy = (int)(r % (IDX)Ho); r /= (IDX)Ho;
    const int z = (int)(r % (IDX)Do); r /= (IDX)Do;
    const int c = (int)(r % (IDX)C);
    const long long n = (long long)(r / (IDX)C);
    float4 v;
    if (c < Ca) {
      const float2 t = *reinterpret_cast<const float2*>(a + (n * Ca + c) * Sa + ((long long)(z / sd) * Ha + (yy >> 1)) * Wa + 2 * xq);
      v = make_float4(t.x, t.x, t.y, t.y);
    } else {
      v = *reinterpret_cast<const float4*>(b + (n * Cb + (c - Ca)) * So + ((long long)z * Ho + yy) * Wo + 4 * xq);
    }
    *reinterpret_cast<float4*>(y + ((n * C + c) * Do + z) * (long long)Ho * Wo + (long long)yy * Wo + 4 * xq) = v;
  }
}
template <typename IDX, bool V2>
__global__ __launch_bounds__(256) void upcat_bwd_a_k(const float* __restrict__ dy, float* __restrict__ da, int N, int Ca, int Cb,
                                                     int Da, int Ha, int Wa, int sd) {
  const int Do = Da * sd, Ho = Ha * 2, Wo = Wa * 2, C = Ca + Cb, Wh = V2 ? (Wa >> 1) : Wa;
  const long long So = (long long)Do * Ho * Wo;
  const IDX total = (IDX)((long long)N * Ca * Da * Ha * Wh);
  for (IDX i = (IDX)blockIdx.x * 256 + threadIdx.x; i < total; i += (IDX)gridDim.x * 256) {
    const int x = (int)(i % (IDX)Wh);
    IDX r = i / (IDX)Wh;
    const int yy = (int)(r % (IDX)Ha); r /= (IDX)Ha;
    const int z = (int)(r % (IDX)Da); r /= (IDX)Da;
    const int c = (int)(r % (IDX)Ca);
    const long long n = (long long)(r / (IDX)Ca);
    const float* gp = dy + (n * C + c) * So;
    float s0 = 0.f, s1 = 0.f;
    for (int dz = 0; dz < sd; ++dz)
#pragma unroll
      for (int dyy = 0; dyy < 2; ++dyy) {
        const float* row = gp + ((long long)(z * sd + dz) * Ho + (2 * yy + dyy)) * Wo;
        if (V2) {
          const float4 t = *reinterpret_cast<const float4*>(row + 4 * x);
          s0 += t.x + t.y; s1 += t.z + t.w;
        } else {
          s0 += row[2 * x] + row[2 * x + 1];
        }
      }
    float* o = da + (((n * Ca + c) * Da + z) * (long long)Ha + yy) * Wa;
    if (V2) *reinterpret_cast<float2*>(o + 2 * x) = make_float2(s0, s1);
    else o[x] = s0;
  }
}
template <typename IDX, int V>
__global__ __launch_bounds__(256) void cat_channels_k(const float* __restrict__ a, const float* __restrict__ b, float* __restrict__ y,
                                                      long long N, long long SA, long long SB, int dir) {
  typedef float vec_t __attribute__((ext_vector_type(V)));
  const IDX ST = (IDX)(SA + SB), total = (IDX)(N * (SA + SB));
  const vec_t* av = reinterpret_cast<const vec_t*>(a);
  const vec_t* bv = reinterpret_cast<const vec_t*>(b);
  vec_t* yv = reinterpret_cast<vec_t*>(y);
  vec_t* aw = const_cast<vec_t*>(av);
  vec_t* bw = const_cast<vec_t*>(bv);
  for (IDX i = (IDX)blockIdx.x * 256 + threadIdx.x; i < total; i += (IDX)gridDim.x * 256) {
    const IDX n = i / ST, r = i - n * ST;
    if (dir == 0) yv[i] = r < (IDX)SA ? av[(long long)n * SA + r] : bv[(long long)n * SB + (r - (IDX)SA)];
    else if (r < (IDX)SA) { if (aw) aw[(long long)n * SA + r] = yv[i]; }
    else { if (bw) bw[(long long)n * SB + (r - (IDX)SA)] = yv[i]; }
  }
}
static void cat_channels_launch(const float* a, const float* b, float* y, long long N, long long SA, long long SB, int dir,
                                hipStream_t st) {
  const bool v4 = ((SA | SB) & 3) == 0 &&
                  ((reinterpret_cast<uintptr_t>(a) | reinterpret_cast<uintptr_t>(b) | reinterpret_cast<uintptr_t>(y)) & 15) == 0;
  const long long V = v4 ? 4 : 1, total = N * (SA + SB) / V;
  const unsigned grid = df_grid(total, 256, 16384);
  const bool small = total < 0x7FFFFFFFLL;
  if (v4) {
    if (small) cat_channels_k<unsigned, 4><<<grid, 256, 0, st>>>(a, b, y, N, SA / 4, SB / 4, dir);
    else cat_channels_k<long long, 4><<<grid, 256, 0, st>>>(a, b, y, N, SA / 4, SB / 4, dir);
  } else {
    if (small) cat_channels_k<unsigned, 1><<<grid, 256, 0, st>>>(a, b, y, N, SA, SB, dir);
    else cat_channels_k<long long, 1><<<grid, 256, 0, st>>>(a, b, y, N, SA, SB, dir);
  }
}
__global__ void scale_k(const float* __restrict__ x, float* __restrict__ y, long long n, float mult) {
  for (long long i = (long long)blockIdx.x * blockDim.x + threadIdx.x; i < n;
       i += (long long)gridDim.x * blockDim.x)
    y[i] = mult * x[i];
}

int df_absmax_launch(const float* x, long long n, float* out, hipStream_t st, bool zero_first);
extern "C" int dfmir_instnorm_stats_ok(long long S) { return (S == 4096 || S == 16384 || S == 65536) ? 1 : 0; }
extern "C" int dfmir_instnorm_stats(const float* x, float* mean, float* rstd, int planes, long long S, float eps, int relu,
                                    float* y_amax, void* stream) {
  DF_ARG_CHECK(x && mean && rstd && planes > 0 && dfmir_instnorm_stats_ok(S));
  hipStream_t st = (hipStream_t)stream;
  if (S == 4096) instnorm_fwd_reg_k<256, 4><<<planes, 256, 0, st>>>(x, nullptr, nullptr, mean, rstd, eps, relu, y_amax);
  else if (S == 16384) instnorm_fwd_reg_k<256, 16><<<planes, 256, 0, st>>>(x, nullptr, nullptr, mean, rstd, eps, relu, y_amax);
  else instnorm_fwd_reg_k<1024, 16><<<planes, 1024, 0, st>>>(x, nullptr, nullptr, mean, rstd, eps, relu, y_amax);
  DF_LAUNCH_CHECK();
  return 0;
}
extern "C" int dfmir_instnorm_fwd(const float* x, const float* res, float* y, float* mean, float* rstd,
                                  int planes, long long S, float eps, int relu, float* y_amax, void* stream) {
  DF_ARG_CHECK(x && y && mean && rstd && planes > 0 && S > 0);
  hipStream_t st = (hipStream_t)stream;
  if (S == 4096) instnorm_fwd_reg_k<256, 4><<<planes, 256, 0, st>>>(x, res, y, mean, rstd, eps, relu, y_amax);
  else if (S == 16384) instnorm_fwd_reg_k<256, 16><<<planes, 256, 0, st>>>(x, res, y, mean, rstd, eps, relu, y_amax);
  else if (S == 65536) instnorm_fwd_reg_k<1024, 16><<<planes, 1024, 0, st>>>(x, res, y, mean, rstd, eps, relu, y_amax);
  else {
    instnorm_fwd_k<<<planes, 256, 0, st>>>(x, res, y, mean, rstd, S, eps, relu);
    if (y_amax) {
      DF_LAUNCH_CHECK();
      const int rc = df_absmax_launch(y, (long long)planes * S, y_amax, st, false);
      if (rc) return df_set_error(rc, __FILE__, __LINE__);
    }
  }
  DF_LAUNCH_CHECK();
  return 0;
}
extern "C" int dfmir_instnorm_bwd_cols_ok(long long S, int W) {
  return ((S == 4096 || S == 16384) && W >= 4 && (W & 3) == 0 && S % W == 0) ? 1 : 0;
}
static int instnorm_bwd_impl(const float* dy, const float* x, const float* mean, const float* rstd, float* dx,
                             int planes, long long S, int relu, float* dx_amax, float* dx_cols, int W, void* stream,
                             float* dx_pmax = nullptr);
extern "C" int dfmir_instnorm_bwd_pmax_ok(long long S) { return (S == 4096 || S == 16384 || S == 65536) ? 1 : 0; }
extern "C" int dfmir_instnorm_bwd_pmax(const float* dy, const float* x, const float* mean, const float* rstd, float* dx,
                                       int planes, long long S, int relu, float* dx_amax, float* dx_cols, int W,
                                       float* dx_pmax, void* stream) {
  DF_ARG_CHECK(dx_amax && dx_pmax && dfmir_instnorm_bwd_pmax_ok(S) && (!dx_cols || dfmir_instnorm_bwd_cols_ok(S, W)));
  return instnorm_bwd_impl(dy, x, mean, rstd, dx, planes, S, relu, dx_amax, dx_cols, W, stream, dx_pmax);
}
extern "C" int dfmir_instnorm_bwd(const float* dy, const float* x, const float* mean, const float* rstd,
                                  float* dx, int planes, long long S, int relu, float* dx_amax, void* stream) {
  return instnorm_bwd_impl(dy, x, mean, rstd, dx, planes, S, relu, dx_amax, nullptr, 0, stream);
}
extern "C" int dfmir_instnorm_bwd_cols(const float* dy, const float* x, const float* mean, const float* rstd,
                                       float* dx, int planes, long long S, int relu, float* dx_amax, float* dx_cols,
                                       int W, void* stream) {
  DF_ARG_CHECK(dx_cols && dfmir_instnorm_bwd_cols_ok(S, W));
  return instnorm_bwd_impl(dy, x, mean, rstd, dx, planes, S, relu, dx_amax, dx_cols, W, stream);
}
static int instnorm_bwd_impl(const float* dy, const float* x, const float* mean, const float* rstd, float* dx,
                             int planes, long long S, int relu, float* dx_amax, float* dx_cols, int W, void* stream,
                             float* dx_pmax) {
  DF_ARG_CHECK(dy && x && mean && rstd && dx && planes > 0 && S > 0);
  hipStream_t st = (hipStream_t)stream;
  if (S == 4096 && dx_cols) instnorm_bwd_reg_k<256, 4, true><<<planes, 256, 0, st>>>(dy, x, mean, rstd, dx, relu, dx_amax, dx_cols, W, dx_pmax);
  else if (S == 4096) instnorm_bwd_reg_k<256, 4, false><<<planes, 256, 0, st>>>(dy, x, mean, rstd, dx, relu, dx_amax, nullptr, 0, dx_pmax);
  else if (S == 16384 && dx_cols) instnorm_bwd_reg_k<256, 16, true><<<planes, 256, 0, st>>>(dy, x, mean, rstd, dx, relu, dx_amax, dx_cols, W, dx_pmax);
  else if (S == 16384) instnorm_bwd_reg_k<256, 16, false><<<planes, 256, 0, st>>>(dy, x, mean, rstd, dx, relu, dx_amax, nullptr, 0, dx_pmax);
  else if (S == 65536 && dx_cols) return df_set_error(-1, __FILE__, __LINE__);
  else if (S == 65536) instnorm_bwd_reg_k<1024, 16, false><<<planes, 1024, 0, st>>>(dy, x, mean, rstd, dx, relu, dx_amax, nullptr, 0, dx_pmax);
  else {
    instnorm_bwd_k<<<planes, 256, 0, st>>>(dy, x, mean, rstd, dx, S, relu);
    if (dx_amax) {
      DF_LAUNCH_CHECK();
      const int rc = df_absmax_launch(dx, (long long)planes * S, dx_amax, st, false);
      if (rc) return df_set_error(rc, __FILE__, __LINE__);
    }
  }
  DF_LAUNCH_CHECK();
  return 0;
}
extern "C" int dfmir_in_relu_blurdown_ok(int H, int W) {
  return ((H == 256 && W == 256) || (H == 128 && W == 128)) ? 1 : 0;
}
extern "C" int dfmir_in_relu_blurdown_fwd(const float* x, float* z, float* mean, float* rstd, int planes, int H, int W,
                                          float eps, float* z_amax, void* stream) {
  DF_ARG_CHECK(x && z && mean && rstd && planes > 0 && dfmir_in_relu_blurdown_ok(H, W));
  return df_in_relu_blurdown_fwd256_launch(x, z, mean, rstd, planes, eps, z_amax, (hipStream_t)stream, W);
}
extern "C" int dfmir_in_relu_blurdown_bwd(const float* dz, const float* x, const float* mean, const float* rstd, float* dx,
                                          int planes, int H, int W, float* dx_amax, float* dx_pmax, void* stream) {
  DF_ARG_CHECK(dz && x && mean && rstd && dx && planes > 0 && dfmir_in_relu_blurdown_ok(H, W));
  return df_in_relu_blurdown_bwd256_launch(dz, x, mean, rstd, dx, planes, dx_amax, dx_pmax, (hipStream_t)stream, W);
}
extern "C" int dfmir_act_bwd(const float* dy, const float* y, float* dx, long long n, int act,
                             float slope, void* stream) {
  DF_ARG_CHECK(dy && y && dx && n > 0 && (act == 1 || act == 2));
  if ((n & 3) == 0 && ((reinterpret_cast<uintptr_t>(dy) | reinterpret_cast<uintptr_t>(y) | reinterpret_cast<uintptr_t>(dx)) & 15) == 0)
    act_bwd_v4_k<<<df_grid(n / 4, 256, 8192), 256, 0, (hipStream_t)stream>>>(
        reinterpret_cast<const float4*>(dy), reinterpret_cast<const float4*>(y), reinterpret_cast<float4*>(dx), n / 4, act, slope);
  else
    act_bwd_k<<<df_grid(n, 256, 4096), 256, 0, (hipStream_t)stream>>>(dy, y, dx, n, act, slope);
  DF_LAUNCH_CHECK();
  return 0;
}
extern "C" int dfmir_act_bwd_amax(const float* dy, const float* y, float* dx, long long n, int act, float slope,
                                  float* dx_amax, void* stream) {
  DF_ARG_CHECK(dy && y && dx && dx_amax && n > 0 && (act == 1 || act == 2));
  DF_ARG_CHECK(((reinterpret_cast<uintptr_t>(dy) | reinterpret_cast<uintptr_t>(y) | reinterpret_cast<uintptr_t>(dx)) & 15) == 0);
  act_bwd_amax_k<<<df_grid((n + 3) / 4, 256, 4096), 256, 0, (hipStream_t)stream>>>(dy, y, dx, n, act, slope, dx_amax);
  DF_LAUNCH_CHECK();
  return 0;
}
extern "C" int dfmir_blur_down_fwd(const float* x, float* y, int planes, int H, int W, void* stream) {
  DF_ARG_CHECK(x && y && planes > 0 && H > 1 && W > 1);
  const int Ho = (H - 1) / 2 + 1, Wo = (W - 1) / 2 + 1;
  if ((H & 1) == 0 && (W & 7) == 0 && planes <= 65535 && (long long)H * W < (1LL << 30)) {
    blur_down_fwd_v4_k<<<dim3((unsigned)(((H / 2) * (W / 8) + 255) / 256), (unsigned)planes), 256, 0,
                         (hipStream_t)stream>>>(x, y, H, W);
    DF_LAUNCH_CHECK();
    return 0;
  }
  blur_down_fwd_k<<<df_grid((long long)planes * Ho * Wo, 256, 8192), 256, 0, (hipStream_t)stream>>>(
      x, y, planes, H, W, Ho, Wo);
  DF_LAUNCH_CHECK();
  return 0;
}
extern "C" int dfmir_blur_down_bwd(const float* dy, float* dx, int planes, int H, int W, void* stream) {
  DF_ARG_CHECK(dy && dx && planes > 0 && H > 1 && W > 1);
  const int Ho = (H - 1) / 2 + 1, Wo = (W - 1) / 2 + 1;
  if ((H & 1) == 0 && (W & 3) == 0 && H >= 4 && W >= 4 && planes <= 65535 && (long long)H * W < (1LL << 30)) {
    blur_down_bwd_v4_k<<<dim3((unsigned)((H * (W / 4) + 255) / 256), (unsigned)planes), 256, 0,
                         (hipStream_t)stream>>>(dy, dx, H, W);
    DF_LAUNCH_CHECK();
    return 0;
  }
  blur_down_bwd_k<<<df_grid((long long)planes * H * W, 256, 8192), 256, 0, (hipStream_t)stream>>>(
      dy, dx, planes, H, W, Ho, Wo);
  DF_LAUNCH_CHECK();
  return 0;
}
extern "C" int dfmir_blur_up_fwd(const float* x, float* y, int planes, int H, int W, void* stream) {
  DF_ARG_CHECK(x && y && planes > 0 && H > 0 && W > 0);
  if ((W & 1) == 0 && planes <= 65535 && (long long)H * W < (1LL << 28)) {
    blur_up_fwd_v4_k<<<dim3((unsigned)((H * (W / 2) + 255) / 256), (unsigned)planes), 256, 0,
                       (hipStream_t)stream>>>(x, y, H, W);
    DF_LAUNCH_CHECK();
    return 0;
  }
  blur_up_fwd_k<<<df_grid((long long)planes * H * W * 4, 256, 8192), 256, 0, (hipStream_t)stream>>>(
      x, y, planes, H, W);
  DF_LAUNCH_CHECK();
  return 0;
}
extern "C" int dfmir_blur_up_bwd(const float* dy, float* dx, int planes, int H, int W, void* stream) {
  DF_ARG_CHECK(dy && dx && planes > 0 && H > 0 && W > 0);
  if ((W & 3) == 0 && planes <= 65535 && (long long)H * W < (1LL << 28)) {
    blur_up_bwd_v4_k<<<dim3((unsigned)((H * (W / 4) + 255) / 256), (unsigned)planes), 256, 0,
                       (hipStream_t)stream>>>(dy, dx, H, W);
    DF_LAUNCH_CHECK();
    return 0;
  }
  blur_up_bwd_k<<<df_grid((long long)planes * H * W, 256, 8192), 256, 0, (hipStream_t)stream>>>(
      dy, dx, planes, H, W);
  DF_LAUNCH_CHECK();
  return 0;
}
extern "C" int dfmir_reflect_pad2d_fwd(const float* x, float* y, int planes, int H, int W, int p,
                                       void* stream) {
  DF_ARG_CHECK(x && y && planes > 0 && p >= 0 && p < H && p < W);
  reflect_pad2d_fwd_k<<<df_grid((long long)planes * (H + 2 * p) * (W + 2 * p), 256, 8192), 256, 0,
                        (hipStream_t)stream>>>(x, y, planes, H, W, p);
  DF_LAUNCH_CHECK();
  return 0;
}
static int reflect_pad2d_bwd_impl(const float* dy, const float* add, float* dx, int planes, int H, int W, int p,
                                  void* stream) {
  DF_ARG_CHECK(dy && dx && planes > 0 && p >= 0 && p < H && p < W);
  if (p == 1 && (W & 3) == 0 && H >= 8 && W >= 8 && planes <= 65535 && (long long)(H + 2) * (W + 2) < (1LL << 29)) {
    reflect_pad1_bwd_v4_k<<<dim3((unsigned)((H * (W / 4) + 255) / 256), (unsigned)planes), 256, 0,
                            (hipStream_t)stream>>>(dy, add, dx, H, W);
    DF_LAUNCH_CHECK();
    return 0;
  }
  reflect_pad2d_bwd_k<<<df_grid((long long)planes * H * W, 256, 8192), 256, 0, (hipStream_t)stream>>>(
      dy, add, dx, planes, H, W, p);
  DF_LAUNCH_CHECK();
  return 0;
}
extern "C" int dfmir_reflect_pad2d_bwd(const float* dy, float* dx, int planes, int H, int W, int p,
                                       void* stream) {
  return reflect_pad2d_bwd_impl(dy, nullptr, dx, planes, H, W, p, stream);
}
extern "C" int dfmir_reflect_pad2d_bwd_add(const float* dy, const float* add, float* dx, int planes, int H, int W,
                                           int p, void* stream) {
  DF_ARG_CHECK(add != nullptr);
  return reflect_pad2d_bwd_impl(dy, add, dx, planes, H, W, p, stream);
}
extern "C" int dfmir_upcat_fwd(const float* a, const float* b, float* y, int N, int Ca, int Cb, int Da,
                               int Ha, int Wa, int sd, void* stream) {
  DF_ARG_CHECK(a && b && y && N > 0 && Ca > 0 && Cb > 0 && (sd == 1 || sd == 2));
  const long long total = (long long)N * (Ca + Cb) * Da * sd * Ha * 2 * Wa * 2;
  if ((Wa & 1) == 0 && ((reinterpret_cast<uintptr_t>(a) & 7) | (reinterpret_cast<uintptr_t>(b) & 15) | (reinterpret_cast<uintptr_t>(y) & 15)) == 0)
  {
    if (total / 4 < 0x7FFFFFFFLL)
      upcat_fwd_v4_k<unsigned><<<df_grid(total / 4, 256, 16384), 256, 0, (hipStream_t)stream>>>(a, b, y, N, Ca, Cb, Da, Ha, Wa, sd);
    else
      upcat_fwd_v4_k<long long><<<df_grid(total / 4, 256, 16384), 256, 0, (hipStream_t)stream>>>(a, b, y, N, Ca, Cb, Da, Ha, Wa, sd);
  } else
    upcat_fwd_k<<<df_grid(total, 256, 16384), 256, 0, (hipStream_t)stream>>>(a, b, y, N, Ca, Cb, Da, Ha, Wa, sd);
  DF_LAUNCH_CHECK();
  return 0;
}
extern "C" int dfmir_upcat_bwd(const float* dy, float* da, float* db, int N, int Ca, int Cb, int Da,
                               int Ha, int Wa, int sd, void* stream) {
  DF_ARG_CHECK(dy && (da || db) && N > 0 && Ca > 0 && Cb > 0 && (sd == 1 || sd == 2));
  const long long Sa = (long long)Da * Ha * Wa, So = Sa * sd * 4;
  hipStream_t st = (hipStream_t)stream;
  if (da) {
    const bool v2 = (Wa & 1) == 0 && ((reinterpret_cast<uintptr_t>(dy) & 15) | (reinterpret_cast<uintptr_t>(da) & 7)) == 0;
    const long long total = (long long)N * Ca * Sa / (v2 ? 2 : 1);
    const unsigned grid = df_grid(total, 256, 16384);
    const bool small = total < 0x7FFFFFFFLL;
    if (v2) {
      if (small) upcat_bwd_a_k<unsigned, true><<<grid, 256, 0, st>>>(dy, da, N, Ca, Cb, Da, Ha, Wa, sd);
      else upcat_bwd_a_k<long long, true><<<grid, 256, 0, st>>>(dy, da, N, Ca, Cb, Da, Ha, Wa, sd);
    } else {
      if (small) upcat_bwd_a_k<unsigned, false><<<grid, 256, 0, st>>>(dy, da, N, Ca, Cb, Da, Ha, Wa, sd);
      else upcat_bwd_a_k<long long, false><<<grid, 256, 0, st>>>(dy, da, N, Ca, Cb, Da, Ha, Wa, sd);
    }
    DF_LAUNCH_CHECK();
  }
  if (db) {
    cat_channels_launch(nullptr, db, const_cast<float*>(dy), N, (long long)Ca * So, (long long)Cb * So, 1, st);
    DF_LAUNCH_CHECK();
  }
  return 0;
}
extern "C" int dfmir_cat_channels_fwd(const float* a, const float* b, float* y, long long N, long long SA,
                                      long long SB, void* stream) {
  DF_ARG_CHECK(a && b && y && N > 0 && SA > 0 && SB > 0);
  cat_channels_launch(a, b, y, N, SA, SB, 0, (hipStream_t)stream);
  DF_LAUNCH_CHECK();
  return 0;
}
extern "C" int dfmir_cat_channels_bwd(const float* dy, float* da, float* db, long long N, long long SA,
                                      long long SB, void* stream) {
  DF_ARG_CHECK(dy && N > 0 && SA > 0 && SB > 0);
  cat_channels_launch(da, db, const_cast<float*>(dy), N, SA, SB, 1, (hipStream_t)stream);
  DF_LAUNCH_CHECK();
  return 0;
}
extern "C" int dfmir_scale(const float* x, float* y, long long n, float mult, void* stream) {
  DF_ARG_CHECK(x && y && n > 0);
  scale_k<<<df_grid(n, 256, 8192), 256, 0, (hipStream_t)stream>>>(x, y, n, mult);
  DF_LAUNCH_CHECK();
  return 0;
}
```

Measured before the change: 220.4.

## Overlap scale-probe reduction with first loads and reverse instance-norm plane order

```diff
diff --git a/dfmir_amd/csrc/common.h b/dfmir_amd/csrc/common.h
--- a/dfmir_amd/csrc/common.h
+++ b/dfmir_amd/csrc/common.h
@@ -168,6 +168,46 @@
   for (int i = threadIdx.x; i < n; i += blockDim.x) m = fmaxf(m, a[i]);
   return block_max(m, sm);
 }
+__device__ __forceinline__ float probe_lane_load(const float* __restrict__ a, int n) {
+  const int lane = threadIdx.x & 63;
+  return lane < n ? a[lane] : 0.f;
+}
+__device__ __forceinline__ float probe_wave_max(float v, int n) {
+  if (n > 1) {
+    int t = __float_as_int(v);
+    v = fmaxf(v, __int_as_float(__builtin_amdgcn_update_dpp(t, t, 0xB1, 0xF, 0xF, false)));
+    t = __float_as_int(v);
+    v = fmaxf(v, __int_as_float(__builtin_amdgcn_update_dpp(t, t, 0x4E, 0xF, 0xF, false)));
+    t = __float_as_int(v);
+    v = fmaxf(v, __int_as_float(__builtin_amdgcn_update_dpp(t, t, 0x141, 0xF, 0xF, false)));
+    t = __float_as_int(v);
+    v = fmaxf(v, __int_as_float(__builtin_amdgcn_update_dpp(t, t, 0x140, 0xF, 0xF, false)));
+    t = __float_as_int(v);
+    const float r0 = __int_as_float(__builtin_amdgcn_readlane(t, 0)), r1 = __int_as_float(__builtin_amdgcn_readlane(t, 16));
+    const float r2 = __int_as_float(__builtin_amdgcn_readlane(t, 32)), r3 = __int_as_float(__builtin_amdgcn_readlane(t, 48));
+    return fmaxf(fmaxf(r0, r1), fmaxf(r2, r3));
+  }
+  return __int_as_float(__builtin_amdgcn_readfirstlane(__float_as_int(v)));
+}
+#ifndef DF_PROBE_WAVE
+#define DF_PROBE_WAVE 1
+#endif
+
+#ifndef DF_PLANE_ORDER_DEFAULT
+#define DF_PLANE_ORDER_DEFAULT 1
+#endif
+static inline int df_plane_order(int planes) {
+  static DfOptInt o{"DFMIR_PLANE_ORDER", DF_PLANE_ORDER_DEFAULT};
+  const int m = o.get();
+  if (m < 0 || m > 2) return 0;
+  return (m == 2 && (planes & 7)) ? 1 : m;
+}
+__device__ __forceinline__ int df_plane(int order) {
+  const int b = (int)blockIdx.x, n = (int)gridDim.x;
+  if (order == 1) return n - 1 - b;
+  if (order == 2) { const int per = n >> 3; return (b & 7) * per + (per - 1 - (b >> 3)); }
+  return b;
+}
 
 __device__ __forceinline__ bool df_in_coord(int o, int t, int stride, int pad, int dil, int size,
                                             int pad_mode, int& idx) {
diff --git a/dfmir_amd/csrc/conv3x3s.hip b/dfmir_amd/csrc/conv3x3s.hip
--- a/dfmir_amd/csrc/conv3x3s.hip
+++ b/dfmir_amd/csrc/conv3x3s.hip
@@ -317,13 +317,12 @@
   u32x4* __restrict__ Xg = Xs[grp];
 
   float xscale = 1.f, oscale = 1.f, oscale2 = 1.f;
-  if (NSP == 2) {
-    const int ex = scale_exp(reduce_absmax(sc.x_amax, sc.x_n, bs));
+  const bool probe_wave = DF_PROBE_WAVE && NSP == 2 && sc.x_n <= DF_PROBE_SLOTS;
+  const float probe_v = probe_wave ? probe_lane_load(sc.x_amax, sc.x_n) : 0.f;
+  float xmax = 0.f;
+  if (NSP == 2 && !probe_wave) {
+    xmax = reduce_absmax(sc.x_amax, sc.x_n, bs);
     __syncthreads();
-    const int ew = (int)sc.w_trailer[1];
-    xscale = pow2f(ex);
-    oscale = pow2f(-ex);
-    oscale2 = pow2f(-ew);
   }
 
   constexpr unsigned OOB = 0x80000000u;
@@ -427,6 +426,13 @@
 
   P3_GLOADW(0);
   P3_GLOADX(0);
+  if (NSP == 2) {
+    if (probe_wave) xmax = probe_wave_max(probe_v, sc.x_n);
+    const int ex = scale_exp(xmax), ew = (int)sc.w_trailer[1];
+    xscale = pow2f(ex);
+    oscale = pow2f(-ex);
+    oscale2 = pow2f(-ew);
+  }
   P3_LSTOREW(0);
   P3_LSTOREX();
   if (grp == 1 && chunks > 1) P3_GLOADW(1);
@@ -908,6 +914,15 @@
 };
 constexpr int RING_KG = 32;
 
+#ifdef RING_TRACE
+__device__ unsigned g_ring_trace[512 * 8];
+extern "C" int dfmir_ring_trace_dump(unsigned* out) {
+  return (int)hipMemcpyFromSymbol(out, HIP_SYMBOL(g_ring_trace), sizeof(g_ring_trace));
+}
+#define RGT(slot_) { if (threadIdx.x == 0 && blockIdx.x < 512 && blockIdx.y == 0) g_ring_trace[blockIdx.x * 8 + (slot_)] = (unsigned)wall_clock64(); }
+#else
+#define RGT(slot_)
+#endif
 template <int RP>
 __global__ __launch_bounds__(512) void conv3x3_reflect_ring_k(const float* __restrict__ dy, const u32x4* __restrict__ ws,
                                                               float* __restrict__ ring, RingP k, SplitScale sc) {
@@ -927,47 +942,38 @@
                      (strip == 0 ? 0 : strip == 1 ? (k.H - 1) * k.W : strip == 2 ? 0 : k.W - 1);
   const int istr = rowstrip ? 1 : k.W;
 
-  const int ex = scale_exp(reduce_absmax(sc.x_amax, sc.x_n, red));
-  const int ew = (int)sc.w_trailer[1];
-  const float xscale = pow2f(ex), oscale = pow2f(-ex), oscale2 = pow2f(-ew);
+  RGT(0)
+  const bool probe_wave = DF_PROBE_WAVE && sc.x_n <= DF_PROBE_SLOTS;
+  const float probe_v = probe_wave ? probe_lane_load(sc.x_amax, sc.x_n) : 0.f;
+  float xmax = 0.f;
+  if (!probe_wave) xmax = reduce_absmax(sc.x_amax, sc.x_n, red);
 
   const int kg_n = (k.K + 7) >> 3;
+  constexpr int LMAX = RP == 72 ? 64 : 94, NIT = (RING_KG * LMAX + 511) / 512;
+  const int qs = 512 / L, rs = 512 - qs * L;
+  float lv[NIT][8];
+  int li[NIT], lg[NIT];
   {
-    const int npad = RP - L;
-    for (int it = tid; it < NSP * RING_KG * npad; it += 512) {
-      const int q = it % npad, g = it / npad;
-      Ls[g * RP + (q < 2 ? q : L + q)] = u32x4{0u, 0u, 0u, 0u};
-    }
-    const int kz = RING_KG - kg_n;
-    for (int it = tid; it < NSP * kz * L; it += 512) {
-      const int i = it % L, g = it / L, s2 = g / kz, kg = kg_n + g % kz;
-      Ls[(s2 * RING_KG + kg) * RP + i + 2] = u32x4{0u, 0u, 0u, 0u};
-    }
-  }
-  for (int it = tid; it < kg_n * L; it += 512) {
-    const int i = it % L, kg = it / L;
-    float v[8];
-#pragma unroll
-    for (int e = 0; e < 8; ++e) {
-      const int kk = kg * 8 + e;
-      if (!rowstrip && k.cols) v[e] = kk < k.K ? k.cols[(((long long)n * k.K + kk) * 2 + (strip - 2)) * k.H + i] : 0.f;
-      else v[e] = kk < k.K ? dyl[(long long)kk * HW + (long long)i * istr] : 0.f;
-    }
-    u32x4 sp[NSP];
-    split8_s<NSP>(v, xscale, sp);
-#pragma unroll
-    for (int s = 0; s < NSP; ++s) Ls[(s * RING_KG + kg) * RP + i + 2] = sp[s];
-  }
-  __syncthreads();
+    int kg = tid / L, i = tid - kg * L;
+#pragma unroll
+    for (int it = 0; it < NIT; ++it) {
+      li[it] = i; lg[it] = kg;
+#pragma unroll
+      for (int e = 0; e < 8; ++e) {
+        const int kk = kg * 8 + e;
+        const bool ok = kg < kg_n && kk < k.K;
+        if (!rowstrip && k.cols) lv[it][e] = ok ? k.cols[(((long long)n * k.K + kk) * 2 + (strip - 2)) * k.H + i] : 0.f;
+        else lv[it][e] = ok ? dyl[(long long)kk * HW + (long long)i * istr] : 0.f;
+      }
+      i += rs; kg += qs;
+      if (i >= L) { i -= L; ++kg; }
+    }
+  }
+  RGT(1)
 
   const int mb = wid & 3, kh = wid >> 2;
   const int m = m0 + mb * 32 + l31;
   const int nb_n = (L + 2 + 31) >> 5;
-  f32x16 acc[3];
-#pragma unroll
-  for (int b = 0; b < 3; ++b)
-#pragma unroll
-    for (int r = 0; r < 16; ++r) acc[b][r] = 0.f;
   const int chunks = (k.K + 15) >> 4;
   const int tap0 = strip == 0 ? 6 : strip == 1 ? 0 : strip == 2 ? 2 : 0, tapd = rowstrip ? 1 : 3;
   u32x4 a[3][NSP], an[3][NSP], an2[3][NSP];
@@ -981,6 +987,37 @@
   }
   RING_LOADA(a, kh)
   RING_LOADA(an, kh + 2)
+
+  {
+    const int npad = RP - L, g = tid >> 3;
+    for (int q = tid & 7; q < npad; q += 8) Ls[g * RP + (q < 2 ? q : L + q)] = u32x4{0u, 0u, 0u, 0u};
+    const int kz = RING_KG - kg_n;
+    for (int it = tid; it < NSP * kz * L; it += 512) {
+      const int i = it % L, g2 = it / L, s2 = g2 / kz, kg = kg_n + g2 % kz;
+      Ls[(s2 * RING_KG + kg) * RP + i + 2] = u32x4{0u, 0u, 0u, 0u};
+    }
+  }
+  RGT(2)
+  if (probe_wave) xmax = probe_wave_max(probe_v, sc.x_n);
+  const int ex = scale_exp(xmax), ew = (int)sc.w_trailer[1];
+  const float xscale = pow2f(ex), oscale = pow2f(-ex), oscale2 = pow2f(-ew);
+#pragma unroll
+  for (int it = 0; it < NIT; ++it) {
+    if (lg[it] < kg_n) {
+      u32x4 sp[NSP];
+      split8_s<NSP>(lv[it], xscale, sp);
+#pragma unroll
+      for (int s = 0; s < NSP; ++s) Ls[(s * RING_KG + lg[it]) * RP + li[it] + 2] = sp[s];
+    }
+  }
+  __syncthreads();
+  RGT(3)
+
+  f32x16 acc[3];
+#pragma unroll
+  for (int b = 0; b < 3; ++b)
+#pragma unroll
+    for (int r = 0; r < 16; ++r) acc[b][r] = 0.f;
   for (int c = kh; c < chunks; c += 2) {
     RING_LOADA(an2, c + 4)
     const int kg = 2 * c + lhi;
@@ -1005,6 +1042,7 @@
       for (int s = 0; s < NSP; ++s) { a[j][s] = an[j][s]; an[j][s] = an2[j][s]; }
   }
 #undef RING_LOADA
+  RGT(4)
 
   __syncthreads();
   float* xch = reinterpret_cast<float*>(Ls);
@@ -1015,6 +1053,7 @@
       for (int r = 0; r < 16; ++r) xch[((mb * 3 + b) * 16 + r) * 64 + lane] = acc[b][r];
   }
   __syncthreads();
+  RGT(5)
   if (kh == 1) return;
   float* rg = ring + ((long long)(n * 4 + strip) * k.M) * k.RL;
 #pragma unroll
@@ -1029,6 +1068,10 @@
         rg[(long long)mm * k.RL + c] = (acc[b][r] + xch[((mb * 3 + b) * 16 + r) * 64 + lane]) * oscale * oscale2;
     }
   }
+#ifdef RING_TRACE
+  __builtin_amdgcn_s_waitcnt(0x0f70);
+#endif
+  RGT(6)
 }
 
 int df_conv3x3_reflect_ring_ok(const DfConvGeom* g) {
diff --git a/dfmir_amd/csrc/conv3x3s_cs_body.inc b/dfmir_amd/csrc/conv3x3s_cs_body.inc
--- a/dfmir_amd/csrc/conv3x3s_cs_body.inc
+++ b/dfmir_amd/csrc/conv3x3s_cs_body.inc
@@ -40,10 +40,13 @@
   const int oy0 = ty * CS_TH, ox0 = tx * CS_TW;
   const int m0 = bm * (2 * CPG), m0g = m0 + CPG * grp;
 
-  const int ex = scale_exp(reduce_absmax(sc.x_amax, sc.x_n, bs));
-  __syncthreads();
-  const int ew = (int)sc.w_trailer[1];
-  const float xscale = pow2f(ex), oscale = pow2f(-ex), oscale2 = pow2f(-ew);
+  const bool probe_wave = DF_PROBE_WAVE && sc.x_n <= DF_PROBE_SLOTS;
+  const float probe_v = probe_wave ? probe_lane_load(sc.x_amax, sc.x_n) : 0.f;
+  float xmax = 0.f;
+  if (!probe_wave) {
+    xmax = reduce_absmax(sc.x_amax, sc.x_n, bs);
+    __syncthreads();
+  }
 
   constexpr unsigned OOB = 0x80000000u;
   unsigned gvo[NS][8];
@@ -122,13 +125,16 @@
   }
 
 #ifdef CS_NORM_PROBE
-  const float np_r = fmaf(oscale2, 0.f, 1.f), np_m = oscale2 * 0.f, np_lo = fmaf(oscale2, 0.f, -3.0e38f);
+  const float np_r = fmaf(k.slope, 0.f, 1.f), np_m = k.slope * 0.f, np_lo = fmaf(k.slope, 0.f, -3.0e38f);
 #define CS_NORM_PROBE_OPS() _Pragma("unroll") for (int c = 0; c < 8; ++c) v[c] = fmaxf(fmaf(v[c], np_r, np_m), np_lo);
 #else
 #define CS_NORM_PROBE_OPS()
 #endif
   CS_GLOADX(0);
   if (grp == 0) CS_GLOADW(0);
+  if (probe_wave) xmax = probe_wave_max(probe_v, sc.x_n);
+  const int ex = scale_exp(xmax), ew = (int)sc.w_trailer[1];
+  const float xscale = pow2f(ex), oscale = pow2f(-ex), oscale2 = pow2f(-ew);
   CS_LSTOREX(0);
   if (grp == 0) CS_LSTOREW();
   if (grp == 1) { CS_GLOADW(0); CS_GLOADX(1); }
diff --git a/dfmir_amd/csrc/conv3x3s_w2_body.inc b/dfmir_amd/csrc/conv3x3s_w2_body.inc
--- a/dfmir_amd/csrc/conv3x3s_w2_body.inc
+++ b/dfmir_amd/csrc/conv3x3s_w2_body.inc
@@ -17,25 +17,19 @@
   int run_end = run_beg + k.runs_per_block;
   if (run_end > k.runs_total) run_end = k.runs_total;
 
-  const int ex = scale_exp(reduce_absmax(k.x_amax, k.x_n, red));
-  __syncthreads();
-  const int ed = scale_exp(reduce_absmax(k.dy_amax, k.dy_n, red));
-  if (tid < BC) {
-    int e = ed;
-    if (k.dy_pmax) {
-      float m = 0.f;
-      if (co0 + tid < k.Cout)
-        for (int n = 0; n < k.N; ++n) m = fmaxf(m, k.dy_pmax[(long long)n * k.Cout + co0 + tid]);
-      e = scale_exp(m);
-    }
-    edc[tid] = e;
-  }
-  __syncthreads();
+  const bool probe_wave = DF_PROBE_WAVE && k.x_n <= DF_PROBE_SLOTS && k.dy_n <= DF_PROBE_SLOTS;
+  const float probe_x = probe_wave ? probe_lane_load(k.x_amax, k.x_n) : 0.f;
+  const float probe_d = probe_wave ? probe_lane_load(k.dy_amax, k.dy_n) : 0.f;
+  float xmax = 0.f, dmax = 0.f;
+  if (!probe_wave) {
+    xmax = reduce_absmax(k.x_amax, k.x_n, red);
+    __syncthreads();
+    dmax = reduce_absmax(k.dy_amax, k.dy_n, red);
+  }
 
   const int xc = tid & 63, xu = (tid >> 6) & 1, xr = tid >> 7;
   const int dc = tid & (BC - 1), du = (tid >> 7) & 1, dk = tid >> 8;
   const bool xin = k.dbx != nullptr && biz == 0 && (xr == 1 || xr == 2);
-  const float xscale = pow2f(ex), dscale = pow2f(edc[dc]), oscale = pow2f(-ex), oscale2 = pow2f(-edc[wc * 32 + l31]);
   const unsigned hw4 = (unsigned)HW * 4u;
   constexpr unsigned OOB = 0x80000000u;
 
@@ -82,7 +76,7 @@
     rdb = __builtin_amdgcn_raw_buffer_load_b128(bd_, db_ == OOB ? OOB : db_ + 16u, 0, 0);        \
   }
 #ifdef W2_NORM_PROBE
-  const float np_r = fmaf(oscale, 0.f, 1.f), np_m = oscale * 0.f, np_lo = fmaf(oscale, 0.f, -3.0e38f);
+  const float np_r = fmaf((float)k.W, 0.f, 1.f), np_m = (float)k.W * 0.f, np_lo = fmaf((float)k.W, 0.f, -3.0e38f);
 #define W2_NORM_PROBE_OPS() _Pragma("unroll") for (int i = 0; i < 10; ++i) r[i] = fmaxf((r[i] - np_m) * np_r, np_lo);
 #else
 #define W2_NORM_PROBE_OPS()
@@ -160,8 +154,23 @@
     }                                                                                            \
   }
 
+  if (run_beg < run_end) W2_GLOAD(run_beg);
+  if (probe_wave) { xmax = probe_wave_max(probe_x, k.x_n); dmax = probe_wave_max(probe_d, k.dy_n); }
+  const int ex = scale_exp(xmax), ed = scale_exp(dmax);
+  if (tid < BC) {
+    int e = ed;
+    if (k.dy_pmax) {
+      float m = 0.f;
+      if (co0 + tid < k.Cout)
+        for (int n = 0; n < k.N; ++n) m = fmaxf(m, k.dy_pmax[(long long)n * k.Cout + co0 + tid]);
+      e = scale_exp(m);
+    }
+    edc[tid] = e;
+  }
+  __syncthreads();
+
+  const float xscale = pow2f(ex), dscale = pow2f(edc[dc]), oscale = pow2f(-ex), oscale2 = pow2f(-edc[wc * 32 + l31]);
   if (run_beg < run_end) {
-    W2_GLOAD(run_beg);
     W2_LSTORE(0);
     W2_GLOAD(run_beg + 1);
   }
diff --git a/dfmir_amd/csrc/in_blurdown.hip b/dfmir_amd/csrc/in_blurdown.hip
--- a/dfmir_amd/csrc/in_blurdown.hip
+++ b/dfmir_amd/csrc/in_blurdown.hip
@@ -22,16 +22,17 @@
 }
 __global__ __launch_bounds__(1024) void in_relu_blurdown_fwd256_k(const float* __restrict__ x, float* __restrict__ z,
                                                                   float* __restrict__ mean_o, float* __restrict__ rstd_o,
-                                                                  float eps, float* __restrict__ amax) {
+                                                                  float eps, float* __restrict__ amax, int order) {
+  const int pl = df_plane(order);
   constexpr int S = 65536;
   __shared__ float sm[17];
   __shared__ unsigned smax;
   __shared__ float edge[16][128];
   if (threadIdx.x == 0) smax = 0u;
   const int w = __builtin_amdgcn_readfirstlane((int)(threadIdx.x >> 6)), l = threadIdx.x & 63;
-  const __amdgpu_buffer_rsrc_t xr = __builtin_amdgcn_make_buffer_rsrc(const_cast<float*>(x + (long long)blockIdx.x * S), 0,
+  const __amdgpu_buffer_rsrc_t xr = __builtin_amdgcn_make_buffer_rsrc(const_cast<float*>(x + (long long)pl * S), 0,
                                                                        S * 4u, 0x00020000);
-  const __amdgpu_buffer_rsrc_t zr = __builtin_amdgcn_make_buffer_rsrc(z + (long long)blockIdx.x * (S / 4), 0, S, 0x00020000);
+  const __amdgpu_buffer_rsrc_t zr = __builtin_amdgcn_make_buffer_rsrc(z + (long long)pl * (S / 4), 0, S, 0x00020000);
   float4 v[16];
   float s = 0.f;
 #pragma unroll
@@ -49,8 +50,8 @@
   const float var = block_sum(q, sm) / (float)S;
   const float rstd = 1.0f / sqrtf(var + eps);
   if (threadIdx.x == 0) {
-    mean_o[blockIdx.x] = mean;
-    rstd_o[blockIdx.x] = rstd;
+    mean_o[pl] = mean;
+    rstd_o[pl] = rstd;
   }
   float am = 0.f;
 #pragma unroll
@@ -80,19 +81,20 @@
 __global__ __launch_bounds__(1024) void in_relu_blurdown_bwd256_k(const float* __restrict__ dz, const float* __restrict__ x,
                                                                   const float* __restrict__ mean_i,
                                                                   const float* __restrict__ rstd_i, float* __restrict__ dx,
-                                                                  float* __restrict__ amax, float* __restrict__ pmax) {
+                                                                  float* __restrict__ amax, float* __restrict__ pmax, int order) {
+  const int pl = df_plane(order);
   constexpr int S = 65536;
   __shared__ float sm[17];
   __shared__ unsigned smax;
   __shared__ __attribute__((aligned(16))) float dzs[129 * 128];
   if (threadIdx.x == 0) smax = 0u;
   const int w = __builtin_amdgcn_readfirstlane((int)(threadIdx.x >> 6)), l = threadIdx.x & 63;
-  const float mean = mean_i[blockIdx.x], rstd = rstd_i[blockIdx.x];
-  const __amdgpu_buffer_rsrc_t xr = __builtin_amdgcn_make_buffer_rsrc(const_cast<float*>(x + (long long)blockIdx.x * S), 0,
+  const float mean = mean_i[pl], rstd = rstd_i[pl];
+  const __amdgpu_buffer_rsrc_t xr = __builtin_amdgcn_make_buffer_rsrc(const_cast<float*>(x + (long long)pl * S), 0,
                                                                        S * 4u, 0x00020000);
-  const __amdgpu_buffer_rsrc_t zr = __builtin_amdgcn_make_buffer_rsrc(const_cast<float*>(dz + (long long)blockIdx.x * (S / 4)), 0,
+  const __amdgpu_buffer_rsrc_t zr = __builtin_amdgcn_make_buffer_rsrc(const_cast<float*>(dz + (long long)pl * (S / 4)), 0,
                                                                        S, 0x00020000);
-  const __amdgpu_buffer_rsrc_t dr = __builtin_amdgcn_make_buffer_rsrc(dx + (long long)blockIdx.x * S, 0, S * 4u, 0x00020000);
+  const __amdgpu_buffer_rsrc_t dr = __builtin_amdgcn_make_buffer_rsrc(dx + (long long)pl * S, 0, S * 4u, 0x00020000);
   float4 v[16];
 #pragma unroll
   for (int i = 0; i < 16; ++i) v[i] = irb_ld4(xr, 16u * l, (unsigned)(16 * w + i) * 1024u);
@@ -169,20 +171,21 @@
 #undef IRB2_ROW
 #undef IRB2_CA
   if (amax) publish_block_absmax_acc(am, &smax, amax);
-  if (amax && pmax && threadIdx.x == 0) pmax[blockIdx.x] = __uint_as_float(smax);
+  if (amax && pmax && threadIdx.x == 0) pmax[pl] = __uint_as_float(smax);
 }
 
 
 __global__ __launch_bounds__(512) void in_relu_blurdown_fwd128_k(const float* __restrict__ x, float* __restrict__ z,
                                                                  float* __restrict__ mean_o, float* __restrict__ rstd_o,
-                                                                 float eps, float* __restrict__ amax) {
+                                                                 float eps, float* __restrict__ amax, int order) {
+  const int pl = df_plane(order);
   constexpr int S = 16384;
   __shared__ float sm[17];
   __shared__ unsigned smax;
   __shared__ float edge[8][64];
   if (threadIdx.x == 0) smax = 0u;
   const int w = __builtin_amdgcn_readfirstlane((int)(threadIdx.x >> 6)), l = threadIdx.x & 63;
-  const __amdgpu_buffer_rsrc_t xr = __builtin_amdgcn_make_buffer_rsrc(const_cast<float*>(x + (long long)blockIdx.x * S), 0,
+  const __amdgpu_buffer_rsrc_t xr = __builtin_amdgcn_make_buffer_rsrc(const_cast<float*>(x + (long long)pl * S), 0,
                                                                        S * 4u, 0x00020000);
   float2 v[16];
   float s = 0.f;
@@ -201,8 +204,8 @@
   const float var = block_sum(q, sm) / (float)S;
   const float rstd = 1.0f / sqrtf(var + eps);
   if (threadIdx.x == 0) {
-    mean_o[blockIdx.x] = mean;
-    rstd_o[blockIdx.x] = rstd;
+    mean_o[pl] = mean;
+    rstd_o[pl] = rstd;
   }
   float h[16], am = 0.f;
 #pragma unroll
@@ -216,7 +219,7 @@
   edge[w][l] = h[15];
   __syncthreads();
   const float up = w > 0 ? edge[w - 1][l] : h[1];
-  float* zp = z + (long long)blockIdx.x * (S / 4) + (8 * w) * 64 + l;
+  float* zp = z + (long long)pl * (S / 4) + (8 * w) * 64 + l;
 #pragma unroll
   for (int j = 0; j < 8; ++j) {
     const float a0 = j == 0 ? up : h[2 * j - 1];
@@ -228,19 +231,20 @@
 __global__ __launch_bounds__(512) void in_relu_blurdown_bwd128_k(const float* __restrict__ dz, const float* __restrict__ x,
                                                                  const float* __restrict__ mean_i,
                                                                  const float* __restrict__ rstd_i, float* __restrict__ dx,
-                                                                 float* __restrict__ amax, float* __restrict__ pmax) {
+                                                                 float* __restrict__ amax, float* __restrict__ pmax, int order) {
+  const int pl = df_plane(order);
   constexpr int S = 16384;
   __shared__ float sm[17];
   __shared__ unsigned smax;
   __shared__ __attribute__((aligned(16))) float dzs[65 * 64 + 4];
   if (threadIdx.x == 0) smax = 0u;
   const int w = __builtin_amdgcn_readfirstlane((int)(threadIdx.x >> 6)), l = threadIdx.x & 63;
-  const float mean = mean_i[blockIdx.x], rstd = rstd_i[blockIdx.x];
-  const __amdgpu_buffer_rsrc_t xr = __builtin_amdgcn_make_buffer_rsrc(const_cast<float*>(x + (long long)blockIdx.x * S), 0,
+  const float mean = mean_i[pl], rstd = rstd_i[pl];
+  const __amdgpu_buffer_rsrc_t xr = __builtin_amdgcn_make_buffer_rsrc(const_cast<float*>(x + (long long)pl * S), 0,
                                                                        S * 4u, 0x00020000);
-  const __amdgpu_buffer_rsrc_t zr = __builtin_amdgcn_make_buffer_rsrc(const_cast<float*>(dz + (long long)blockIdx.x * (S / 4)), 0,
+  const __amdgpu_buffer_rsrc_t zr = __builtin_amdgcn_make_buffer_rsrc(const_cast<float*>(dz + (long long)pl * (S / 4)), 0,
                                                                        S, 0x00020000);
-  const __amdgpu_buffer_rsrc_t dr = __builtin_amdgcn_make_buffer_rsrc(dx + (long long)blockIdx.x * S, 0, S * 4u, 0x00020000);
+  const __amdgpu_buffer_rsrc_t dr = __builtin_amdgcn_make_buffer_rsrc(dx + (long long)pl * S, 0, S * 4u, 0x00020000);
   float2 v[16];
 #pragma unroll
   for (int i = 0; i < 16; ++i) v[i] = irb_ld2(xr, 8u * l, (unsigned)(16 * w + i) * 512u);
@@ -300,20 +304,22 @@
 #undef IRB1_ROW
 #undef IRB1_CA
   if (amax) publish_block_absmax_acc(am, &smax, amax);
-  if (amax && pmax && threadIdx.x == 0) pmax[blockIdx.x] = __uint_as_float(smax);
+  if (amax && pmax && threadIdx.x == 0) pmax[pl] = __uint_as_float(smax);
 }
 
 int df_in_relu_blurdown_fwd256_launch(const float* x, float* z, float* mean, float* rstd, int planes, float eps, float* z_amax,
                                       hipStream_t st, int W) {
-  if (W == 128) in_relu_blurdown_fwd128_k<<<planes, 512, 0, st>>>(x, z, mean, rstd, eps, z_amax);
-  else in_relu_blurdown_fwd256_k<<<planes, 1024, 0, st>>>(x, z, mean, rstd, eps, z_amax);
+  const int po = df_plane_order(planes);
+  if (W == 128) in_relu_blurdown_fwd128_k<<<planes, 512, 0, st>>>(x, z, mean, rstd, eps, z_amax, po);
+  else in_relu_blurdown_fwd256_k<<<planes, 1024, 0, st>>>(x, z, mean, rstd, eps, z_amax, po);
   DF_LAUNCH_CHECK();
   return 0;
 }
 int df_in_relu_blurdown_bwd256_launch(const float* dz, const float* x, const float* mean, const float* rstd, float* dx,
                                       int planes, float* dx_amax, float* dx_pmax, hipStream_t st, int W) {
-  if (W == 128) in_relu_blurdown_bwd128_k<<<planes, 512, 0, st>>>(dz, x, mean, rstd, dx, dx_amax, dx_pmax);
-  else in_relu_blurdown_bwd256_k<<<planes, 1024, 0, st>>>(dz, x, mean, rstd, dx, dx_amax, dx_pmax);
+  const int po = df_plane_order(planes);
+  if (W == 128) in_relu_blurdown_bwd128_k<<<planes, 512, 0, st>>>(dz, x, mean, rstd, dx, dx_amax, dx_pmax, po);
+  else in_relu_blurdown_bwd256_k<<<planes, 1024, 0, st>>>(dz, x, mean, rstd, dx, dx_amax, dx_pmax, po);
   DF_LAUNCH_CHECK();
   return 0;
 }
diff --git a/dfmir_amd/csrc/norm_resample.hip b/dfmir_amd/csrc/norm_resample.hip
--- a/dfmir_amd/csrc/norm_resample.hip
+++ b/dfmir_amd/csrc/norm_resample.hip
@@ -74,12 +74,13 @@
                                                          const float* __restrict__ res,
                                                          float* __restrict__ y, float* __restrict__ mean_o,
                                                          float* __restrict__ rstd_o, float eps, int relu,
-                                                         float* __restrict__ amax) {
+                                                         float* __restrict__ amax, int order) {
+  const int pl = df_plane(order);
   __shared__ float sm[17];
   __shared__ unsigned smax;
   if (threadIdx.x == 0) smax = 0u;
   constexpr long long S = (long long)NT * 4 * E;
-  const long long base = (long long)blockIdx.x * S;
+  const long long base = (long long)pl * S;
   const float4* x4 = reinterpret_cast<const float4*>(x + base);
   float4 v[E];
   float s = 0.f;
@@ -98,8 +99,8 @@
   const float var = block_sum(q, sm) / (float)S;
   const float rstd = 1.0f / sqrtf(var + eps);
   if (threadIdx.x == 0) {
-    mean_o[blockIdx.x] = mean;
-    rstd_o[blockIdx.x] = rstd;
+    mean_o[pl] = mean;
+    rstd_o[pl] = rstd;
   }
   const float4* r4 = res ? reinterpret_cast<const float4*>(res + base) : nullptr;
   float4* y4 = reinterpret_cast<float4*>(y + base);
@@ -128,13 +129,14 @@
                                                          const float* __restrict__ rstd_i,
                                                          float* __restrict__ dx, int relu,
                                                          float* __restrict__ amax, float* __restrict__ cols, int W,
-                                                         float* __restrict__ pmax) {
+                                                         float* __restrict__ pmax, int order) {
+  const int pl = df_plane(order);
   __shared__ float sm[17];
   __shared__ unsigned smax;
   if (threadIdx.x == 0) smax = 0u;
   constexpr long long S = (long long)NT * 4 * E;
-  const long long base = (long long)blockIdx.x * S;
-  const float mean = mean_i[blockIdx.x], rstd = rstd_i[blockIdx.x];
+  const long long base = (long long)pl * S;
+  const float mean = mean_i[pl], rstd = rstd_i[pl];
   const float4* x4 = reinterpret_cast<const float4*>(x + base);
   const float4* g4 = reinterpret_cast<const float4*>(dy + base);
   float4 xh[E], g[E];
@@ -169,13 +171,13 @@
     am = fmaxf(fmaxf(am, fmaxf(fabsf(o.x), fabsf(o.y))), fmaxf(fabsf(o.z), fabsf(o.w)));
     if (COLS && cols) {
       const int e0 = 4 * (threadIdx.x + NT * i), H = (int)(S / W);
-      float* cp = cols + (long long)blockIdx.x * 2 * H;
+      float* cp = cols + (long long)pl * 2 * H;
       if (e0 % W == 0) cp[e0 / W] = o.x;
       if ((e0 + 3) % W == W - 1) cp[H + (e0 + 3) / W] = o.w;
     }
   }
   if (amax) publish_block_absmax_acc(am, &smax, amax);
-  if (amax && pmax && threadIdx.x == 0) pmax[blockIdx.x] = __uint_as_float(smax);
+  if (amax && pmax && threadIdx.x == 0) pmax[pl] = __uint_as_float(smax);
 }
 
 __global__ __launch_bounds__(256) void instnorm_bwd_k(const float* __restrict__ dy,
@@ -738,9 +740,10 @@
                                     float* y_amax, void* stream) {
   DF_ARG_CHECK(x && mean && rstd && planes > 0 && dfmir_instnorm_stats_ok(S));
   hipStream_t st = (hipStream_t)stream;
-  if (S == 4096) instnorm_fwd_reg_k<256, 4><<<planes, 256, 0, st>>>(x, nullptr, nullptr, mean, rstd, eps, relu, y_amax);
-  else if (S == 16384) instnorm_fwd_reg_k<256, 16><<<planes, 256, 0, st>>>(x, nullptr, nullptr, mean, rstd, eps, relu, y_amax);
-  else instnorm_fwd_reg_k<1024, 16><<<planes, 1024, 0, st>>>(x, nullptr, nullptr, mean, rstd, eps, relu, y_amax);
+  const int po = df_plane_order(planes);
+  if (S == 4096) instnorm_fwd_reg_k<256, 4><<<planes, 256, 0, st>>>(x, nullptr, nullptr, mean, rstd, eps, relu, y_amax, po);
+  else if (S == 16384) instnorm_fwd_reg_k<256, 16><<<planes, 256, 0, st>>>(x, nullptr, nullptr, mean, rstd, eps, relu, y_amax, po);
+  else instnorm_fwd_reg_k<1024, 16><<<planes, 1024, 0, st>>>(x, nullptr, nullptr, mean, rstd, eps, relu, y_amax, po);
   DF_LAUNCH_CHECK();
   return 0;
 }
@@ -748,9 +751,10 @@
                                   int planes, long long S, float eps, int relu, float* y_amax, void* stream) {
   DF_ARG_CHECK(x && y && mean && rstd && planes > 0 && S > 0);
   hipStream_t st = (hipStream_t)stream;
-  if (S == 4096) instnorm_fwd_reg_k<256, 4><<<planes, 256, 0, st>>>(x, res, y, mean, rstd, eps, relu, y_amax);
-  else if (S == 16384) instnorm_fwd_reg_k<256, 16><<<planes, 256, 0, st>>>(x, res, y, mean, rstd, eps, relu, y_amax);
-  else if (S == 65536) instnorm_fwd_reg_k<1024, 16><<<planes, 1024, 0, st>>>(x, res, y, mean, rstd, eps, relu, y_amax);
+  const int po = df_plane_order(planes);
+  if (S == 4096) instnorm_fwd_reg_k<256, 4><<<planes, 256, 0, st>>>(x, res, y, mean, rstd, eps, relu, y_amax, po);
+  else if (S == 16384) instnorm_fwd_reg_k<256, 16><<<planes, 256, 0, st>>>(x, res, y, mean, rstd, eps, relu, y_amax, po);
+  else if (S == 65536) instnorm_fwd_reg_k<1024, 16><<<planes, 1024, 0, st>>>(x, res, y, mean, rstd, eps, relu, y_amax, po);
   else {
     instnorm_fwd_k<<<planes, 256, 0, st>>>(x, res, y, mean, rstd, S, eps, relu);
     if (y_amax) {
@@ -790,12 +794,18 @@
                              float* dx_pmax) {
   DF_ARG_CHECK(dy && x && mean && rstd && dx && planes > 0 && S > 0);
   hipStream_t st = (hipStream_t)stream;
-  if (S == 4096 && dx_cols) instnorm_bwd_reg_k<256, 4, true><<<planes, 256, 0, st>>>(dy, x, mean, rstd, dx, relu, dx_amax, dx_cols, W, dx_pmax);
-  else if (S == 4096) instnorm_bwd_reg_k<256, 4, false><<<planes, 256, 0, st>>>(dy, x, mean, rstd, dx, relu, dx_amax, nullptr, 0, dx_pmax);
-  else if (S == 16384 && dx_cols) instnorm_bwd_reg_k<256, 16, true><<<planes, 256, 0, st>>>(dy, x, mean, rstd, dx, relu, dx_amax, dx_cols, W, dx_pmax);
-  else if (S == 16384) instnorm_bwd_reg_k<256, 16, false><<<planes, 256, 0, st>>>(dy, x, mean, rstd, dx, relu, dx_amax, nullptr, 0, dx_pmax);
+  const int po = df_plane_order(planes);
+  if (S == 4096 && dx_cols) instnorm_bwd_reg_k<256, 4, true><<<planes, 256, 0, st>>>(
+        dy, x, mean, rstd, dx, relu, dx_amax, dx_cols, W, dx_pmax, po);
+  else if (S == 4096) instnorm_bwd_reg_k<256, 4, false><<<planes, 256, 0, st>>>(
+        dy, x, mean, rstd, dx, relu, dx_amax, nullptr, 0, dx_pmax, po);
+  else if (S == 16384 && dx_cols) instnorm_bwd_reg_k<256, 16, true><<<planes, 256, 0, st>>>(
+        dy, x, mean, rstd, dx, relu, dx_amax, dx_cols, W, dx_pmax, po);
+  else if (S == 16384) instnorm_bwd_reg_k<256, 16, false><<<planes, 256, 0, st>>>(
+        dy, x, mean, rstd, dx, relu, dx_amax, nullptr, 0, dx_pmax, po);
   else if (S == 65536 && dx_cols) return df_set_error(-1, __FILE__, __LINE__);
-  else if (S == 65536) instnorm_bwd_reg_k<1024, 16, false><<<planes, 1024, 0, st>>>(dy, x, mean, rstd, dx, relu, dx_amax, nullptr, 0, dx_pmax);
+  else if (S == 65536) instnorm_bwd_reg_k<1024, 16, false><<<planes, 1024, 0, st>>>(
+        dy, x, mean, rstd, dx, relu, dx_amax, nullptr, 0, dx_pmax, po);
   else {
     instnorm_bwd_k<<<planes, 256, 0, st>>>(dy, x, mean, rstd, dx, S, relu);
     if (dx_amax) {
```

New measurement: 222.0, median of 6. Within noise of the previous version (+0.7%).
